# zyt334/AdaFace

Hardware: AMD Instinct MI355X
Metric: 512x512 images/sec @ 50 DDIM steps, batch 8 (higher is better)
Workload: dtype bf16

## Files before the change

adaface_amd/_lib.py:

```python
from __future__ import annotations

import ctypes as C
import os
from pathlib import Path

AF_DTYPE_BF16 = 0
AF_DTYPE_F32 = 1
AF_DTYPE_F16 = 2
DTYPES = {"bf16": AF_DTYPE_BF16, "bfloat16": AF_DTYPE_BF16, "f32": AF_DTYPE_F32, "fp32": AF_DTYPE_F32,
          "float32": AF_DTYPE_F32, "f16": AF_DTYPE_F16, "fp16": AF_DTYPE_F16, "float16": AF_DTYPE_F16}

_LIB_PATH = Path(__file__).resolve().parent / "libadaface_hip.so"


class AfConfig(C.Structure):
    _fields_ = [
        ("dtype", C.c_int),
        ("build_unet", C.c_int),
        ("in_channels", C.c_int), ("model_channels", C.c_int), ("out_channels", C.c_int),
        ("num_res_blocks", C.c_int),
        ("n_attention_resolutions", C.c_int), ("attention_resolutions", C.c_int * 8),
        ("n_channel_mult", C.c_int), ("channel_mult", C.c_int * 8),
        ("num_heads", C.c_int), ("context_dim", C.c_int), ("transformer_depth", C.c_int),
        ("n_context_layers", C.c_int),
        ("build_vae", C.c_int),
        ("vae_ch", C.c_int), ("vae_out_ch", C.c_int), ("vae_num_res_blocks", C.c_int),
        ("vae_z_channels", C.c_int), ("vae_embed_dim", C.c_int),
        ("n_vae_ch_mult", C.c_int), ("vae_ch_mult", C.c_int * 8),
        ("build_vae_encoder", C.c_int), ("vae_in_channels", C.c_int),
        ("build_clip", C.c_int),
        ("clip_vocab", C.c_int), ("clip_hidden", C.c_int), ("clip_layers", C.c_int), ("clip_heads", C.c_int),
        ("clip_intermediate", C.c_int), ("clip_max_pos", C.c_int),
    ]


class AfError(RuntimeError):
    pass


_lib = None

_P = C.c_void_p
_SIGS = [
    ("af_last_error", C.c_char_p, []),
    ("af_version", C.c_int, []),
    ("af_create", C.c_int, [C.c_int, C.POINTER(AfConfig), C.POINTER(_P)]),
    ("af_destroy", None, [_P]),
    ("af_load_tensor", C.c_int, [_P, C.c_char_p, _P, C.c_int, C.POINTER(C.c_int64)]),
    ("af_load_tensor_device", C.c_int, [_P, C.c_char_p, _P, C.c_int, C.POINTER(C.c_int64)]),
    ("af_num_tensors", C.c_int, [_P]),
    ("af_tensor_name", C.c_char_p, [_P, C.c_int]),
    ("af_tensor_loaded", C.c_int, [_P, C.c_int]),
    ("af_tensor_shape", C.c_int, [_P, C.c_int, C.POINTER(C.c_int64)]),
    ("af_set_context", C.c_int, [_P, _P, C.c_int, C.c_int, C.c_int, _P]),
    ("af_unet_forward", C.c_int, [_P, _P, _P, _P, C.c_int, C.c_int, C.c_int, _P]),
    ("af_unet_forward_twin", C.c_int, [_P, _P, _P, _P, C.c_int, C.c_int, C.c_int, _P]),
    ("af_unet_forward_cached", C.c_int, [_P, _P, _P, _P] + [C.c_int] * 6 + [_P]),
    ("af_unet_cache_invalidate", C.c_int, [_P]),
    ("af_ddim_step", C.c_int, [_P, _P, _P, _P, C.c_int64, C.c_float, C.c_float, C.c_float, C.c_float, C.c_float,
                               C.c_float, _P, _P, _P]),
    ("af_dpmpp_coeffs", C.c_int, [C.c_double, C.c_double, C.c_double, C.POINTER(C.c_double)]),
    ("af_dpmpp_step", C.c_int, [_P, _P, _P, _P, C.c_int64] + [C.c_float] * 7 + [_P, _P, _P]),
    ("af_philox4x32_10", C.c_int, [C.POINTER(C.c_uint32), C.POINTER(C.c_uint32), C.POINTER(C.c_uint32)]),
    ("af_philox_randn", C.c_int, [_P, C.c_int64, C.c_int64, _P, C.c_int64, C.c_uint64, C.c_uint32, C.c_uint32, _P]),
    ("af_dpmpp_sde_coeffs", C.c_int, [C.c_double, C.c_double, C.c_double, C.POINTER(C.c_double)]),
    ("af_dpmpp_sde_step", C.c_int, [_P, _P, _P, _P, C.c_int64] + [C.c_float] * 7 + [_P, _P, C.c_float, _P, C.c_int64, _P, C.c_int64,
                                    C.c_uint64, C.c_uint32, _P]),
    ("af_lincomb", C.c_int, [_P, C.c_int64, _P, C.c_float, _P, C.c_float, _P, C.c_float, _P, C.c_float, C.c_int, _P]),
    ("af_vae_decode", C.c_int, [_P, _P, C.c_float, _P, _P, C.c_int, C.c_int, C.c_int, _P]),
    ("af_to_uint8", C.c_int, [_P, _P, C.c_int, C.c_int, C.c_int, _P]),
    ("af_arena_bytes", C.c_int64, [_P]),
    ("af_prof_enable", C.c_int, [C.c_int]),
    ("af_prof_reset", C.c_int, []),
    ("af_set_conv_attn", C.c_int, [_P, C.c_int, C.c_int, C.POINTER(C.c_int), C.POINTER(C.c_int)]),
    ("af_vae_encode", C.c_int, [_P, _P, _P, C.c_int, C.c_int, C.c_int, _P]),
    ("af_posterior_sample", C.c_int, [_P, _P, C.c_float, _P, C.c_int, C.c_int, C.c_int, _P]),
    ("af_prof_set_stride", C.c_int, [C.c_int]),
    ("af_last_gemm_plan", C.c_int, [C.POINTER(C.c_int), C.POINTER(C.c_int), C.POINTER(C.c_int)]),
    ("af_prof_collect", C.c_int, [C.c_int, C.POINTER(C.c_double), C.POINTER(C.c_int64), C.POINTER(C.c_double),
                                  C.POINTER(C.c_double)]),
    ("af_prof_event_overhead_us", C.c_double, [_P, C.c_int]),
    ("af_unet_num_blocks", C.c_int, [_P]),
    ("af_unet_block_shape", C.c_int, [_P, C.c_int, C.c_int, C.c_int, C.POINTER(C.c_int), C.POINTER(C.c_int), C.POINTER(C.c_int)]),
    ("af_unet_set_tap", C.c_int, [_P, C.c_int, _P]),
    ("af_gemm_plan_counts", C.c_int, [C.POINTER(C.c_int64)]),
    ("af_gemm_plan_counts_reset", C.c_int, []),
    ("af_gemm_plan_query", C.c_int, [C.c_int, C.c_int64] + [C.c_int] * 16 + [C.POINTER(C.c_int64)]),
    ("af_norm_plan_query", C.c_int, [C.c_int, C.c_int, C.c_int, C.c_int64, C.c_int, C.c_int, C.POINTER(C.c_int64)]),
    ("af_knob_set", C.c_int, [C.c_char_p, C.c_int]),
    ("af_knob_get", C.c_int, [C.c_char_p, C.POINTER(C.c_int)]),
    ("af_knob_reset", C.c_int, []),
    ("af_op_conv2d", C.c_int, [C.c_int, _P, _P, _P, _P, _P] + [C.c_int] * 9 + [_P]),
    ("af_op_linear", C.c_int, [C.c_int, _P, _P, _P, _P, _P, C.c_int64, C.c_int, C.c_int, C.c_int, _P]),
    ("af_op_conv2d_ex", C.c_int, [C.c_int, _P, _P, _P, _P, _P, C.c_float, _P] + [C.c_int] * 10 + [_P]),
    ("af_op_linear_ex", C.c_int, [C.c_int, _P, _P, _P, _P, C.c_float, _P, C.c_int64, C.c_int, C.c_int, C.c_int, C.c_int, _P]),
    ("af_op_groupnorm", C.c_int, [C.c_int, _P, _P, _P, C.c_float, C.c_int, _P, C.c_int, C.c_int, C.c_int, C.c_int, _P]),
    ("af_op_conv_gn", C.c_int, [_P, _P, _P, _P, _P, _P, C.c_float, C.c_int, _P, _P] + [C.c_int] * 5 + [_P]),
    ("af_set_fp8", C.c_int, [_P, C.c_int]),
    ("af_fp8_gemm_launches", C.c_int64, []),
    ("af_set_fp8_scope", C.c_int, [_P, C.c_int]),
    ("af_get_fp8_scope", C.c_int, [_P]),
    ("af_ff8_launches", C.c_int64, []),
    ("af_op_ff_fp8", C.c_int, [_P] * 4 + [C.c_float] + [_P] * 5 + [C.c_int64] + [C.c_int] * 5 + [_P, _P, _P, C.POINTER(C.c_int), _P]),
    ("af_fp8_num_sites", C.c_int, [_P]),
    ("af_fp8_site_name", C.c_char_p, [_P, C.c_int]),
    ("af_fp8_record", C.c_int, [_P, C.c_int, _P]),
    ("af_fp8_read_record", C.c_int, [_P, C.c_int, C.POINTER(C.c_float), C.POINTER(C.c_int64), _P]),
    ("af_fp8_get_shifts", C.c_int, [_P, C.c_int, C.POINTER(C.c_int)]),
    ("af_fp8_set_shifts", C.c_int, [_P, C.c_int, C.POINTER(C.c_int)]),
    ("af_fp8_shift_for_amax", C.c_int, [C.c_float, C.c_int]),
    ("af_halo8_launches", C.c_int64, []),
    ("af_rowpanel_launches", C.c_int64, []),
    ("af_up_phase4_launches", C.c_int64, []),
    ("af_gn_producer_launches", C.c_int64, []),
    ("af_attn_short_launches", C.c_int64, []),
    ("af_gn_consumer_launches", C.c_int64, []),
    ("af_xattn_fused_launches", C.c_int64, []),
    ("af_conv_attn_short_launches", C.c_int64, []),
    ("af_op_conv_attention", C.c_int, [C.c_int, _P, _P, _P, _P] + [C.c_int] * 6 + [C.c_float] + [C.c_int] * 3 + [_P]),
    ("af_op_vae_attention", C.c_int, [C.c_int, _P, _P, _P, _P, C.c_int, C.c_int, C.c_int, _P, _P, C.POINTER(C.c_int), _P]),
    ("af_op_xattn_fused", C.c_int, [C.c_void_p] * 10 + [C.c_int] * 3 + [C.c_void_p]),
    ("af_op_conv2d_fp8", C.c_int, [_P, _P, _P, _P, _P] + [C.c_int] * 10 + [_P]),
    ("af_op_groupnorm_fp8", C.c_int, [_P, _P, _P, C.c_float, C.c_int, _P, C.c_int, C.c_int, C.c_int, C.c_int, C.c_int, _P]),
    ("af_op_layernorm_fp8", C.c_int, [_P, _P, _P, C.c_float, _P, C.c_int64, C.c_int, C.c_int, _P]),
    ("af_op_groupnorm_fp8_rec", C.c_int, [_P, _P, _P, C.c_float, C.c_int, _P, C.c_int, C.c_int, C.c_int, C.c_int, C.c_int, _P, _P]),
    ("af_op_layernorm_fp8_rec", C.c_int, [_P, _P, _P, C.c_float, _P, C.c_int64, C.c_int, C.c_int, _P, _P]),
    ("af_op_layernorm", C.c_int, [C.c_int, _P, _P, _P, C.c_float, _P, C.c_int64, C.c_int, _P]),
    ("af_op_attention", C.c_int, [C.c_int, _P, _P, _P, _P, C.c_int, C.c_int, C.c_int, C.c_int, C.c_int, C.c_float, C.c_int, _P]),
    ("af_clip_embed_tokens", C.c_int, [_P, _P, C.c_int64, _P, _P]),
    ("af_clip_text_forward", C.c_int, [_P, _P, C.c_int, C.c_int, C.c_float, C.c_float, _P, _P]),
    ("af_clip_text_forward3", C.c_int, [_P, _P, C.c_int, C.c_int, C.c_float, C.c_float, C.c_float, _P, _P]),
    ("af_op_timestep_embedding", C.c_int, [C.c_int, _P, _P, C.c_int, C.c_int, _P]),
    ("af_op_gn_conv1x1", C.c_int, [_P, _P, _P, C.c_float, _P, _P, _P, _P] + [C.c_int] * 5 + [_P]),
    ("af_set_tome", C.c_int, [_P, C.c_double, C.c_int]),
    ("af_tome_plan_query", C.c_int, [C.c_int, C.c_int, C.c_double, C.POINTER(C.c_int64)]),
    ("af_tome_num_sites", C.c_int, [_P]),
    ("af_tome_set_tap", C.c_int, [_P, C.c_int, _P]),
    ("af_op_tome_match", C.c_int, [C.c_int, _P] + [C.c_int] * 4 + [C.c_double, C.c_int, _P, _P, _P, _P]),
    ("af_op_tome_merge", C.c_int, [C.c_int, _P, _P, _P, C.c_float, _P] + [C.c_int] * 4 + [_P, _P]),
    ("af_op_tome_unmerge_add", C.c_int, [C.c_int, _P, _P, _P] + [C.c_int] * 4 + [_P, _P]),
    ("af_set_freeu", C.c_int, [_P, C.c_int] + [C.c_double] * 4),
    ("af_freeu_num_sites", C.c_int, [_P]),
    ("af_freeu_site", C.c_int, [_P, C.c_int, C.POINTER(C.c_int)]),
    ("af_freeu_plan_query", C.c_int, [C.c_int] * 6 + [C.POINTER(C.c_int64)]),
    ("af_op_freeu", C.c_int, [C.c_int, _P, _P] + [C.c_int] * 6 + [C.c_double, C.c_double, _P, _P, _P]),
    ("af_flops_issued", C.c_double, [C.c_int]),
    ("af_clock_probe", C.c_int, [_P, C.c_int, C.POINTER(C.c_double), C.POINTER(C.c_double)]),
]
EXPORTED_SYMBOLS = [s[0] for s in _SIGS]

DEEPCACHE_MODES = {"refresh": 1, "reuse": 2}


def lib_path() -> Path:
    return _LIB_PATH


def load():
    global _lib
    if _lib is not None:
        return _lib
    if not _LIB_PATH.exists():
        raise AfError(
            f"{_LIB_PATH} not found: build it with `python -m adaface_amd.build` (needs hipcc). "
            "adaface_amd has no fallback path.")
    lib = C.CDLL(os.fspath(_LIB_PATH))
    for name, res, args in _SIGS:
        fn = getattr(lib, name)
        fn.restype = res
        fn.argtypes = args
    _lib = lib
    return lib


def set_knob(name: str, value: int) -> None:
    check(load().af_knob_set(name.encode(), int(value)), f"af_knob_set({name})")


def reset_knobs() -> None:
    load().af_knob_reset()


def plan_counts(reset: bool = False) -> dict:
    lib = load()
    c = (C.c_int64 * 10)()
    check(lib.af_gemm_plan_counts(c), "af_gemm_plan_counts")
    out = {f"tile{i}": int(c[i]) for i in range(6)}
    out["halo"], out["splitk"], out["ln_consumer"], out["ln_producer"] = int(c[6]), int(c[7]), int(c[8]), int(c[9])
    out["fp8"] = int(lib.af_fp8_gemm_launches())
    out["ff8"] = int(lib.af_ff8_launches())
    out["halo8"] = int(lib.af_halo8_launches())
    out["rowpanel"] = int(lib.af_rowpanel_launches())
    out["up_phase4"] = int(lib.af_up_phase4_launches())
    out["gn_producer"] = int(lib.af_gn_producer_launches())
    out["attn_short"] = int(lib.af_attn_short_launches())
    out["gn_consumer"] = int(lib.af_gn_consumer_launches())
    out["xattn_fused"] = int(lib.af_xattn_fused_launches())
    out["conv_attn_short"] = int(lib.af_conv_attn_short_launches())
    if reset:
        lib.af_gemm_plan_counts_reset()
    return out


def gemm_plan_query(dtype, M, N, K, cin_pad, ks=1, stride=1, pad=0, up=0, Hs=1, Ws=None, Ho=1, Wo=None, ldc=None, ldo=None,
                    gn_hw=0, gn_cpg=0, flags=0) -> tuple:
    Ws = M if Ws is None else Ws
    Wo = M if Wo is None else Wo
    out = (C.c_int64 * 7)()
    check(load().af_gemm_plan_query(int(dtype), int(M), N, K, cin_pad, ks, stride, pad, up, Hs, Ws, Ho, Wo,
                                    cin_pad if ldc is None else ldc, N if ldo is None else ldo, gn_hw, gn_cpg, flags, out),
          "af_gemm_plan_query")
    return tuple(int(v) for v in out)


def tome_plan_query(H, W, ratio) -> tuple:
    out = (C.c_int64 * 4)()
    check(load().af_tome_plan_query(int(H), int(W), float(ratio), out), "af_tome_plan_query")
    return tuple(int(v) for v in out)


FREEU_KERNELS = ("refused", "single", "chunked")


def freeu_plan_query(dtype, H, W, Ch, Cs, version=1) -> dict:
    out = (C.c_int64 * 4)()
    dt = DTYPES[dtype] if isinstance(dtype, str) else int(dtype)
    check(load().af_freeu_plan_query(dt, int(H), int(W), int(Ch), int(Cs), int(version), out), "af_freeu_plan_query")
    return {"kernel": FREEU_KERNELS[int(out[0])], "launches": int(out[1]), "chunks": int(out[2]), "partial_bytes": int(out[3])}


GN_KERNELS = ("refused", "small", "fold", "finalize")
LN_KERNELS = ("refused", "wave_row", "rowgroup")
_Out5 = C.c_int64 * 5


def norm_plan_query(kind, dtype, B=1, HW=None, C=None, pre_npart=0, rows=None) -> dict:
    dt = DTYPES[dtype] if isinstance(dtype, str) else int(dtype)
    out = _Out5()
    if kind == "groupnorm":
        check(load().af_norm_plan_query(0, dt, int(B), int(HW), int(C), int(pre_npart), out), "af_norm_plan_query")
        return {"kernel": GN_KERNELS[out[0]], "P": int(out[1]), "nchunk": int(out[2]), "npart": int(out[3]), "wide": bool(out[4])}
    if kind == "layernorm":
        check(load().af_norm_plan_query(1, dt, 1, int(rows), int(C), 0, out), "af_norm_plan_query")
        return {"kernel": LN_KERNELS[out[0]], "nv": int(out[1]), "rows_per_block": int(out[2])}
    raise ValueError(f"norm_plan_query: kind {kind!r}")


def check(rc: int, what: str = "") -> None:
    if rc != 0:
        msg = load().af_last_error().decode("utf-8", "replace")
        raise AfError(f"{what or 'libadaface_hip'} failed (rc={rc}): {msg}")


def stream_ptr():
    import torch
    return C.c_void_p(torch.cuda.current_stream().cuda_stream)


def ptr(t):
    return C.c_void_p(0 if t is None else t.data_ptr())
```

adaface_amd/csrc/af_common.h:

```cpp
#pragma once
#include <hip/hip_runtime.h>
#include <stdint.h>
#include <atomic>

typedef __bf16 bf16;
typedef __attribute__((ext_vector_type(8))) __bf16 bf16x8;
typedef _Float16 f16;
typedef __attribute__((ext_vector_type(8))) _Float16 f16x8;
enum AfStorage { AF_ST_BF16 = 0, AF_ST_F32 = 1, AF_ST_F16 = 2 };
template <typename T> struct StorageOf;
template <> struct StorageOf<__bf16> { static constexpr AfStorage value = AF_ST_BF16; };
template <> struct StorageOf<float> { static constexpr AfStorage value = AF_ST_F32; };
template <> struct StorageOf<_Float16> { static constexpr AfStorage value = AF_ST_F16; };
typedef __attribute__((ext_vector_type(16))) float f32x16;
typedef __attribute__((ext_vector_type(4))) float f32x4;

#define AF_WAVE 64

#define HIP_CHECK_RET(expr)                                                       \
  do {                                                                            \
    hipError_t _e = (expr);                                                       \
    if (_e != hipSuccess) {                                                       \
      af_set_error_msg("%s failed: %s (%s:%d)", #expr, hipGetErrorString(_e),     \
                       __FILE__, __LINE__);                                       \
// ... 135 lines not shown
}
__device__ __forceinline__ float gelu_erf_f(float x) {
  return 0.5f * x * (1.0f + erf_as_f(x * 0.70710678118654752440f));
}
__device__ __forceinline__ float gelu_bf16out_f(float x) {
  const float u = x * fmaf(x * x, -0.07068715223f * 1.44269504089f, -1.59748341624f * 1.44269504089f);
  return x * __builtin_amdgcn_rcpf(1.0f + __builtin_amdgcn_exp2f(u));
}

typedef float f32x2 __attribute__((ext_vector_type(2)));
__device__ __forceinline__ f32x2 gelu_bf16out_f2(f32x2 x) {
  f32x2 xc;
  xc.x = __builtin_amdgcn_fmed3f(x.x, -4.0f, 4.0f);
  xc.y = __builtin_amdgcn_fmed3f(x.y, -4.0f, 4.0f);
  const f32x2 s = xc * xc;
  f32x2 q = s * 2.27794120e-08f + (-1.59850396e-06f);
  q = q * s + 4.79536935e-05f;
  q = q * s + (-8.13999317e-04f);
  q = q * s + 8.77231965e-03f;
  q = q * s + (-6.45729896e-02f);
  q = q * s + 3.97883296e-01f;
  const f32x2 ph = xc * q + 0.5f;
  return x * ph;
}

__device__ __forceinline__ unsigned gn_pack4_e4m3(float a, float b, float c, float d, float mul) {
  a = __builtin_amdgcn_fmed3f(a * mul, -448.f, 448.f);
  b = __builtin_amdgcn_fmed3f(b * mul, -448.f, 448.f);
  c = __builtin_amdgcn_fmed3f(c * mul, -448.f, 448.f);
  d = __builtin_amdgcn_fmed3f(d * mul, -448.f, 448.f);
  int v = 0;
  v = __builtin_amdgcn_cvt_pk_fp8_f32(a, b, v, false);
  v = __builtin_amdgcn_cvt_pk_fp8_f32(c, d, v, true);
  return (unsigned)v;
}

__device__ __forceinline__ void fp8_rec_note4(float a, float b, float c, float d, float mul, float& amax, unsigned& nsat) {
  a = fabsf(a); b = fabsf(b); c = fabsf(c); d = fabsf(d);
  amax = fmaxf(fmaxf(amax, fmaxf(a, b)), fmaxf(c, d));
  nsat += (unsigned)(a * mul > 448.f) + (unsigned)(b * mul > 448.f) + (unsigned)(c * mul > 448.f) + (unsigned)(d * mul > 448.f);
}
template <int WAVES = 4>
__device__ __forceinline__ void fp8_rec_commit(float amax, unsigned nsat, unsigned* __restrict__ rec) {
  __shared__ unsigned s_rec[2 * WAVES];
  unsigned m = __float_as_uint(amax);
#pragma unroll
  for (int o = 32; o > 0; o >>= 1) {
    m = max(m, (unsigned)__shfl_xor((int)m, o, 64));
    nsat += (unsigned)__shfl_xor((int)nsat, o, 64);
  }
  const int lane = threadIdx.x & 63, wave = threadIdx.x >> 6;
  if (lane == 0) { s_rec[wave] = m; s_rec[WAVES + wave] = nsat; }
  __syncthreads();
  if (threadIdx.x == 0) {
    if constexpr (WAVES == 4) {
      atomicMax(rec, max(max(s_rec[0], s_rec[1]), max(s_rec[2], s_rec[3])));
      atomicAdd(rec + 1, s_rec[4] + s_rec[5] + s_rec[6] + s_rec[7]);
    } else {
      unsigned mm = s_rec[0], nn = s_rec[WAVES];
#pragma unroll
      for (int w = 1; w < WAVES; ++w) { mm = max(mm, s_rec[w]); nn += s_rec[WAVES + w]; }
      atomicMax(rec, mm);
      atomicAdd(rec + 1, nn);
    }
  }
}

template <typename T> struct Mma;
template <> struct Mma<bf16> {
  static __device__ __forceinline__ void step(const uint4& a, const uint4& b, f32x16& c) {
    c = __builtin_amdgcn_mfma_f32_32x32x16_bf16(__builtin_bit_cast(bf16x8, a),
                                                __builtin_bit_cast(bf16x8, b), c, 0, 0, 0);
  }
};
template <> struct Mma<f16> {
  static __device__ __forceinline__ void step(const uint4& a, const uint4& b, f32x16& c) {
    c = __builtin_amdgcn_mfma_f32_32x32x16_f16(__builtin_bit_cast(f16x8, a), __builtin_bit_cast(f16x8, b), c, 0, 0, 0);
  }
};
template <> struct Mma<float> {
  static __device__ __forceinline__ void step(const uint4& a, const uint4& b, f32x16& c) {
    c = __builtin_amdgcn_mfma_f32_32x32x2f32(__builtin_bit_cast(float, a.x),
                                             __builtin_bit_cast(float, b.x), c, 0, 0, 0);
    c = __builtin_amdgcn_mfma_f32_32x32x2f32(__builtin_bit_cast(float, a.y),
                                             __builtin_bit_cast(float, b.y), c, 0, 0, 0);
    c = __builtin_amdgcn_mfma_f32_32x32x2f32(__builtin_bit_cast(float, a.z),
                                             __builtin_bit_cast(float, b.z), c, 0, 0, 0);
    c = __builtin_amdgcn_mfma_f32_32x32x2f32(__builtin_bit_cast(float, a.w),
                                             __builtin_bit_cast(float, b.w), c, 0, 0, 0);
  }
};

__device__ __forceinline__ int acc_row(int r, int h) { return (r & 3) + 8 * (r >> 2) + 4 * h; }

enum { AF_EPI_NONE = 0, AF_EPI_GEGLU = 1 };

struct ConvGemmParams {
  const void* src;
  long src_batch_stride;
  int ldc;
  int Cin;
  int Hs, Ws;
  int up;
  int Hi, Wi;
  int Ho, Wo;
  int ks, stride, pad;
  const void* W;
  int ldw;
  int Wrows;
  int M, N, K;
  int k_logical;
  const float* bias;
  const void* rowbias;
  int ldrb;
  const void* residual;
  int ldr;
  void* out;
  int ldo;
  int epilogue;
  float alpha;
  long bs_src, bs_w, bs_out, bs_res;
  int splitk;
  void* ws;
  int group_m;
  int howo_shift, wo_shift;
  float* ln_stats_out;
  const float* ln_stats;
  const float* ln_colsum;
  int ln_parts_n;
  float ln_inv_count, ln_eps;
  int epi_direct;
  int ablate;
  int fp8;
  const unsigned char* w_scale;
  int x_scale_e8;
  const void* W_up4;
  int phase4;
  float* gn_stats_out;
  int gn_cpg;
  const float* gn_ab;
  int gn_hw;
};

enum AfGemmKernel {
  AF_GK_NONE = 0,
  AF_GK_WAVE4 = 1,
  AF_GK_HALO4 = 2,
  AF_GK_PP = 3,
  AF_GK_PP_FP8 = 4,
  AF_GK_HALO8 = 5,
  AF_GK_S8 = 6,
  AF_GK_UP_PHASE4 = 7,
  AF_GK_ROWPANEL = 8,
  AF_GK_M128 = 9
};

struct AfGemmPlan {
  int kernel;
  int rowpanel;
  int tile;
  int splitk;
  size_t ws_bytes;
  int halo_tw;
  int group_m;
  int ln_slabs;
};
inline AfGemmPlan af_empty_plan(int kernel, int tile) { return AfGemmPlan{kernel, 0, tile, 1, 0, 0, 1, 0}; }

struct AttnParams {
  const void* q; const void* k; const void* v; void* o;
  int ldq, ldk, ldv, ldo;
  long bsq, bsk, bsv, bso;
  int Nq, Nk, H;
  float scale;
  float* lse;
  int causal;
  const void* vt_pack;
};
```

adaface_amd/csrc/af_conv_gemm.hip:

```cpp
#include "af_device.h"
#include "af_kernels.h"

#include <cstdlib>
#include <cstring>
#include <mutex>

template <int BM, int BN> struct TileCfg {
  static constexpr int XR = BM / 32, WR = BN / 32;
  static constexpr int WM = BM / 2, WN = BN / 2;
  static constexpr int MI = WM / 32, NI = WN / 32;
  static constexpr int TILE_BYTES = (BM + BN) * 128;
  static constexpr int EPI_LD = BN + 4;
  static constexpr int EPI_BYTES = BM * EPI_LD * 4;
  static constexpr int LDS_BYTES = (2 * TILE_BYTES > EPI_BYTES) ? 2 * TILE_BYTES : EPI_BYTES;
};

__device__ __forceinline__ void tile_coords(int wg, int nwg, int ntm, int ntn, int gm, int& tm, int& tn) {
  const int xcd = wg & 7, q = nwg >> 3, r = nwg & 7;
  wg = (xcd < r ? xcd * (q + 1) : r * (q + 1) + (xcd - r) * q) + (wg >> 3);
  const int per_group = gm * ntn;
  const int gid = wg / per_group;
  const int first_m = gid * gm;
  const int gsz = min(ntm - first_m, gm);
  const int in_g = wg - gid * per_group;
// ... 826 lines not shown
  auto dma = [&](__amdgpu_buffer_rsrc_t rs, char* dst, unsigned voff, unsigned soff) {
    if constexpr ((LABL & 1) == 0) lds_dma16(rs, dst, voff, soff);
  };

  if (!(lab & 32)) {
    const unsigned kc = (unsigned)chunk0 * 128u;
#pragma unroll
    for (int q = 0; q < NHQ; ++q)
      if (q < nhq) lds_dma16(rs_x, smem + (wid + 8 * q) * 1024, h_off[q], kc);
#pragma unroll
    for (int s = 0; s < 2; ++s) {
      char* const dst = smem + H::W_BASE + s * H::WBYTES + wid * 1024;
      lds_dma16(rs_w, dst, w_off[0], s * cin2 + kc);
      lds_dma16(rs_w, dst + 8 * 1024, w_off[1], s * cin2 + kc);
      if (g == 0) lds_dma16(rs_w, dst + 16 * 1024, w_off[2], s * cin2 + kc);
    }
  }
#ifdef AF_LAB_ABLATE
  if (lab & 64) st1 = lab_now();
#endif

  auto chunk_loop = [&](auto gc) {
    constexpr int G = decltype(gc)::value;
    constexpr int NWQ = G == 0 ? 3 : 2;
    constexpr int NHT = G == 0 ? 7 : 6;
    char* const wdst = smem + H::W_BASE + wid * 1024;
    for (int c = 0; c < nch; ++c) {
      const unsigned kc = (unsigned)(chunk0 + c) * 128u;
      const int nrec = c + 1 < nch ? (int)0xFFFFFFF0u : 0;
      const __amdgpu_buffer_rsrc_t rs_xn = buffer_rsrc(p.src, nrec);
      const __amdgpu_buffer_rsrc_t rs_wn = buffer_rsrc(p.W, nrec);
      const unsigned hrd8 = (lds0 + (unsigned)((c & 1) * H::HBUF)) >> 3;
      char* const hdst = smem + ((c & 1) ^ 1) * H::HBUF + wid * 1024;
      static_for<0, 9>([&](auto tc) {
        constexpr int TAP = decltype(tc)::value;
        constexpr int KY = TAP / 3, KX = TAP % 3, WS = TAP % 3, WS2 = (TAP + 2) % 3, T2 = TAP + 2;
        constexpr int NB = NI + MI;
        wait_vm<NWQ + (TAP >= 1 && TAP <= NHT ? 1 : 0)>();
        __builtin_amdgcn_s_barrier();
        const unsigned ut = hrd8 + KY * hw16 + KX * 16u;
        unsigned xa0[MI];
#pragma unroll
        for (int j = 0; j < MI; ++j) {
          const unsigned u = xh16[j] + ut;
          xa0[j] = (u << 3) | ((u ^ qsel16) & 0x70u);
        }
        u32x4 xc[MI][2];
        if constexpr ((LABL & 2) != 0) {
#pragma unroll
          for (int j = 0; j < MI; ++j) xc[j][0] = xc[j][1] = u32x4{0u, 0u, 0u, 0u};
        }
        auto rd_block = [&](auto bc) {
          constexpr int bi = decltype(bc)::value;
          if constexpr ((LABL & 2) != 0) {
          } else if constexpr (bi == 0) {
            w8[0][0] = lds_read128<WS * H::WBYTES>(wrd0);
            w8[0][1] = lds_read128<WS * H::WBYTES>(wrd1);
          } else if constexpr (bi <= MI) {
            xc[bi - 1][0] = lds_read128<0>(xa0[bi - 1]);
            xc[bi - 1][1] = lds_read128<0>(xa0[bi - 1] ^ 64u);
          } else {
            w8[bi - MI][0] = lds_read128<WS * H::WBYTES + (bi - MI) * 2048>(wrd0);
            w8[bi - MI][1] = lds_read128<WS * H::WBYTES + (bi - MI) * 2048>(wrd1);
          }
        };
        auto stage_w = [&](auto qc) {
          constexpr int q = decltype(qc)::value;
          char* const dst = wdst + WS2 * H::WBYTES + 8 * q * 1024;
          if constexpr (T2 < 9) dma(rs_w, dst, w_off[q], T2 * cin2 + kc);
          else dma(rs_wn, dst, w_off[q], (T2 - 9) * cin2 + kc + 128u);
        };
        auto stage_h = [&]() {
          if constexpr (TAP < NHT) {
            if constexpr (TAP < NHQ - 1) dma(rs_xn, hdst + 8 * TAP * 1024, h_off[TAP], kc + 128u);
            else dma(rs_xn, hdst + hl6, h_off[NHQ - 1], kc + 128u);
          }
        };
        rd_block(std::integral_constant<int, 0>{});
        rd_block(std::integral_constant<int, 1>{});
        __builtin_amdgcn_sched_barrier(0);
        static_for<0, MI * NI>([&](auto mc) {
          constexpr int m = decltype(mc)::value;
          if constexpr (m < MI) {
            mfma2(acc[NI - 1][m], w8[NI - 1], xp[m]);
          } else {
            constexpr int i = (m - MI) / MI, j = (m - MI) % MI;
            constexpr int issued = (2 + m) < NB ? (2 + m) : NB;
            constexpr int need = i == 0 ? 1 + j : (j == 0 ? MI + i : -1);
            if constexpr (need >= 0) {
              std::integral_constant<int, 2 * (issued - need - 1)> cnt;
              if constexpr (i == 0 && j == 0) wait_block2(cnt, xc[0], w8[0]);
              else if constexpr (i == 0) wait_block(cnt, xc[j]);
              else wait_block(cnt, w8[i]);
            }
            mfma2(acc[i][j], w8[i], xc[j]);
          }
          if constexpr (2 + m < NB) rd_block(std::integral_constant<int, 2 + m>{});
          if constexpr (m == MI + G) stage_w(std::integral_constant<int, 0>{});
          if constexpr (m == MI + 2 + G) stage_w(std::integral_constant<int, 1>{});
          if constexpr (G == 0 && m == MI + 4) stage_w(std::integral_constant<int, 2>{});
          if constexpr (m == MI + 6 + G) stage_h();
          __builtin_amdgcn_sched_barrier(0);
        });
        wait_lgkm_fenced<0>();
#pragma unroll
        for (int j = 0; j < MI; ++j) xp[j][0] = xc[j][0], xp[j][1] = xc[j][1];
      });
    }
  };
  if (g == 0) chunk_loop(std::integral_constant<int, 0>{});
  else chunk_loop(std::integral_constant<int, 1>{});
  wait_vm<0>();
#pragma unroll
  for (int j = 0; j < MI; ++j) mfma2(acc[NI - 1][j], w8[NI - 1], xp[j]);
  __builtin_amdgcn_s_barrier();
#ifdef AF_LAB_ABLATE
  if (lab & 64) st2 = lab_now();
#endif
  if (lab & 8) {
    float sum = 0.f;
#pragma unroll
    for (int i = 0; i < NI; ++i)
#pragma unroll
      for (int j = 0; j < MI; ++j) sum += acc[i][j][0] + acc[i][j][1] + acc[i][j][2] + acc[i][j][3];
    if (sum == 12345.678f) reinterpret_cast<float*>(p.out)[tid] = sum;
    return;
  }
  const int cl = 4 * (lane >> 4);
  float4 bias_r[NI];
#pragma unroll
  for (int i = 0; i < NI; ++i) {
    bias_r[i] = float4{0.f, 0.f, 0.f, 0.f};
    if (p.bias && p.splitk <= 1) bias_r[i] = *reinterpret_cast<const float4*>(p.bias + n0 + g * C::HN + i * 16 + cl);
  }
  float4 ln_cs[1];
  float ln_mu[1], ln_rs[1];
  pp_epilogue<160, 0>(p, acc, bias_r, ln_cs, ln_mu, ln_rs, smem, tid, lane, g, wq, m0, n0, tn, zk);
#ifdef AF_LAB_ABLATE
  if (lab & 64) {
    wait_vm<0>();
    __syncthreads();
    const unsigned long long st3 = lab_now();
    unsigned xcc, hwid;
    asm volatile("s_getreg_b32 %0, hwreg(HW_REG_XCC_ID)" : "=s"(xcc));
    asm volatile("s_getreg_b32 %0, hwreg(HW_REG_HW_ID)" : "=s"(hwid));
    if (tid == 0 && blockIdx.x < 2048 && blockIdx.z == 0) {
      unsigned long long* o = g_lab_stamps + (long)blockIdx.x * 5;
      o[0] = st0; o[1] = st1; o[2] = st2; o[3] = st3; o[4] = ((unsigned long long)xcc << 32) | hwid;
    }
  }
#endif
}

template <bool GEGLU, int KC_ = 5, int MJ_ = 2, int D_ = 2> struct RowPanelCfgT {
  static constexpr int KC = KC_, MJ = MJ_, K = KC * 64, D = D_, NS = D_ + 1;
  static constexpr int WROWS = 16 * MJ, BM = 8 * WROWS;
  static constexpr int BN = GEGLU ? 128 : 160;
  static constexpr int WBYTES = BN * 128, WPIECES = BN / 8;
  static constexpr int NIW = BN / 16;
  static constexpr int OCOLS = GEGLU ? BN / 2 : BN;
  static constexpr int OPITCH = OCOLS * 2 + 16, OBYTES = WROWS * OPITCH;
  static constexpr int LDS_BYTES = NS * WBYTES + 8 * OBYTES;
  static constexpr int CPR = OCOLS / 8;
  static constexpr int NST = WROWS * CPR / 64;
  static_assert(LDS_BYTES <= 160 * 1024 && (WROWS * CPR) % 64 == 0 && (MJ * KC == 10 || (MJ == 1 && KC == 20)) && D >= 2 && D <= KC,
                "row-panel LDS / store mapping / 80 (K = 1280, 16 rows per wave: 160) fragment registers / ring depth");
};
typedef RowPanelCfgT<true> RowPanelCfg;

template <bool GEGLU, int LNMODE, bool RES, int KC_ = 5, int MJ_ = 2, int D_ = 2>
__global__ __launch_bounds__(512) void rowpanel_kernel(const ConvGemmParams p) {
  using C = RowPanelCfgT<GEGLU, KC_, MJ_, D_>;
  typedef bf16 T;
  constexpr int KC = C::KC, NIW = C::NIW, MJ = C::MJ, NST = C::NST, CPR = C::CPR, D = C::D, NS = C::NS;
  static_assert(!(GEGLU && (RES || LNMODE == 2)), "GEGLU: plain or LayerNorm-consumer epilogue, no residual");
  extern __shared__ __attribute__((aligned(1024))) char smem[];
  const int tid = threadIdx.x, lane = tid & 63, wid = __builtin_amdgcn_readfirstlane(tid >> 6);
  const int m0 = blockIdx.x * C::BM;
  const int r0 = m0 + wid * C::WROWS;
  const int ntn_all = p.N / C::BN;
  const int nt_begin = (int)((long)blockIdx.y * ntn_all / gridDim.y), nt_end = (int)((long)(blockIdx.y + 1) * ntn_all / gridDim.y);
  const int ntn = nt_end - nt_begin;
  const __amdgpu_buffer_rsrc_t rs_x = buffer_rsrc(p.src);
  const __amdgpu_buffer_rsrc_t rs_w = buffer_rsrc(p.W);
  const __amdgpu_buffer_rsrc_t rs_o = buffer_rsrc(p.out);

  float* vecs = reinterpret_cast<float*>(smem + C::LDS_BYTES);
  const int nvcol = ntn * C::BN;
  float4 vb[3], vc[3];
#pragma unroll
  for (int r = 0; r < 3; ++r) {
    const int c4 = tid + 512 * r;
    const int col = nt_begin * C::BN + 4 * c4;
    vb[r] = vc[r] = float4{0.f, 0.f, 0.f, 0.f};
    if (c4 < nvcol / 4) {
      if (p.bias) vb[r] = *reinterpret_cast<const float4*>(p.bias + col);
      if constexpr (LNMODE == 1) vc[r] = *reinterpret_cast<const float4*>(p.ln_colsum + col);
    }
  }

  u32x4 xr[MJ][KC][2];
  unsigned orow[NST];
#pragma unroll
  for (int i = 0; i < NST; ++i) {
    const int c = lane + 64 * i;
    const int row = c / CPR, ch = c - row * CPR;
    const int m = r0 + row;
    orow[i] = m < p.M ? (unsigned)((long)m * p.ldo * 2) + (unsigned)ch * 16u : 0xFFFFFFFFu;
  }
  float ln_mu[LNMODE == 1 ? MJ : 1], ln_rs[LNMODE == 1 ? MJ : 1];
#pragma unroll
  for (int j = 0; j < MJ; ++j) {
    const int m = r0 + j * 16 + (lane & 15);
    const bool ok = m < p.M;
    const unsigned xo = ok ? (unsigned)((long)m * p.ldc * 2) + (unsigned)(lane >> 4) * 16u : 0xFFFFFFFFu;
#pragma unroll
    for (int kc = 0; kc < KC; ++kc)
#pragma unroll
      for (int u = 0; u < 2; ++u)
        xr[j][kc][u] = __builtin_bit_cast(u32x4, __builtin_amdgcn_raw_buffer_load_b128(rs_x, xo, (kc * 64 + u * 32) * 2, 0));
    if constexpr (LNMODE == 1) {
      float2 st = float2{0.f, 0.f};
      if (ok && p.ln_parts_n > 0) {
        float s1 = 0.f, s2 = 0.f;
        for (int q = 0; q < p.ln_parts_n; ++q) {
          const float2 pq2 = *reinterpret_cast<const float2*>(p.ln_stats + ((long)q * p.M + m) * 2);
          s1 += pq2.x;
          s2 += pq2.y;
        }
        st = ln_mu_rstd(s1, s2, p.ln_inv_count, p.ln_eps);
      } else if (ok) {
        st = *reinterpret_cast<const float2*>(p.ln_stats + (long)m * 2);
      }
      ln_mu[j] = st.x;
      ln_rs[j] = st.y;
    }
  }

#pragma unroll
  for (int r = 0; r < 3; ++r) {
    const int c4 = tid + 512 * r;
    if (c4 < nvcol / 4) {
      *reinterpret_cast<float4*>(vecs + 4 * c4) = vb[r];
      if constexpr (LNMODE == 1) *reinterpret_cast<float4*>(vecs + nvcol + 4 * c4) = vc[r];
    }
  }
  wait_lgkm<0>();

  if (p.gn_ab) {
    const float* ga = p.gn_ab + (long)(m0 / p.gn_hw) * 2 * C::K + 8 * (lane >> 4);
#pragma unroll
    for (int kc = 0; kc < KC; ++kc)
#pragma unroll
      for (int u = 0; u < 2; ++u) {
        const float* gp = ga + kc * 64 + u * 32;
        float sc[8], sh[8];
        *reinterpret_cast<float4*>(sc) = *reinterpret_cast<const float4*>(gp);
        *reinterpret_cast<float4*>(sc + 4) = *reinterpret_cast<const float4*>(gp + 4);
        *reinterpret_cast<float4*>(sh) = *reinterpret_cast<const float4*>(gp + C::K);
        *reinterpret_cast<float4*>(sh + 4) = *reinterpret_cast<const float4*>(gp + C::K + 4);
#pragma unroll
        for (int j = 0; j < MJ; ++j) {
          Vec16<T> v;
          v.u = __builtin_bit_cast(uint4, xr[j][kc][u]);
#pragma unroll
          for (int e = 0; e < 8; ++e) v.e[e] = from_f32<T>(fmaf(to_f32<T>(v.e[e]), sc[e], sh[e]));
          xr[j][kc][u] = __builtin_bit_cast(u32x4, v.u);
        }
      }
  }

  const int srow = lane >> 3;
  const unsigned dchunk = (unsigned)((lane & 7) ^ srow);
  constexpr int NWQ = (C::WPIECES + 7) / 8;
  const int nwq = (C::WPIECES - wid + 7) / 8;
  unsigned w_off[NWQ];
#pragma unroll
  for (int q = 0; q < NWQ; ++q) w_off[q] = (unsigned)(((wid + 8 * q) * 8 + srow) * p.ldw * 2) + dchunk * 16u;
  const int T_all = ntn * KC;
  const unsigned tile_stride = (unsigned)(C::BN * p.ldw * 2);
  auto stage = [&](int t, int slot) {
    const int ntl = t / KC, kc = t - ntl * KC;
    const bool live = t < T_all;
    const unsigned so = (unsigned)(nt_begin + ntl) * tile_stride + (unsigned)kc * 128u;
#pragma unroll
    for (int q = 0; q < NWQ; ++q)
      if (q < 2 || wid + 8 * q < C::WPIECES)
        lds_dma16(rs_w, smem + slot * C::WBYTES + (wid + 8 * q) * 1024, live ? w_off[q] : 0xFFFFFFFFu, so);
  };

  const unsigned lds0 = (unsigned)(__UINTPTR_TYPE__)((__attribute__((address_space(3))) char*)smem);
  const unsigned fch0 = (unsigned)((lane >> 4) ^ (lane & 7)) * 16u;
  const unsigned fch1 = (unsigned)(((lane >> 4) + 4) ^ (lane & 7)) * 16u;
  const unsigned w_base = (unsigned)((lane & 15) * 128);
  const int cl = 4 * (lane >> 4);

#ifdef AF_LAB_ABLATE
  const int lab = p.ablate >> 4;
#else
  constexpr int lab = 0;
#endif
  char* otile = smem + NS * C::WBYTES + wid * C::OBYTES;
  f32x4 acc[NIW][MJ];
  u32x4 wf[NIW][2];
  auto zero_acc = [&]() {
#pragma unroll
// ... 742 lines not shown
    const int idx = q * 4, u = idx >> 6, i = idx & 63;
    const int cc = u / taps, tap = u - cc * taps;
    float v[4] = {0.f, 0.f, 0.f, 0.f};
    if (cc * 64 < cin_pad) {
      const bf16* sp = wr + (long)tap * cin_pad + cc * 64 + i;
#pragma unroll
      for (int j = 0; j < 4; ++j) v[j] = to_f32<bf16>(sp[j]) * mul;
    }
    dst[q] = pack4_e4m3(v[0], v[1], v[2], v[3]);
  }
}
int af_launch_quant_weight_fp8(const void* w, int rows, int ldw, int cin_pad, int ks, void* w8, int k8, unsigned char* sc,
                               hipStream_t stream) {
  if (cin_pad % 64 != 0 || k8 % 128 != 0 || k8 < ks * ks * cin_pad || ldw != ks * ks * cin_pad) {
    af_set_error_msg("quant_weight_fp8: cin_pad=%d k8=%d ldw=%d ks=%d", cin_pad, k8, ldw, ks);
    return -1;
  }
  hipLaunchKernelGGL(quant_weight_fp8_kernel, dim3(rows), dim3(256), 0, stream, reinterpret_cast<const bf16*>(w), ldw,
                     cin_pad, ks * ks, reinterpret_cast<unsigned char*>(w8), k8, sc);
  HIP_CHECK_RET(hipGetLastError());
  return 0;
}
__global__ __launch_bounds__(256) void cast_fp8_kernel(const bf16* __restrict__ x, unsigned* __restrict__ y, long n4, float mul) {
  for (long i = (long)blockIdx.x * 256 + threadIdx.x; i < n4; i += (long)gridDim.x * 256) {
    Quad<bf16> q;
    q.load(x + i * 4);
    y[i] = pack4_e4m3(to_f32<bf16>(q.e[0]) * mul, to_f32<bf16>(q.e[1]) * mul, to_f32<bf16>(q.e[2]) * mul, to_f32<bf16>(q.e[3]) * mul);
  }
}
int af_launch_cast_fp8(const void* x, void* y, long n, float mul, hipStream_t stream) {
  if (n % 4 != 0) { af_set_error_msg("cast_fp8: n must be a multiple of 4"); return -1; }
  unsigned blocks = (unsigned)((n / 4 + 255) / 256);
  if (blocks > 8192) blocks = 8192;
  if (blocks == 0) return 0;
  hipLaunchKernelGGL(cast_fp8_kernel, dim3(blocks), dim3(256), 0, stream, reinterpret_cast<const bf16*>(x),
                     reinterpret_cast<unsigned*>(y), n / 4, mul);
  HIP_CHECK_RET(hipGetLastError());
  return 0;
}

static std::mutex g_last_plan_mu;
static AfGemmPlan g_af_last_plan = af_empty_plan(AF_GK_WAVE4, 0);
void af_set_last_plan(const AfGemmPlan& pl) { std::lock_guard<std::mutex> lk(g_last_plan_mu); g_af_last_plan = pl; }
AfGemmPlan af_get_last_plan() { std::lock_guard<std::mutex> lk(g_last_plan_mu); return g_af_last_plan; }
std::atomic<long> g_af_gn_consumer_launches{0};
std::atomic<long> g_af_ff8_launches{0};
std::atomic<long> g_af_plan_counts[AF_PC_COUNT] = {};

static void plan_group_m(AfGemmPlan& pl, const ConvGemmParams& p);

static AfGemmPlan plan_fp8(const ConvGemmParams& p, int batch) {
  AfGemmPlan pl = af_empty_plan(AF_GK_NONE, -1);
  const int cand = p.N % 160 == 0 ? 5 : (p.N % 128 == 0 ? 4 : -1);
  if (batch != 1 || p.epilogue == AF_EPI_GEGLU || cand < 0 || p.K % 128 != 0 || p.Cin % 64 != 0 || (p.ks != 1 && p.ks != 3) ||
      p.up != 0 || p.M < 512 || !g_af_knobs.gemm_pp)
    return pl;
  const int KT = p.K / 128;
  const long nb = (long)((p.M + 255) / 256) * (p.N / (cand == 5 ? 160 : 128));
  int s = 1;
  if (nb < 208) {
    s = (int)((256 + nb / 2) / nb);
    if (s > KT / 8) s = KT / 8;
    if (s > 16) s = 16;
    if (s < 1) s = 1;
  }
  const long nbs = nb * s;
  const double fill = (double)nbs / (double)(((nbs + 255) / 256) * 256);
  if (fill < g_af_knobs.gemm_pp_minfill * 0.01) return pl;
  pl.kernel = AF_GK_PP_FP8;
  pl.tile = cand;
  pl.splitk = s;
  plan_group_m(pl, p);
  return pl;
}

static AfGemmPlan plan_tiled(const ConvGemmParams& p, int batch, AfStorage st) {
  const int elem_size = st == AF_ST_F32 ? 4 : 2;
  const bool is_bf16 = st == AF_ST_BF16;
  AfGemmPlan pl = af_empty_plan(AF_GK_WAVE4, 0);
  const bool geglu = p.epilogue == AF_EPI_GEGLU;
  const bool n128 = geglu || (p.N % 128) == 0 || p.N > 640;
  static const int bm[4] = {128, 64, 128, 64}, bn[4] = {128, 128, 64, 64};
  static const double eff[4] = {1.0, 0.88, 0.88, 0.72};
  double best = 1e30;
  for (int t = 0; t < 4; ++t) {
    if (n128 && bn[t] != 128) continue;
    if (!n128 && bn[t] != 64) continue;
    const long nb = (long)((p.M + bm[t] - 1) / bm[t]) * ((p.N + bn[t] - 1) / bn[t]) * batch;
    const double rounds = (double)((nb + 255) / 256);
    const double cost = rounds * bm[t] * bn[t] / eff[t];
    if (cost < best) { best = cost; pl.tile = t; }
  }
  const int BK = 128 / elem_size;
  const int KT = p.K / BK;
  const long nb = (long)((p.M + bm[pl.tile] - 1) / bm[pl.tile]) * ((p.N + bn[pl.tile] - 1) / bn[pl.tile]) * batch;
  if (batch == 1 && !geglu && nb < 256 && KT >= 16) {
    const int target = g_af_knobs.splitk_target;
    int s = (int)((target + nb - 1) / nb);
    if (s > KT / 8) s = KT / 8;
    if (s > 16) s = 16;
    if (s >= 2) {
      pl.tile = n128 ? 0 : 2;
      const long nb2 = (long)((p.M + bm[pl.tile] - 1) / bm[pl.tile]) * ((p.N + bn[pl.tile] - 1) / bn[pl.tile]);
      s = (int)((target + nb2 - 1) / nb2);
      if (s > KT / 8) s = KT / 8;
      if (s > 16) s = 16;
      if (s >= 2) pl.splitk = s;
    }
  }
  if (g_af_knobs.small_m_tile64 && batch == 1 && !geglu && p.M <= 1024 && p.N % 64 == 0 && KT <= 32) {
    const long nb64 = (long)((p.M + 63) / 64) * (p.N / 64);
    if (nb64 >= 64 && nb64 <= 1024) { pl.tile = 3; pl.splitk = 1; }
  }
  if (p.ks == 3 && p.stride == 1 && p.up == 0 && p.pad == 1 && batch == 1 && !geglu && pl.splitk == 1 &&
      p.Ho == p.Hi && p.Wo == p.Wi && p.ldc >= p.Cin && g_af_knobs.conv_halo) {
    if (p.Wo % 32 == 0 && p.Ho % 4 == 0) pl.halo_tw = 32;
    else if (p.Wo % 16 == 0 && p.Ho % 8 == 0) pl.halo_tw = 16;
    if (pl.halo_tw) {
      const long nb128 = (long)(p.M / 128) * ((p.N + 127) / 128), nb64 = (long)(p.M / 128) * ((p.N + 63) / 64);
      const double c128 = (double)((nb128 + 255) / 256) * 128, c64 = (double)((nb64 + 255) / 256) * 64 / 0.9;
      pl.tile = (n128 && c128 <= c64) ? 0 : 2;
      if (!n128 && (p.N % 64) != 0) pl.tile = 2;
    }
  }
  if (is_bf16 && batch == 1 && p.K % 64 == 0 && p.Cin % 64 == 0 && g_af_knobs.gemm_pp) {
    int cand = -1;
    if (!geglu && p.N % 160 == 0) cand = 5;
    else if (p.N % 128 == 0) cand = 4;
    if (cand >= 0) {
      const int tbn = cand == 5 ? 160 : 128;
      const long nb = (long)((p.M + 255) / 256) * (p.N / tbn);
      int s = 1;
      if (!geglu && nb < 208) {
        s = (int)((256 + nb / 2) / nb);
        if (s > KT / 16) s = KT / 16;
        if (s > 16) s = 16;
        if (s < 1) s = 1;
      }
      const long nbs = nb * s;
      const double fill = (double)nbs / (double)(((nbs + 255) / 256) * 256);
      if (fill >= g_af_knobs.gemm_pp_minfill * 0.01 && p.M >= 512) {
        pl.tile = cand;
        pl.splitk = s;
        pl.halo_tw = 0;
      }
    }
  }
  if (pl.tile == 5 && pl.halo_tw == 0 && p.ks == 3 && p.stride == 1 && p.pad == 1 && p.up == 0 && p.Ho == p.Hi && p.Wo == p.Wi &&
      (p.Wo == 16 || p.Wo == 32 || p.Wo == 64) && (p.Ho & (p.Ho - 1)) == 0 && p.Ho >= 256 / p.Wo && p.M % 256 == 0 &&
      p.K == 9 * p.Cin && p.ldc >= p.Cin && (g_af_knobs.conv_halo8 & 1) && !p.ln_stats && !p.ln_stats_out) {
    pl.halo_tw = 256;
    while (pl.splitk > 1 && (p.Cin / 64) % pl.splitk != 0) --pl.splitk;
  }
  if (is_bf16 && (g_af_knobs.conv_halo8 & 2) && g_af_knobs.gemm_pp && af_conv_s8_slices(p, batch) && !p.gn_stats_out &&
      (p.Wo <= 16 || (g_af_knobs.conv_halo8 & 4))) {
    pl.tile = 5;
    pl.halo_tw = 8;
    pl.splitk = af_conv_s8_slices(p, batch);
  }
  const int ft = g_af_knobs.gemm_tile;
  if (ft >= 0 && ft < 4 && !(geglu && bn[ft] != 128)) pl.tile = ft;
  const int fs = g_af_knobs.gemm_splitk;
  if (fs >= 1 && batch == 1 && !geglu) pl.splitk = fs > KT ? KT : fs;
  if (pl.halo_tw == 8 && (pl.tile != 5 || pl.splitk != af_conv_s8_slices(p, batch))) pl.halo_tw = 0;
  if (pl.splitk > 1 && pl.halo_tw != 256 && pl.halo_tw != 8) pl.halo_tw = 0;
  if (pl.halo_tw == 256 && (pl.tile != 5 || (p.Cin / 64) % pl.splitk != 0)) pl.halo_tw = 0;
  pl.kernel = pl.halo_tw == 8 ? AF_GK_S8 : pl.halo_tw == 256 ? AF_GK_HALO8 : pl.halo_tw ? AF_GK_HALO4 : pl.tile >= 4 ? AF_GK_PP : AF_GK_WAVE4;
  plan_group_m(pl, p);
  return pl;
}

static void plan_group_m(AfGemmPlan& pl, const ConvGemmParams& p) {
  static const int bm[4] = {128, 64, 128, 64}, bn[4] = {128, 128, 64, 64};
  {
    const bool h4 = pl.kernel == AF_GK_HALO4;
    const int tbm = h4 ? 128 : (pl.tile >= 4 ? 256 : bm[pl.tile]);
    const int tbn = h4 ? ((pl.tile == 0 || pl.tile == 1) ? 128 : 64) : (pl.tile == 5 ? 160 : pl.tile == 4 ? 128 : bn[pl.tile]);
    const int MT = (p.M + tbm - 1) / tbm, NT = (p.N + tbn - 1) / tbn;
    const int resident = pl.tile >= 4 ? 32 : 32 * ((tbm * tbn >= 128 * 128) ? 2 : 3);
    const bool taps_reuse = pl.halo_tw || (pl.tile >= 4 && p.ks > 1);
    const double xb = (double)p.M * (p.K / (p.ks * p.ks)) * (taps_reuse ? (p.stride == 1 ? 1.5 : 1.0) : (double)(p.ks * p.ks) / (p.stride * p.stride));
    const double wb = (double)p.N * p.K;
    double bestc = 1e300;
    int bestg = 1;
    for (int gmm = 1; gmm <= 64; gmm *= 2) {
      const int gm_eff = gmm < MT ? gmm : MT;
      int gn_eff = resident / gm_eff;
      if (gn_eff < 1) gn_eff = 1;
      if (gn_eff > NT) gn_eff = NT;
      const double c = xb * ((double)NT / gn_eff) + wb * ((double)MT / gm_eff);
      if (c < bestc * 0.999) { bestc = c; bestg = gmm; }
    }
    pl.group_m = g_af_knobs.gemm_groupm >= 1 ? g_af_knobs.gemm_groupm : bestg;
  }
}

template <typename T, int BM, int BN, bool DMA>
static int launch_cfg2(const ConvGemmParams& p, int batch, hipStream_t stream) {
  using C = TileCfg<BM, BN>;
  const int ntm = (p.M + BM - 1) / BM, ntn = (p.N + BN - 1) / BN;
  dim3 grid(ntm * ntn, 1, p.splitk > 1 ? p.splitk : batch);
  return af_launch_lds<conv_gemm_kernel<T, BM, BN, DMA>>(grid, dim3(256), C::LDS_BYTES, C::LDS_BYTES, stream, p);
}
template <typename T, int BM, int BN>
static int launch_cfg(const ConvGemmParams& p, int batch, hipStream_t stream) {
  const int force = g_af_knobs.gemm_dma;
  const int kt_per_slice = p.K / (128 / (int)sizeof(T)) / (p.splitk > 1 ? p.splitk : 1);
  const bool use_dma = force >= 0 ? force != 0 : kt_per_slice >= 32;
  return use_dma ? launch_cfg2<T, BM, BN, true>(p, batch, stream) : launch_cfg2<T, BM, BN, false>(p, batch, stream);
}

static void set_launch_fields(ConvGemmParams& p, const AfGemmPlan& pl) {
  auto lg2 = [](int v) { int s = 0; while ((1 << s) < v) ++s; return (v > 0 && (1 << s) == v) ? s : -1; };
  p.howo_shift = lg2(p.Ho * p.Wo);
  p.wo_shift = lg2(p.Wo);
  p.group_m = pl.group_m > 0 ? pl.group_m : 1;
  p.epi_direct = (p.gn_stats_out || p.phase4) ? 1 : 0;
  p.ablate = p.phase4 ? 0 : g_af_knobs.ablate;
}

template <typename T> static int launch_splitk_reduce(const ConvGemmParams& p, hipStream_t stream) {
  const long nq = (long)p.M * (p.N >> 2);
  unsigned blocks = (unsigned)((nq + 255) / 256);
  if (blocks > 4096) blocks = 4096;
  hipLaunchKernelGGL((splitk_reduce_kernel<T>), dim3(blocks), dim3(256), 0, stream, p);
  HIP_CHECK_RET(hipGetLastError());
  return 0;
}

template <int BN, int LNMODE, bool GATHER, bool FP8, int SCHED>
static int launch_pp_one(const ConvGemmParams& p, dim3 grid, hipStream_t stream) {
  using C = PpCfg<BN>;
  return af_launch_lds<conv_gemm_pp_kernel<BN, GATHER, LNMODE, FP8, SCHED>>(grid, dim3(512), C::LDS_BYTES, C::LDS_BYTES, stream, p);
}
template <int BN, int LNMODE, bool GATHER> static int launch_pp_bf16(const ConvGemmParams& p, dim3 grid, hipStream_t stream) {
  const bool phased = p.epilogue == AF_EPI_GEGLU || (GATHER && !(p.up == 0 && p.ks * p.ks <= 31));
  if (!phased) return launch_pp_one<BN, LNMODE, GATHER, false, 2>(p, grid, stream);
  if constexpr (GATHER || (BN == 128 && LNMODE != 2)) return launch_pp_one<BN, LNMODE, GATHER, false, 0>(p, grid, stream);
  af_set_error_msg("conv_gemm: GEGLU on the ping-pong kernel needs the 128-column tile and no LayerNorm statistics");
  return -1;
}
template <int BN> static int launch_pp(const ConvGemmParams& p, hipStream_t stream) {
  const bool gather = !(p.ks == 1 && p.pad == 0);
  dim3 grid(((p.M + 255) / 256) * (p.N / BN), 1, p.splitk > 1 ? p.splitk : 1);
  if (p.ln_stats || p.ln_stats_out) {
    if (gather || p.splitk > 1 || (p.ln_stats && p.ln_stats_out) || (p.ln_stats_out && p.epilogue == AF_EPI_GEGLU)) {
      af_set_error_msg("conv_gemm: LayerNorm-fused launch needs a 1x1 GEMM without split-K");
      return -1;
    }
    return p.ln_stats ? launch_pp_bf16<BN, 1, false>(p, grid, stream) : launch_pp_bf16<BN, 2, false>(p, grid, stream);
  }
  return gather ? launch_pp_bf16<BN, 0, true>(p, grid, stream) : launch_pp_bf16<BN, 0, false>(p, grid, stream);
}

template <int BN> static int launch_pp8(const ConvGemmParams& p, hipStream_t stream) {
  const bool gather = !(p.ks == 1 && p.pad == 0);
  dim3 grid(((p.M + 255) / 256) * (p.N / BN), 1, p.splitk > 1 ? p.splitk : 1);
  return gather ? launch_pp_one<BN, 0, true, true, 2>(p, grid, stream) : launch_pp_one<BN, 0, false, true, 2>(p, grid, stream);
}

static int validate_fp8(const ConvGemmParams& p) {
  if (p.K % 128 != 0 || p.Cin % 64 != 0 || (p.ks != 1 && p.ks != 3) || p.K < p.ks * p.ks * p.Cin || p.ldw < p.K ||
      p.ldw % 16 != 0 || p.ldc % 16 != 0 || p.ldc < p.Cin || !p.w_scale || p.epilogue == AF_EPI_GEGLU || p.ln_stats || p.ln_stats_out) {
    af_set_error_msg("conv_gemm fp8: K=%d Cin=%d ks=%d ldw=%d ldc=%d (need K%%128==0, Cin%%64==0, ks 1|3, 16-byte pitches, row scales)",
                     p.K, p.Cin, p.ks, p.ldw, p.ldc);
    return -1;
  }
  return 0;
}

bool af_ff_geglu_fp8_ok(const ConvGemmParams& p) {
  return g_af_knobs.gemm_pp && p.fp8 && p.epilogue == AF_EPI_GEGLU && p.ks == 1 && p.pad == 0 && p.stride == 1 && p.up == 0 &&
         p.K % 128 == 0 && p.Cin % 64 == 0 && p.K >= p.Cin && p.ldw >= p.K && p.ldw % 16 == 0 && p.ldc % 16 == 0 && p.ldc >= p.Cin &&
         p.w_scale && p.N % 128 == 0 && p.Wrows >= p.N && p.ldo % 16 == 0 && p.ldo >= p.N / 2 && p.M >= 512 && !p.residual &&
         !p.rowbias && !p.ln_stats && !p.ln_stats_out && !p.gn_stats_out && !p.gn_ab &&
         (double)p.M * p.ldc < 4294967280.0 && (double)p.Wrows * p.ldw < 4294967280.0;
}
int af_launch_ff_geglu_fp8(ConvGemmParams p, float out_mul, unsigned* rec, hipStream_t stream) {
  if (!af_ff_geglu_fp8_ok(p) || ((__UINTPTR_TYPE__)p.out & 15) != 0 || !(out_mul > 0.f)) {
    af_set_error_msg("ff_geglu_fp8: M=%d N=%d K=%d Cin=%d ldo=%d cannot be launched (ask af_ff_geglu_fp8_ok first)", p.M, p.N, p.K, p.Cin, p.ldo);
    return -1;
  }
  using C = PpCfg<128>;
  AfGemmPlan pl = af_empty_plan(AF_GK_PP_FP8, 4);
  plan_group_m(pl, p);
  p.splitk = 1;
  p.ws = nullptr;
  set_launch_fields(p, pl);
  af_set_last_plan(pl);
  g_af_plan_counts[AF_PC_FP8] += 1;
  g_af_ff8_launches += 1;
  AfProfScope prof(AF_K_PP_FP8, stream, 2.0 * p.M * (double)p.N * (p.k_logical ? p.k_logical : p.K),
                   (double)p.M * p.Cin + (double)p.N * p.K + (double)p.M * p.N * 0.5);
  const dim3 grid(((p.M + 255) / 256) * (p.N / 128), 1, 1);
  if (rec) return af_launch_lds<ff_geglu_fp8_kernel<true>>(grid, dim3(512), C::LDS_BYTES, C::LDS_BYTES, stream, p, out_mul, rec);
  return af_launch_lds<ff_geglu_fp8_kernel<false>>(grid, dim3(512), C::LDS_BYTES, C::LDS_BYTES, stream, p, out_mul, nullptr);
}

template <int LABL> static int launch_halo8_lab(const ConvGemmParams& p, hipStream_t stream) {
  dim3 grid((p.M / 256) * (p.N / 160), 1, p.splitk > 1 ? p.splitk : 1);
  return af_launch_lds<conv3x3_halo8_kernel<LABL>>(grid, dim3(512), Halo8Cfg::LDS_BYTES, Halo8Cfg::LDS_BYTES, stream, p);
}
static int launch_halo8(const ConvGemmParams& p, hipStream_t stream) {
  if (p.Cin % 64 != 0 || (p.Cin / 64) % (p.splitk > 1 ? p.splitk : 1) != 0) {
    af_set_error_msg("conv_gemm: halo kernel needs K slices of whole 64-channel chunks (Cin=%d splitk=%d)", p.Cin, p.splitk);
    return -1;
  }
#ifdef AF_LAB_ABLATE
  switch ((p.ablate >> 4) & 7) {
    case 1: return launch_halo8_lab<1>(p, stream);
    case 2: return launch_halo8_lab<2>(p, stream);
    case 3: return launch_halo8_lab<3>(p, stream);
    case 4: return launch_halo8_lab<4>(p, stream);
    case 5: return launch_halo8_lab<5>(p, stream);
    case 6: return launch_halo8_lab<6>(p, stream);
    case 7: return launch_halo8_lab<7>(p, stream);
    default: break;
  }
#endif
  return launch_halo8_lab<0>(p, stream);
}

template <typename T, int TW, int BN> static int launch_halo(const ConvGemmParams& p, hipStream_t stream) {
  using C = HaloCfg<TW, BN>;
  dim3 grid((p.M / 128) * ((p.N + BN - 1) / BN), 1, 1);
  return af_launch_lds<conv3x3_halo_kernel<T, TW, BN>>(grid, dim3(256), C::LDS_BYTES, C::LDS_BYTES, stream, p);
}

__global__ __launch_bounds__(256) void up_phase4_weights_kernel(const bf16* __restrict__ w3, bf16* __restrict__ w4, long total,
                                                                int rows, int cin, int ldw3) {
  const long idx = (long)blockIdx.x * 256 + threadIdx.x;
  if (idx >= total) return;
  const int n = (int)(idx / cin), c = (int)(idx - (long)n * cin);
  float w[3][3];
#pragma unroll
  for (int ky = 0; ky < 3; ++ky)
#pragma unroll
    for (int kx = 0; kx < 3; ++kx) w[ky][kx] = to_f32<bf16>(w3[(long)n * ldw3 + (ky * 3 + kx) * cin + c]);
  const long ld4 = 4L * cin;
#pragma unroll
  for (int ph = 0; ph < 4; ++ph) {
    const int dy = ph >> 1, dx = ph & 1;
#pragma unroll
    for (int ty = 0; ty < 2; ++ty)
#pragma unroll
      for (int tx = 0; tx < 2; ++tx) {
        const int ylo = ty == 0 ? 0 : (dy == 0 ? 1 : 2), yhi = ty == 0 ? (dy == 0 ? 0 : 1) : 2;
        const int xlo = tx == 0 ? 0 : (dx == 0 ? 1 : 2), xhi = tx == 0 ? (dx == 0 ? 0 : 1) : 2;
        float sum = 0.f;
#pragma unroll
        for (int ky = 0; ky < 3; ++ky)
#pragma unroll
          for (int kx = 0; kx < 3; ++kx)
            if (ky >= ylo && ky <= yhi && kx >= xlo && kx <= xhi) sum += w[ky][kx];
        w4[((long)ph * rows + n) * ld4 + (ty * 2 + tx) * cin + c] = from_f32<bf16>(sum);
      }
  }
}
int af_launch_up_phase4_weights(const void* w3, int rows, int cin, int ldw3, void* w4, hipStream_t stream) {
  const long total = (long)rows * cin;
  if (total <= 0) return 0;
  hipLaunchKernelGGL(up_phase4_weights_kernel, dim3((unsigned)((total + 255) / 256)), dim3(256), 0, stream,
                     reinterpret_cast<const bf16*>(w3), reinterpret_cast<bf16*>(w4), total, rows, cin, ldw3);
  HIP_CHECK_RET(hipGetLastError());
  return 0;
}
static bool up_phase4_ok(const ConvGemmParams& p, int batch) {
  auto pow2 = [](int v) { return v > 0 && (v & (v - 1)) == 0; };
  return p.W_up4 && g_af_knobs.conv_up_phase4 && g_af_knobs.gemm_pp && batch == 1 && p.up == 1 && p.ks == 3 && p.stride == 1 &&
         p.pad == 1 && p.Cin % 64 == 0 && p.ldc >= p.Cin && p.K == 9 * p.Cin && (p.N % 160 == 0 || p.N % 128 == 0) &&
         pow2(p.Hs) && pow2(p.Ws) && p.Ho == 2 * p.Hs && p.Wo == 2 * p.Ws && p.M == (p.M / (p.Ho * p.Wo)) * p.Ho * p.Wo &&
         p.M / 4 >= 1024 && !p.residual && !p.rowbias && !p.ln_stats && !p.ln_stats_out && p.epilogue != AF_EPI_GEGLU &&
         (double)4 * p.Wrows * 4 * p.Cin * 2 < 4294967280.0;
}
static void up_phase4_params(ConvGemmParams& p) {
  p.W = p.W_up4;
  p.ks = 2; p.up = 0; p.pad = 1;
  p.Hi = p.Ho = p.Hs; p.Wi = p.Wo = p.Ws;
  p.M /= 4;
  p.K = 4 * p.Cin; p.ldw = p.K;
  p.k_logical = p.K;
  p.phase4 = 1;
  p.splitk = 1; p.ws = nullptr;
}
static int launch_up_phase4(const ConvGemmParams& p, int tile, hipStream_t stream) {
  const int bn = tile == 5 ? 160 : 128;
  dim3 grid(((p.M + 255) / 256) * (p.N / bn), 4, 1);
  return bn == 160 ? launch_pp_one<160, 0, true, false, 2>(p, grid, stream) : launch_pp_one<128, 0, true, false, 2>(p, grid, stream);
}

bool af_conv_gn_stats_ok(const ConvGemmParams& p, const AfGemmPlan& pl, int cpg) {
  auto pow2 = [](int v) { return v > 0 && (v & (v - 1)) == 0; };
  const int hn = pl.tile == 5 ? 80 : 64;
  const bool eight_wave = pl.kernel == AF_GK_PP || pl.kernel == AF_GK_PP_FP8 || pl.kernel == AF_GK_HALO8;
  return g_af_knobs.gn_producer && eight_wave && pl.splitk <= 1 && p.ks == 3 && p.stride == 1 && p.up == 0 &&
         p.epilogue != AF_EPI_GEGLU && !p.ln_stats && !p.ln_stats_out && cpg >= 2 && cpg % 2 == 0 && hn % cpg == 0 &&
         p.N == 32 * cpg && pow2(p.Ho * p.Wo) && p.Ho * p.Wo >= 64 && p.M % 64 == 0;
}

static int rowpanel_kind(const ConvGemmParams& p, int batch) {
  const int lvl = g_af_knobs.geglu_rowpanel;
  if (!lvl || batch != 1 || p.ks != 1 || p.pad != 0 || p.stride != 1 || p.up != 0 || p.rowbias || p.fp8 ||
      p.Cin != p.K || p.ldc < p.Cin)
    return 0;
  const bool geglu = p.epilogue == AF_EPI_GEGLU;
  if (p.K == RowPanelCfg::K && p.M >= 128 * RowPanelCfg::BM) {
    if (p.gn_ab && (p.gn_hw <= 0 || p.gn_hw % RowPanelCfg::BM != 0)) return 0;
    if (geglu) return (p.N % RowPanelCfg::BN == 0 && !p.residual && !p.ln_stats_out) ? 1 : 0;
    return (lvl >= 2 && p.N % 160 == 0 && p.alpha == 1.0f && !(p.ln_stats && p.ln_stats_out) && (!p.residual || p.ldr % 4 == 0)) ? 2 : 0;
  }
  if (g_af_knobs.gemm_m128 && !geglu && !(p.ln_stats && p.ln_stats_out) && (!p.ln_stats || p.alpha == 1.0f) && !p.gn_ab && p.M % 128 == 0 &&
      p.M <= 8192 && p.N % 160 == 0 &&
      p.K % 64 == 0 && p.K >= 256 && (!p.residual || p.ldr % 4 == 0) && p.ldo % 8 == 0 && ((__UINTPTR_TYPE__)p.out & 15) == 0) {
    const long nb128 = (long)(p.M / 128) * (p.N / 160), nb256 = (long)((p.M + 255) / 256) * (p.N / 160);
    if (nb128 >= 128 && nb128 <= 512 && nb256 <= 170) return 6;
    if (nb128 % 256 == 0 && nb128 <= 1024 && nb256 % 256 != 0) return 6;
  }
  if (g_af_knobs.gemm_m128 && !geglu && !(p.ln_stats && p.ln_stats_out) && (!p.ln_stats || p.alpha == 1.0f) && !p.gn_ab && p.M % 128 == 0 &&
      p.M > 8192 && p.M <= 16384 && p.N % 160 == 0 && p.K % 64 == 0 && p.K >= 256 && p.K <= 1280 && (!p.residual || p.ldr % 4 == 0) &&
      p.ldo % 8 == 0 && ((__UINTPTR_TYPE__)p.out & 15) == 0 && (long)(p.M / 128) * (p.N / 160) == 512)
    return 6;
  if (p.K == 1280)
    return (lvl >= 4 && p.N == 1280 && p.M >= 4096 && !geglu && p.alpha == 1.0f && !p.ln_stats && !p.ln_stats_out && !p.gn_ab &&
            (!p.residual || p.ldr % 4 == 0)) ? 3 : 0;
  if (p.K == 640 && lvl >= 3 && p.M >= 16384 && !p.residual) {
    if (p.gn_ab) return 0;
    if (p.ln_stats_out) return 0;
    if (geglu) return p.N % 128 == 0 ? 4 : 0;
    return (p.N % 160 == 0 && p.N >= 1920 && p.alpha == 1.0f) ? 5 : 0;
  }
  return 0;
}

AfGemmPlan af_plan_conv_gemm(const ConvGemmParams& p, int batch, AfStorage st, bool have_ws) {
  const bool is_bf16 = st == AF_ST_BF16;
  AfGemmPlan pl;
  if (p.fp8) {
    pl = plan_fp8(p, batch);
  } else if (is_bf16 && up_phase4_ok(p, batch)) {
    ConvGemmParams q = p;
    up_phase4_params(q);
    pl = af_empty_plan(AF_GK_UP_PHASE4, p.N % 160 == 0 ? 5 : 4);
    plan_group_m(pl, q);
    return pl;
  } else {
    pl = plan_tiled(p, batch, st);
    if (pl.kernel == AF_GK_PP && pl.splitk == 1) pl.ln_slabs = (p.N / (pl.tile == 5 ? 160 : 128)) * 2;
  }
  if (!have_ws) pl.splitk = 1;
  if (const int rk = is_bf16 ? rowpanel_kind(p, batch) : 0; rk == 6 || (rk && pl.splitk == 1)) {
    pl.kernel = rk == 6 ? AF_GK_M128 : AF_GK_ROWPANEL;
    pl.rowpanel = rk == 6 ? 0 : rk;
    pl.splitk = 1;
  }
  if (pl.splitk > 1) pl.ws_bytes = (size_t)pl.splitk * p.M * p.N * sizeof(float);
  return pl;
}

static int launch_bf16_only(const ConvGemmParams& p, const AfGemmPlan& pl, hipStream_t stream) {
  switch (pl.kernel) {
    case AF_GK_PP: return pl.tile == 4 ? launch_pp<128>(p, stream) : launch_pp<160>(p, stream);
    case AF_GK_PP_FP8: return pl.tile == 4 ? launch_pp8<128>(p, stream) : launch_pp8<160>(p, stream);
    case AF_GK_HALO8: return launch_halo8(p, stream);
    case AF_GK_S8: return af_launch_conv_s8(p, stream);
    case AF_GK_UP_PHASE4: return launch_up_phase4(p, pl.tile, stream);
    case AF_GK_M128: return launch_gemm_m128(p, stream);
    case AF_GK_ROWPANEL:
      switch (pl.rowpanel) {
        case 1: return launch_geglu_rowpanel(p, stream);
        case 2: return launch_plain_rowpanel(p, stream);
        case 3: return launch_plain_rowpanel_k1280(p, stream);
        case 4: return launch_geglu_rowpanel(p, stream, true);
        case 5: return launch_plain_rowpanel(p, stream, true);
        default: break;
      }
      break;
    default: break;
  }
  af_set_error_msg("conv_gemm: plan names no kernel (kernel %d, row-panel kind %d)", pl.kernel, pl.rowpanel);
  return -1;
}

template <typename T>
int af_launch_conv_gemm(const ConvGemmParams& p_in, int batch, hipStream_t stream, const AfGemmPlan* plan, void* ws) {
  constexpr int BK = 128 / sizeof(T);
  constexpr bool kBf16 = std::is_same_v<T, bf16>;
  ConvGemmParams p = p_in;
  if (p.fp8) {
    if (!kBf16) { af_set_error_msg("conv_gemm: fp8 operands need the bf16 storage mode"); return -1; }
    if (batch != 1) { af_set_error_msg("conv_gemm fp8: no batched form"); return -1; }
    if (int rc = validate_fp8(p)) return rc;
  } else {
    if (p.gn_ab && !kBf16) { af_set_error_msg("conv_gemm: consumer-side GroupNorm exists on the bf16 row-panel kernels only"); return -1; }
    if (p.K % BK != 0 || p.Cin % BK != 0 || p.K != p.ks * p.ks * p.Cin) {
      af_set_error_msg("conv_gemm: K=%d Cin=%d ks=%d must satisfy K==ks*ks*Cin and Cin%%%d==0", p.K, p.Cin, p.ks, BK);
      return -1;
    }
    if (p.ldw % (16 / (int)sizeof(T)) != 0 || p.ldc % (16 / (int)sizeof(T)) != 0) {
      af_set_error_msg("conv_gemm: ldw/ldc must be multiples of 16 bytes");
      return -1;
    }
    if (p.epilogue == AF_EPI_GEGLU && p.N % 64 != 0) { af_set_error_msg("conv_gemm: GEGLU needs N%%64==0"); return -1; }
  }
  if (p.N % 4 != 0 || p.ldo % 4 != 0 || (p.residual && p.ldr % 4 != 0) || (p.rowbias && p.ldrb % 4 != 0)) {
    af_set_error_msg("conv_gemm: N/ldo/ldr/ldrb must be multiples of 4 (N=%d ldo=%d)", p.N, p.ldo);
    return -1;
  }
  if (p.M <= 0 || p.N <= 0) return 0;
  {
    const int HoWo = p.Ho * p.Wo > 0 ? p.Ho * p.Wo : 1;
    const double nb = (double)((p.M + HoWo - 1) / HoWo), esz = p.fp8 ? 1.0 : (double)sizeof(T);
    const double src_bytes = nb * (double)p.src_batch_stride * esz, w_bytes = (double)p.Wrows * p.ldw * esz;
    if (src_bytes >= 4294967280.0 || w_bytes >= 4294967280.0) {
      af_set_error_msg("conv_gemm: operand of %.2f GB exceeds the 4 GB range of the 32-bit gather offsets (split the batch)",
                       (src_bytes > w_bytes ? src_bytes : w_bytes) / 1e9);
      return -1;
    }
  }
  const AfGemmPlan pl = (plan && (ws || plan->splitk <= 1)) ? *plan : af_plan_conv_gemm(p, batch, StorageOf<T>::value, ws != nullptr);
  const int k = pl.kernel;
  if ((k == AF_GK_PP_FP8) != (p.fp8 != 0)) {
    af_set_error_msg("conv_gemm%s: shape M=%d N=%d K=%d has no %s plan (ask af_plan_conv_gemm first)", p.fp8 ? " fp8" : "", p.M, p.N, p.K,
                     p.fp8 ? "fp8" : "bf16-operand");
    return -1;
  }
  if (!kBf16 && k != AF_GK_WAVE4 && k != AF_GK_HALO4) { af_set_error_msg("conv_gemm: kernel %d of the plan is bf16 only", k); return -1; }
  p.splitk = pl.splitk;
  p.ws = ws;
  af_set_last_plan(pl);
  if (g_af_knobs.plan_log && k != AF_GK_PP_FP8 && k != AF_GK_UP_PHASE4)
    fprintf(stderr, "[af plan] M=%ld N=%d K=%d ks=%d stride=%d up=%d HoWo=%dx%d batch=%d tile=%d halo=%d splitk=%d rowpanel=%d res=%d geglu=%d ln=%d\n",
            (long)p.M, p.N, p.K, p.ks, p.stride, p.up, p.Ho, p.Wo, batch, pl.tile, pl.halo_tw, pl.splitk, k == AF_GK_M128 ? 6 : pl.rowpanel,
            p.residual ? 1 : 0, p.epilogue == AF_EPI_GEGLU ? 1 : 0, (p.ln_stats || p.ln_stats_out) ? 1 : 0);
  if (k == AF_GK_PP_FP8 || k == AF_GK_UP_PHASE4) {
    g_af_plan_counts[k == AF_GK_PP_FP8 ? AF_PC_FP8 : AF_PC_UP_PHASE4] += 1;
  } else {
    g_af_plan_counts[k == AF_GK_HALO4 ? AF_PC_HALO4 : AF_PC_TILE0 + (pl.tile >= 0 && pl.tile < 6 ? pl.tile : 0)] += 1;
    if (k == AF_GK_HALO8) g_af_plan_counts[AF_PC_HALO8] += 1;
    if (p.ln_stats) g_af_plan_counts[AF_PC_LN_CONSUMER] += 1;
    if (p.ln_stats_out) g_af_plan_counts[AF_PC_LN_PRODUCER] += 1;
  }
  if (pl.splitk > 1) g_af_plan_counts[AF_PC_SPLITK] += 1;
  if (p.gn_stats_out) {
    if (!kBf16 || batch != 1 || !af_conv_gn_stats_ok(p, pl, p.gn_cpg)) {
      af_set_error_msg("conv_gemm: GroupNorm partial sums asked of a launch that cannot write them (ask af_conv_gn_stats_ok first)");
      return -1;
    }
    g_af_plan_counts[AF_PC_GN_PRODUCER] += 1;
  }
  const bool rows_resident = k == AF_GK_ROWPANEL || k == AF_GK_M128;
  if ((p.ln_stats || p.ln_stats_out) && k != AF_GK_PP && k != AF_GK_M128 && !(k == AF_GK_ROWPANEL && pl.tile >= 4)) {
    af_set_error_msg("conv_gemm: LayerNorm-fused launch planned on a kernel without that epilogue (kernel %d, tile %d)", k, pl.tile);
    return -1;
  }
  if (p.ln_parts_n > 0 && !rows_resident) {
    af_set_error_msg("conv_gemm: un-finalised LayerNorm statistics handed to a launch that is not a row-panel one");
    return -1;
  }
  if (p.gn_ab && k != AF_GK_ROWPANEL) {
    af_set_error_msg("conv_gemm: consumer-side GroupNorm asked of a launch that is not a row-panel one (ask af_plan_conv_gemm first)");
    return -1;
  }
  if (p.gn_ab) g_af_gn_consumer_launches += 1;
  if (rows_resident) g_af_plan_counts[AF_PC_ROWPANEL] += 1;
  if (k == AF_GK_UP_PHASE4) up_phase4_params(p);
  set_launch_fields(p, pl);
  int prof_cls = pl.tile == 5 ? ((p.ks == 1 && p.pad == 0) ? AF_K_PP160_PLAIN : AF_K_PP160_GATHER) : (pl.tile == 4 ? AF_K_PP128 : AF_K_CONV_GEMM);
  double flops = 2.0 * p.M * (double)p.N * (p.k_logical ? p.k_logical : p.K) * batch;
  double bytes = ((double)p.M * p.K / (p.ks * p.ks) + (double)p.N * p.K + (double)p.M * p.N) * batch * sizeof(T);
  if (k == AF_GK_HALO8) prof_cls = AF_K_HALO8;
  if (k == AF_GK_PP_FP8) { prof_cls = AF_K_PP_FP8; bytes = (double)p.M * p.Cin + (double)p.N * p.K + (double)p.M * p.N * 2.0; }
  if (k == AF_GK_UP_PHASE4) { flops *= 4; bytes = ((double)p.M * p.Cin + 4.0 * p.N * p.K + 4.0 * p.M * p.N) * 2; }
  AfProfScope prof(prof_cls, stream, flops, bytes);
  int rc;
  switch (k) {
    case AF_GK_WAVE4:
      switch (pl.tile) {
        case 0: rc = launch_cfg<T, 128, 128>(p, batch, stream); break;
        case 1: rc = launch_cfg<T, 64, 128>(p, batch, stream); break;
        case 2: rc = launch_cfg<T, 128, 64>(p, batch, stream); break;
        default: rc = launch_cfg<T, 64, 64>(p, batch, stream); break;
      }
      break;
    case AF_GK_HALO4: {
      const bool bn128 = pl.tile == 0 || pl.tile == 1;
      if (pl.halo_tw == 32) rc = bn128 ? launch_halo<T, 32, 128>(p, stream) : launch_halo<T, 32, 64>(p, stream);
      else rc = bn128 ? launch_halo<T, 16, 128>(p, stream) : launch_halo<T, 16, 64>(p, stream);
      break;
    }
    default:
      if constexpr (kBf16) rc = launch_bf16_only(p, pl, stream);
      else rc = -1;
      break;
  }
  if (rc) return rc;
  return p.splitk > 1 ? launch_splitk_reduce<T>(p, stream) : 0;
}

template int af_launch_conv_gemm<bf16>(const ConvGemmParams&, int, hipStream_t, const AfGemmPlan*, void*);
template int af_launch_conv_gemm<float>(const ConvGemmParams&, int, hipStream_t, const AfGemmPlan*, void*);
template int af_launch_conv_gemm<f16>(const ConvGemmParams&, int, hipStream_t, const AfGemmPlan*, void*);
```

adaface_amd/csrc/af_kernels.h:

```cpp
#pragma once
#include "af_common.h"

AfGemmPlan af_plan_conv_gemm(const ConvGemmParams& p, int batch, AfStorage st, bool have_ws = true);
template <typename T>
int af_launch_conv_gemm(const ConvGemmParams& p, int batch, hipStream_t stream, const AfGemmPlan* plan = nullptr,
                        void* ws = nullptr);
template <typename T> int af_launch_attention(const AttnParams& p, int B, int dh, hipStream_t stream);
template <typename T> long af_attn_short_pack_elems(int B, int H, int dh, int Nk);
template <typename T>
int af_launch_attn_short_pack(const void* v, int ldv, long bsv, int Nk, int H, int dh, int B, void* vt, hipStream_t stream);
extern std::atomic<long> g_af_attn_short_launches;
bool af_conv_attn_short_ok(bool is_bf16, int dh, int Nk, bool vt_pack, int ks, int groups);
int af_launch_conv_attn_short(const AttnParams& p, int B, int dh, int ks, int groups, int Hh, int Ww, const float* amap,
                              hipStream_t stream);
extern std::atomic<long> g_af_conv_attn_short_launches;
struct AfXattnFusedParams {
  const void* x; int ldx; int M; int rows_per_sample;
  const float* ln_stats; int ln_parts_n; float ln_inv_count, ln_eps;
  const void* wq; int ldwq; const float* q_colsum; const float* q_bias;
  const void* kvpack;
  const void* wo; int ldwo; const float* o_bias;
  void* out; int ldo;
  float* ln_stats_out;
  int Nk;
// ... 5 lines not shown
int af_launch_xattn_fused(const AfXattnFusedParams& a, hipStream_t stream);
extern std::atomic<long> g_af_xattn_fused_launches;

bool af_ff_geglu_fp8_ok(const ConvGemmParams& p);
int af_launch_ff_geglu_fp8(ConvGemmParams p, float out_mul, unsigned* rec, hipStream_t stream);
extern std::atomic<long> g_af_ff8_launches;

enum AfGnKernel {
  AF_GNK_REFUSED = 0,
  AF_GNK_SMALL = 1,
  AF_GNK_FOLD = 2,
  AF_GNK_FINALIZE = 3
};
struct AfGnPlan {
  int kernel;
  int P;
  int nchunk;
  int npart;
  int wide_stats;
};
AfGnPlan af_plan_groupnorm(AfStorage st, int B, int HW, int Cn, int pre_npart, bool to_affine = false);
enum AfLnKernel {
  AF_LNK_REFUSED = 0,
  AF_LNK_WAVE_ROW = 1,
  AF_LNK_ROWGROUP = 2
};
struct AfLnPlan {
  int kernel;
  int nv;
  int rows_per_block;
};
AfLnPlan af_plan_layernorm(AfStorage st, long rows, int Cn);

size_t af_gn_workspace_bytes(int B, int HW);
template <typename T>
int af_launch_groupnorm(const void* x, long x_bs, int ldx, int B, int HW, int Cn, const float* gamma,
                        const float* beta, float eps, int silu, void* y, long y_bs, int ldy, void* workspace,
                        hipStream_t stream, float fp8_mul = 0.f,
                        const float* pre_partial = nullptr, int pre_npart = 0,
                        unsigned* fp8_rec = nullptr);
template <typename T>
int af_launch_groupnorm_fold(const void* x, long x_bs, int ldx, int B, int HW, int Cn, const float* gamma, const float* beta,
                             float eps, void* workspace, hipStream_t stream, const float* pre_partial, int pre_npart,
                             float* ab_out);
bool af_conv_gn_stats_ok(const ConvGemmParams& p, const AfGemmPlan& pl, int cpg);
int af_conv_s8_slices(const ConvGemmParams& p, int batch);
int af_launch_conv_s8(const ConvGemmParams& p, hipStream_t stream);
template <typename T>
int af_launch_layernorm(const void* x, int ldx, long rows, int Cn, const float* gamma, const float* beta,
                        float eps, void* y, int ldy, hipStream_t stream, float fp8_mul = 0.f, unsigned* fp8_rec = nullptr);

struct AfTomePlan { long Nd, Ns, r, Np; };
int af_tome_plan(int H, int W, double ratio, AfTomePlan* pl);
size_t af_tome_match_ws_bytes(int B, int H, int W);
template <typename T>
int af_launch_tome_match(const void* x, int ldx, int B, int H, int W, int C, double ratio, int normalize, int* node_idx,
                         float* node_max, int* map, void* ws, hipStream_t s);
template <typename T>
int af_launch_tome_merge(const void* x, int ldx, const float* gamma, const float* beta, float eps, const int* map, int B, int N,
                         int Np, int C, void* y, int ldy, hipStream_t s);
template <typename T>
int af_launch_tome_unmerge_add(const void* o, int ldo, const void* res, int ldr, const int* map, int B, int N, int Np, int C,
                               void* y, int ldy, float* ln_stats_out, int ln_parts, hipStream_t s);

enum AfFreeuKernel {
  AF_FREEUK_REFUSED = 0,
  AF_FREEUK_SINGLE = 1,
  AF_FREEUK_CHUNKED = 2
};
struct AfFreeuPlan {
  int kernel;
  int launches;
  int nchunk;
  long part_bytes;
};
int af_plan_freeu(int H, int W, int Ch, int Cs, int version, AfFreeuPlan* pl);
size_t af_freeu_ws_bytes(int B, int H, int W, int Ch, int Cs, int version);
template <typename T>
int af_launch_freeu(void* cat, int ld, int B, int H, int W, int Ch, int Cs, int version, float b, float s, bool backbone,
                    bool skip, void* ws, hipStream_t stream);

template <typename T>
int af_launch_nchw_to_nhwc(const float* x, void* y, int B, int Cn, int HW, int Cpad, float scale, hipStream_t s);
template <typename T> int af_launch_nhwc_to_nchw(const void* x, float* y, int B, int Cn, int HW, int ld, hipStream_t s);
template <typename T> int af_launch_cast_f32(const float* x, void* y, long n, hipStream_t s);
template <typename T>
int af_launch_gather_rows_cast(const float* x, const int* rowmap, void* y, long rows, int D, hipStream_t s);
template <typename T>
int af_launch_conv_attn(const void* q, int ldq, long bsq, const void* kv, int ldk, long bsk, int tok0, float* sN,
                        float* lse, void* o, int ldo, long bso, int B, int N, int H, int dh, int Hh, int Ww,
                        float scale, int ks, hipStream_t s);
inline size_t af_conv_attn_map_floats(int groups, int B, int H, int N) { return (size_t)groups * B * H * N + 1; }
template <typename T>
int af_launch_conv_attn_map(const void* q, int ldq, long bsq, const void* k, int ldk, long bsk, int tok0, int groups,
                            float* amap, int B, int H, int dh, int Hh, int Ww, int ks, hipStream_t s);
template <typename T> int af_launch_cast_to_f32(const void* x, float* y, long n, hipStream_t s);
template <typename T> int af_launch_timestep_embedding(const long long* t, void* y, int B, int dim, hipStream_t s);
template <typename T> int af_launch_silu(const void* x, void* y, long n, hipStream_t s);
template <typename T> int af_launch_quick_gelu(const void* x, void* y, long n, hipStream_t s);
template <typename T>
int af_launch_embed_rows(const long long* ids, const void* table, int vocab, int D, float* y, long n, hipStream_t s);
template <typename T>
int af_launch_add_pos_cast(const float* x, const void* pos, int Tn, int D, void* y, long rows, hipStream_t s);
template <typename T> int af_launch_blend2(const void* a, float w0, const void* b, float w1, void* y, long n, hipStream_t s);
template <typename T>
int af_launch_copy_channels(const void* src, int lds_, void* dst, int ldd, int off, int Cn, long npix, hipStream_t s);
int af_launch_ddim_step(const float* x, const float* eps_c, const float* eps_u, const float* noise, long n,
                        float guidance, float a_t, float a_prev, float sqrt_one_minus_at, float sigma_t,
                        float temperature, float* x_prev, float* pred_x0, hipStream_t s);
int af_launch_dpmpp_step(const float* x, const float* eps_c, const float* eps_u, const float* x0_prev, long n, float guidance,
                         float alpha_t, float sigma_t, float c_x, float c_d, float w_cur, float w_prev, float* x_next,
                         float* x0_out, hipStream_t s);
int af_launch_posterior_sample(const float* mom, const float* noise, float scale, float* z, int B, int Cn, long HW,
                               hipStream_t s);
int af_launch_lincomb(float* out, long n, const float* x0, float w0, const float* x1, float w1, const float* x2, float w2,
                      const float* x3, float w3, int mode, hipStream_t s);
template <typename T> int af_launch_softmax_rows(void* x, int ld, int ncols, long rows, hipStream_t s);
template <typename T>
int af_launch_transpose(const void* x, long x_bs, int ldx, void* y, long y_bs, int R, int Cn, int B, hipStream_t s);
struct AfVaeAttnTaps {
  void* scores;
  void* probs;
  int plans[2][3];
};
bool af_vae_attn_shape_ok(int dtype, int N);
int af_vae_attn_core(int dtype, void* qkv, void* sc, void* vt, void* out, int B, int N, int C, hipStream_t s,
                     AfVaeAttnTaps* taps = nullptr);
template <typename T> int af_launch_to_uint8(const void* x, int ld, uint8_t* y, long npix, hipStream_t s);
int af_launch_nchw_to_uint8(const float* x, uint8_t* y, int B, int HW, hipStream_t s);

template <typename T>
int af_launch_repack_weight(const float* src, void* dst, int rows, int cin, int cin_pad, int ks, int ldw, int row_off,
                            int perm, hipStream_t s);
int af_launch_permute_bias(const float* src, float* dst, int rows, int perm, hipStream_t s);
template <typename T>
int af_launch_ln_fold(const void* W, void* Wf, const float* gamma, const float* beta, const float* bias, float* colsum,
                      float* biasf, int rows, int K, int ldw, hipStream_t s);

int af_launch_ln_finalize(const float* part, int parts, int M, int count, float eps, float* out, hipStream_t s);

void af_set_last_plan(const AfGemmPlan& pl);
AfGemmPlan af_get_last_plan();
enum AfPlanCount {
  AF_PC_TILE0 = 0,
  AF_PC_HALO4 = 6,
  AF_PC_SPLITK = 7,
  AF_PC_LN_CONSUMER = 8,
  AF_PC_LN_PRODUCER = 9,
  AF_PC_FP8 = 10,
  AF_PC_HALO8 = 11,
  AF_PC_ROWPANEL = 12,
  AF_PC_UP_PHASE4 = 13,
  AF_PC_GN_PRODUCER = 14,
  AF_PC_COUNT = 15
};
extern std::atomic<long> g_af_plan_counts[AF_PC_COUNT];
extern std::atomic<long> g_af_gn_consumer_launches;
int af_launch_up_phase4_weights(const void* w3, int rows, int cin, int ldw3, void* w4, hipStream_t stream);
int af_launch_quant_weight_fp8(const void* w, int rows, int ldw, int cin_pad, int ks, void* w8, int k8, unsigned char* sc,
                               hipStream_t stream);
int af_launch_cast_fp8(const void* x, void* y, long n, float mul, hipStream_t stream);
```

adaface_amd/csrc/af_model.hip:

```cpp
#include "../../include/adaface_hip.h"
#include "af_host.h"

#include <cmath>
#include <cstdarg>
#include <cstdio>
#include <cstdlib>
#include <cstring>
#include <algorithm>
#include <map>
#include <memory>
#include <string>
#include <vector>

static thread_local char g_err[1024] = "";
void af_set_error_msg(const char* fmt, ...) {
  va_list ap;
  va_start(ap, fmt);
  vsnprintf(g_err, sizeof(g_err), fmt, ap);
  va_end(ap);
}
static int knob_env(const char* name, int dflt) {
  const char* s = getenv(name);
  return s ? atoi(s) : dflt;
}
AfKnobs g_af_knobs = {
    knob_env("AF_SPLITK_TARGET", 320), knob_env("AF_CONV_HALO", 1),       knob_env("AF_GEMM_PP", 1),
    knob_env("AF_GEMM_PP_MINFILL", 50), knob_env("AF_GEMM_TILE", -1),
    knob_env("AF_GEMM_SPLITK", -1),    knob_env("AF_GEMM_GROUPM", -1),    knob_env("AF_GEMM_DMA", -1),
    knob_env("AF_ATTN_RING", 3),       knob_env("AF_GN_SMALL", 1),
    knob_env("AF_LN_FUSE", 1),         knob_env("AF_GEGLU_ROWPANEL", 4), knob_env("AF_CONV_HALO8", 3), knob_env("AF_ABLATE", 0),
    knob_env("AF_GN_PRODUCER", 1),     knob_env("AF_CONV_UP_PHASE4", 1), knob_env("AF_ATTN_SHORT", 1),
    knob_env("AF_GEMM_M128", 1),       knob_env("AF_SMALL_M_TILE64", 1),  knob_env("AF_GN_CONSUMER", 1),
    knob_env("AF_XATTN_FUSED", 1),     knob_env("AF_PLAN_LOG", 0),      knob_env("AF_FF8_MIN_K", 512),   knob_env("AF_FF8_MIN_ROWS", 0),
    knob_env("AF_CONV_ATTN_SHORT", 1)};
static const AfKnobs g_af_knobs_initial = g_af_knobs;
static int* knob_slot(const char* name) {
  static const struct { const char* n; int AfKnobs::*m; } tab[] = {
      {"splitk_target", &AfKnobs::splitk_target}, {"conv_halo", &AfKnobs::conv_halo}, {"gemm_pp", &AfKnobs::gemm_pp},
      {"gemm_pp_minfill", &AfKnobs::gemm_pp_minfill},
      {"gemm_tile", &AfKnobs::gemm_tile}, {"gemm_splitk", &AfKnobs::gemm_splitk}, {"gemm_groupm", &AfKnobs::gemm_groupm},
      {"gemm_dma", &AfKnobs::gemm_dma}, {"attn_ring", &AfKnobs::attn_ring},
      {"gn_small", &AfKnobs::gn_small}, {"ln_fuse", &AfKnobs::ln_fuse},
      {"geglu_rowpanel", &AfKnobs::geglu_rowpanel}, {"conv_halo8", &AfKnobs::conv_halo8}, {"ablate", &AfKnobs::ablate}, {"gn_producer", &AfKnobs::gn_producer}, {"conv_up_phase4", &AfKnobs::conv_up_phase4},
      {"attn_short", &AfKnobs::attn_short},
      {"gemm_m128", &AfKnobs::gemm_m128}, {"small_m_tile64", &AfKnobs::small_m_tile64}, {"gn_consumer", &AfKnobs::gn_consumer}, {"xattn_fused", &AfKnobs::xattn_fused}, {"plan_log", &AfKnobs::plan_log}, {"ff8_min_k", &AfKnobs::ff8_min_k}, {"ff8_min_rows", &AfKnobs::ff8_min_rows},
      {"conv_attn_short", &AfKnobs::conv_attn_short}};
  if (!name) return nullptr;
  for (auto& t : tab)
    if (strcmp(t.n, name) == 0) return &(g_af_knobs.*(t.m));
  return nullptr;
}

int g_af_prof_enabled = 0;
int g_af_prof_stride = 1;
std::atomic<long> g_af_prof_seen[AF_K_COUNT] = {};
std::atomic<double> g_af_flops_issued{0.0};
namespace {
struct ProfRec {
  hipEvent_t start, stop;
  int cls;
  double flops, bytes;
};
std::vector<ProfRec> g_prof_recs;
std::vector<hipEvent_t> g_prof_pool;
size_t g_prof_pool_used = 0;
hipEvent_t prof_event() {
  if (g_prof_pool_used == g_prof_pool.size()) {
    hipEvent_t e;
    hipEventCreate(&e);
    g_prof_pool.push_back(e);
  }
  return g_prof_pool[g_prof_pool_used++];
}
}
void af_prof_begin_impl(int cls, hipStream_t s, double flops, double bytes) {
  ProfRec r;
  r.start = prof_event();
  r.stop = prof_event();
  r.cls = cls;
  r.flops = flops;
  r.bytes = bytes;
  hipEventRecord(r.start, s);
  g_prof_recs.push_back(r);
}
void af_prof_end_impl(hipStream_t s) { hipEventRecord(g_prof_recs.back().stop, s); }

struct Arena {
  char* base = nullptr;
  size_t cap = 0, off = 0, peak = 0;
  bool dry = false;
  void* alloc(size_t bytes) {
    bytes = (bytes + 255) & ~(size_t)255;
    size_t o = off;
    off += bytes;
    if (off > peak) peak = off;
    if (dry) return reinterpret_cast<void*>((uintptr_t)0x1000 + o);
    if (off > cap) return nullptr;
    return base + o;
  }
  size_t mark() const { return off; }
  void release(size_t m) { off = m; }
};

struct Act {
  void* p = nullptr;
  int B = 0, H = 0, W = 0, C = 0;
  int ld = 0;
  bool f8 = false;
  int f8_shift = AF_FP8_SHIFT_DEFAULT;
  int f8_site = -1;
  const float* gn_part = nullptr;
  int gn_npart = 0;
  long npix() const { return (long)B * H * W; }
};

struct Linear {
  void* w = nullptr;
  float* bias = nullptr;
  int cin = 0, cin_pad = 0, cout = 0, ks = 1, rows_pad = 0, ldw = 0;
  bool geglu = false;
  void* w8 = nullptr;
  unsigned char* sc8 = nullptr;
  int k8 = 0;
  int f8_site = -1;
  void* w_up4 = nullptr;
};
struct Norm {
  float* gamma = nullptr;
  float* beta = nullptr;
  int C = 0;
  float eps = 1e-5f;
};
struct ResBlockW {
  Norm n1, n2;
  Linear c1, c2, skip;
  bool has_skip = false;
  int cin = 0, cout = 0;
  int emb_off = -1;
};
struct XfmrBlockW {
  Norm ln1, ln2, ln3;
  Linear qkv1, out1, q2, kv2, out2, ff1, ff2;
  Linear qkv1_ln, q2_ln, ff1_ln;
  float *qkv1_cs = nullptr, *q2_cs = nullptr, *ff1_cs = nullptr;
  void* out2_perm = nullptr;
};
struct XfmrW {
  int C = 0, heads = 0, dh = 0;
  Norm gn;
  Linear proj_in, proj_out;
  std::vector<XfmrBlockW> blocks;
  int ca_slot = -1;
  int ds = 1;
};
struct VaeAttnW {
  Norm gn;
  Linear qkv, proj_out;
  int C = 0;
};
struct ClipLayerW {
  Norm ln1, ln2;
  Linear qkv, out, fc1, fc2;
};
enum LayerKind { L_CONV_IN, L_RES, L_XFMR, L_DOWN, L_UP };
struct LayerRef {
  LayerKind kind;
  int idx;
};
struct UBlock {
  std::vector<LayerRef> layers;
};

struct Slot {
  enum Kind { WEIGHT, BIAS_VEC, TABLE } kind = WEIGHT;
  std::vector<int64_t> shape;
  void* dst = nullptr;
  int rows = 0, cin = 0, cin_pad = 0, ks = 1, ldw = 0, row_off = 0, perm = 0;
  float* dst_f = nullptr;
  bool loaded = false;
};

struct CtxKV {
  void* kv = nullptr;
// ... 2243 lines not shown
  if (!out) { af_set_error_msg("af_dpmpp_coeffs: null output"); return AF_ERR_INVALID; }
  if (!std::isfinite(acp_t) || !std::isfinite(acp_prev) || !std::isfinite(h_last)) {
    af_set_error_msg("af_dpmpp_coeffs: non-finite argument (acp_t %g, acp_prev %g, h_last %g)", acp_t, acp_prev, h_last);
    return AF_ERR_INVALID;
  }
  if (!(acp_t > 0.0 && acp_t < 1.0 && acp_prev > 0.0 && acp_prev < 1.0)) {
    af_set_error_msg("af_dpmpp_coeffs: acp_t %g / acp_prev %g outside (0, 1)", acp_t, acp_prev);
    return AF_ERR_INVALID;
  }
  if (!(acp_prev > acp_t)) {
    af_set_error_msg("af_dpmpp_coeffs: acp_prev %g <= acp_t %g (a step must go towards less noise)", acp_prev, acp_t);
    return AF_ERR_INVALID;
  }
  const double alpha_t = sqrt(acp_t), sigma_t = sqrt(1.0 - acp_t);
  const double alpha_p = sqrt(acp_prev), sigma_p = sqrt(1.0 - acp_prev);
  const double h = 0.5 * log((acp_prev * (1.0 - acp_t)) / (acp_t * (1.0 - acp_prev)));
  const bool second = h_last > 0.0;
  const double r = second ? h_last / h : 0.0;
  out[0] = alpha_t;
  out[1] = sigma_t;
  out[2] = sigma_p / sigma_t;
  out[3] = -alpha_p * expm1(-h);
  out[4] = second ? 1.0 + 1.0 / (2.0 * r) : 1.0;
  out[5] = second ? -1.0 / (2.0 * r) : 0.0;
  out[6] = h;
  out[7] = r;
  return AF_OK;
}

int af_dpmpp_step(const float* x_dev, const float* eps_cond_dev, const float* eps_uncond_dev, const float* x0_prev_dev, int64_t n,
                  float guidance, float alpha_t, float sigma_t, float c_x, float c_d, float w_cur, float w_prev,
                  float* x_next_dev, float* x0_out_dev, void* stream) {
  if (!x_dev || !eps_cond_dev || !x_next_dev || n <= 0) { af_set_error_msg("af_dpmpp_step: bad argument"); return AF_ERR_INVALID; }
  if (!(alpha_t > 0.f)) { af_set_error_msg("af_dpmpp_step: alpha_t %g is not positive", (double)alpha_t); return AF_ERR_INVALID; }
  auto overlaps = [n](const float* p, const float* q) {
    return p && q && (uintptr_t)p < (uintptr_t)(q + n) && (uintptr_t)q < (uintptr_t)(p + n);
  };
  if (overlaps(x0_out_dev, x0_prev_dev) || overlaps(x0_out_dev, x_dev) || overlaps(x0_out_dev, x_next_dev)) {
    af_set_error_msg("af_dpmpp_step: x0_out must not alias x0_prev, x or x_next");
    return AF_ERR_INVALID;
  }
  return af_launch_dpmpp_step(x_dev, eps_cond_dev, eps_uncond_dev, x0_prev_dev, (long)n, guidance, alpha_t, sigma_t, c_x, c_d,
                              w_cur, w_prev, x_next_dev, x0_out_dev, reinterpret_cast<hipStream_t>(stream));
}

int af_lincomb(float* out_dev, int64_t n, const float* x0_dev, float w0, const float* x1_dev, float w1,
               const float* x2_dev, float w2, const float* x3_dev, float w3, int mode, void* stream) {
  if (!out_dev || !x0_dev || n <= 0 || (mode == 1 && !x1_dev)) { af_set_error_msg("af_lincomb: bad argument"); return AF_ERR_INVALID; }
  return af_launch_lincomb(out_dev, (long)n, x0_dev, w0, x1_dev, w1, x2_dev, w2, x3_dev, w3, mode,
                           reinterpret_cast<hipStream_t>(stream));
}

int af_vae_decode(af_handle* h, const float* z_dev, float scale_factor, float* img_dev, uint8_t* u8_dev, int B, int H,
                  int W, void* stream) {
  if (!h || !z_dev || (!img_dev && !u8_dev)) { af_set_error_msg("af_vae_decode: null argument"); return AF_ERR_INVALID; }
  if (!h->cfg.build_vae) { af_set_error_msg("af_vae_decode: handle has no VAE"); return AF_ERR_STATE; }
  HIP_CHECK_RET(hipSetDevice(h->device));
  AF_TRY(check_loaded(h, "first_stage_model.decoder."));
  AF_TRY(check_loaded(h, "first_stage_model.post_quant_conv."));
  hipStream_t s = reinterpret_cast<hipStream_t>(stream);
  AF_TRY(ensure_up4_twins(h, s));
  auto run = [&] { return vae_decode_impl(h, s, z_dev, scale_factor, img_dev, u8_dev, B, H, W); };
  AF_TRY(run_sized(h, s, run));
  return run();
}

int af_vae_encode(af_handle* h, const float* x_dev, float* moments_dev, int B, int H, int W, void* stream) {
  if (!h || !x_dev || !moments_dev || B <= 0) { af_set_error_msg("af_vae_encode: bad argument"); return AF_ERR_INVALID; }
  if (!h->cfg.build_vae || !h->cfg.build_vae_encoder) { af_set_error_msg("af_vae_encode: handle has no VAE encoder"); return AF_ERR_STATE; }
  const int f = 1 << (h->cfg.n_vae_ch_mult - 1);
  if (H % f != 0 || W % f != 0) { af_set_error_msg("af_vae_encode: H, W must be multiples of %d", f); return AF_ERR_INVALID; }
  HIP_CHECK_RET(hipSetDevice(h->device));
  AF_TRY(check_loaded(h, "first_stage_model.encoder."));
  AF_TRY(check_loaded(h, "first_stage_model.quant_conv."));
  hipStream_t s = reinterpret_cast<hipStream_t>(stream);
  auto run = [&] { return vae_encode_impl(h, s, x_dev, moments_dev, B, H, W); };
  AF_TRY(run_sized(h, s, run));
  return run();
}

int af_posterior_sample(const float* moments_dev, const float* noise_dev, float scale, float* z_dev, int B, int C,
                        int HW, void* stream) {
  if (!moments_dev || !z_dev || B <= 0 || C <= 0 || HW <= 0) { af_set_error_msg("af_posterior_sample: bad argument"); return AF_ERR_INVALID; }
  return af_launch_posterior_sample(moments_dev, noise_dev, scale, z_dev, B, C, (long)HW, reinterpret_cast<hipStream_t>(stream));
}

int af_to_uint8(const float* img_dev, uint8_t* u8_dev, int B, int H, int W, void* stream) {
  if (!img_dev || !u8_dev) { af_set_error_msg("af_to_uint8: null argument"); return AF_ERR_INVALID; }
  return af_launch_nchw_to_uint8(img_dev, u8_dev, B, H * W, reinterpret_cast<hipStream_t>(stream));
}

int64_t af_arena_bytes(af_handle* h) { return h ? (int64_t)h->arena.cap : 0; }

int af_knob_set(const char* name, int value) {
  int* k = knob_slot(name);
  if (!k) { af_set_error_msg("af_knob_set: unknown knob '%s'", name ? name : "(null)"); return AF_ERR_NAME; }
  *k = value;
  return AF_OK;
}
int af_knob_get(const char* name, int* value) {
  int* k = knob_slot(name);
  if (!k || !value) { af_set_error_msg("af_knob_get: unknown knob '%s'", name ? name : "(null)"); return AF_ERR_NAME; }
  *value = *k;
  return AF_OK;
}
int af_knob_reset(void) {
  g_af_knobs = g_af_knobs_initial;
  return AF_OK;
}

int af_prof_enable(int class_mask) {
  g_af_prof_enabled = class_mask;
  return 0;
}
int af_prof_reset(void) {
  g_prof_recs.clear();
  g_prof_pool_used = 0;
  for (int c = 0; c < AF_K_COUNT; ++c) g_af_prof_seen[c] = 0;
  return 0;
}
double af_flops_issued(int reset) {
  const double v = reset ? g_af_flops_issued.exchange(0.0) : g_af_flops_issued.load();
  return v;
}
int af_prof_set_stride(int every) {
  if (every < 1) { af_set_error_msg("af_prof_set_stride: stride must be >= 1"); return AF_ERR_INVALID; }
  g_af_prof_stride = every;
  return AF_OK;
}
int af_last_gemm_plan(int* tile, int* splitk, int* halo_tw) {
  const AfGemmPlan lp = af_get_last_plan();
  if (tile) *tile = lp.tile;
  if (splitk) *splitk = lp.splitk;
  if (halo_tw) *halo_tw = lp.halo_tw;
  return AF_OK;
}
int af_gemm_plan_counts(int64_t* counts10) {
  if (!counts10) { af_set_error_msg("af_gemm_plan_counts: null argument"); return AF_ERR_INVALID; }
  for (int i = 0; i < 10; ++i) counts10[i] = g_af_plan_counts[i];
  return AF_OK;
}
int af_gemm_plan_counts_reset(void) {
  g_af_attn_short_launches = 0;
  g_af_xattn_fused_launches = 0;
  g_af_conv_attn_short_launches = 0;
  g_af_gn_consumer_launches = 0;
  g_af_ff8_launches = 0;
  for (int i = 0; i < AF_PC_COUNT; ++i) g_af_plan_counts[i] = 0;
  return AF_OK;
}
int64_t af_fp8_gemm_launches(void) { return g_af_plan_counts[AF_PC_FP8]; }
int64_t af_ff8_launches(void) { return g_af_ff8_launches; }
int64_t af_halo8_launches(void) { return g_af_plan_counts[AF_PC_HALO8]; }
int64_t af_rowpanel_launches(void) { return g_af_plan_counts[AF_PC_ROWPANEL]; }
int64_t af_up_phase4_launches(void) { return g_af_plan_counts[AF_PC_UP_PHASE4]; }
int64_t af_gn_producer_launches(void) { return g_af_plan_counts[AF_PC_GN_PRODUCER]; }
int64_t af_attn_short_launches(void) { return g_af_attn_short_launches; }
int64_t af_xattn_fused_launches(void) { return g_af_xattn_fused_launches; }
int64_t af_conv_attn_short_launches(void) { return g_af_conv_attn_short_launches; }
int64_t af_gn_consumer_launches(void) { return g_af_gn_consumer_launches; }
int af_set_fp8(af_handle* h, int on) {
  if (!h) { af_set_error_msg("af_set_fp8: null handle"); return AF_ERR_INVALID; }
  if (on && h->tome_ratio > 0.0) { af_set_error_msg("af_set_fp8: the fp8 mode does not combine with token merging (af_set_tome)"); return AF_ERR_STATE; }
  if (on && h->dtype != AF_DTYPE_BF16) { af_set_error_msg("af_set_fp8: the fp8 convolutions extend the bf16 mode (handle is %s)", h->dtype == AF_DTYPE_F16 ? "f16" : "f32"); return AF_ERR_STATE; }
  if (h->fp8_on != (on != 0)) h->dc.valid = false;
  h->fp8_on = on != 0;
  return AF_OK;
}
int af_set_fp8_scope(af_handle* h, int mask) {
  if (!h) { af_set_error_msg("af_set_fp8_scope: null handle"); return AF_ERR_INVALID; }
  if (h->dtype != AF_DTYPE_BF16) { af_set_error_msg("af_set_fp8_scope: the fp8 mode extends the bf16 mode (handle is %s)", h->dtype == AF_DTYPE_F16 ? "f16" : "f32"); return AF_ERR_STATE; }
  if (!(mask & AF_FP8_SCOPE_BASE) || (mask & ~(AF_FP8_SCOPE_BASE | AF_FP8_SCOPE_FF))) {
    af_set_error_msg("af_set_fp8_scope: mask %d (AF_FP8_SCOPE_BASE is always part of the scope, AF_FP8_SCOPE_FF may be added)", mask);
    return AF_ERR_INVALID;
  }
  if (mask != h->fp8_scope) h->dc.valid = false;
  if (mask != h->fp8_scope) h->fp8_dirty = true;
  h->fp8_scope = mask;
  return AF_OK;
}
int af_get_fp8_scope(af_handle* h) { return h ? h->fp8_scope : 0; }
int af_fp8_num_sites(af_handle* h) { return h ? h->fp8_nsites() : 0; }
const char* af_fp8_site_name(af_handle* h, int i) {
  if (!h || i < 0 || i >= h->fp8_nsites()) return nullptr;
  return h->fp8_site_names[i].c_str();
}
static int fp8_sites_arg(af_handle* h, int n, const char* who) {
  if (!h) { af_set_error_msg("%s: null handle", who); return AF_ERR_INVALID; }
  if (n != h->fp8_nsites()) { af_set_error_msg("%s: n = %d, the handle has %d fp8 sites in its scope", who, n, h->fp8_nsites()); return AF_ERR_INVALID; }
  return AF_OK;
}
int af_fp8_record(af_handle* h, int on, void* stream) {
  if (!h) { af_set_error_msg("af_fp8_record: null handle"); return AF_ERR_INVALID; }
  if (on && !h->fp8_rec) { af_set_error_msg("af_fp8_record: the handle has no fp8 sites (f32 or fp16 handle, or no UNet)"); return AF_ERR_STATE; }
  if (on) {
    HIP_CHECK_RET(hipSetDevice(h->device));
    HIP_CHECK_RET(hipMemsetAsync(h->fp8_rec, 0, h->fp8_shift.size() * 2 * sizeof(unsigned), reinterpret_cast<hipStream_t>(stream)));
  }
  h->fp8_recording = on != 0;
  return AF_OK;
}
int af_fp8_read_record(af_handle* h, int n, float* amax, int64_t* nsat, void* stream) {
  AF_TRY(fp8_sites_arg(h, n, "af_fp8_read_record"));
  if (n == 0) return AF_OK;
  if (!amax || !nsat) { af_set_error_msg("af_fp8_read_record: null output"); return AF_ERR_INVALID; }
  std::vector<unsigned> host(2 * (size_t)n);
  hipStream_t s = reinterpret_cast<hipStream_t>(stream);
  HIP_CHECK_RET(hipSetDevice(h->device));
  HIP_CHECK_RET(hipMemcpyAsync(host.data(), h->fp8_rec, host.size() * sizeof(unsigned), hipMemcpyDeviceToHost, s));
  HIP_CHECK_RET(hipStreamSynchronize(s));
  for (int i = 0; i < n; ++i) {
    memcpy(&amax[i], &host[2 * i], sizeof(float));
    nsat[i] = (int64_t)host[2 * i + 1];
  }
  return AF_OK;
}
int af_fp8_get_shifts(af_handle* h, int n, int* shifts) {
  AF_TRY(fp8_sites_arg(h, n, "af_fp8_get_shifts"));
  if (n && !shifts) { af_set_error_msg("af_fp8_get_shifts: null output"); return AF_ERR_INVALID; }
  for (int i = 0; i < n; ++i) shifts[i] = h->fp8_shift[i];
  return AF_OK;
}
int af_fp8_set_shifts(af_handle* h, int n, const int* shifts) {
  if (!h) { af_set_error_msg("af_fp8_set_shifts: null handle"); return AF_ERR_INVALID; }
  h->dc.valid = false;
  if (!shifts) {
    for (int& v : h->fp8_shift) v = AF_FP8_SHIFT_DEFAULT;
    return AF_OK;
  }
  AF_TRY(fp8_sites_arg(h, n, "af_fp8_set_shifts"));
  for (int i = 0; i < n; ++i)
    if (shifts[i] < AF_FP8_SHIFT_MIN || shifts[i] > AF_FP8_SHIFT_MAX) {
      af_set_error_msg("af_fp8_set_shifts: shift %d of site %d (%s) outside [%d, %d]", shifts[i], i, h->fp8_site_names[i].c_str(),
                       AF_FP8_SHIFT_MIN, AF_FP8_SHIFT_MAX);
      return AF_ERR_INVALID;
    }
  for (int i = 0; i < n; ++i) h->fp8_shift[i] = shifts[i];
  return AF_OK;
}
int af_fp8_shift_for_amax(float amax, int headroom) {
  if (!(amax > 0.f) || std::isinf(amax)) return AF_FP8_SHIFT_DEFAULT;
  int e = 0;
  const float m = frexpf(amax, &e);
  long sft = 9L - e - (m > 0.875f ? 1 : 0) - headroom;
  if (sft < AF_FP8_SHIFT_MIN) sft = AF_FP8_SHIFT_MIN;
  if (sft > AF_FP8_SHIFT_MAX) sft = AF_FP8_SHIFT_MAX;
  return (int)sft;
}
double af_prof_event_overhead_us(void* stream, int n) {
  hipStream_t s = reinterpret_cast<hipStream_t>(stream);
  if (n <= 0) n = 32;
  std::vector<hipEvent_t> ev(2 * (size_t)n);
  for (auto& e : ev) if (hipEventCreate(&e) != hipSuccess) return -1.0;
  for (int i = 0; i < n; ++i) { hipEventRecord(ev[2 * i], s); hipEventRecord(ev[2 * i + 1], s); }
  if (hipStreamSynchronize(s) != hipSuccess) return -1.0;
  double tot = 0.0;
  for (int i = 0; i < n; ++i) { float ms = 0.f; hipEventElapsedTime(&ms, ev[2 * i], ev[2 * i + 1]); tot += ms; }
  for (auto& e : ev) hipEventDestroy(e);
  return 1e3 * tot / n;
}
int af_prof_collect(int n_classes, double* ms, int64_t* launches, double* flops, double* bytes) {
  for (int c = 0; c < n_classes; ++c) { ms[c] = 0; launches[c] = 0; flops[c] = 0; bytes[c] = 0; }
  for (auto& r : g_prof_recs) {
    HIP_CHECK_RET(hipEventSynchronize(r.stop));
    float t = 0.f;
    HIP_CHECK_RET(hipEventElapsedTime(&t, r.start, r.stop));
    if (r.cls < n_classes) {
      ms[r.cls] += t;
      launches[r.cls] += 1;
      flops[r.cls] += r.flops;
      bytes[r.cls] += r.bytes;
    }
  }
  return 0;
}

}
```

adaface_amd/csrc/af_ops.hip:

```cpp
#include "../../include/adaface_hip.h"
#include "af_host.h"

#include <algorithm>
#include <cstring>
#include <vector>

namespace {
struct Tmp {
  std::vector<void*> bufs;
  void* get(size_t bytes, bool zero = false) {
    void* p = nullptr;
    if (hipMalloc(&p, bytes ? bytes : 16) != hipSuccess) return nullptr;
    if (zero) hipMemset(p, 0, bytes);
    bufs.push_back(p);
    return p;
  }
  ~Tmp() {
    hipDeviceSynchronize();
    for (void* p : bufs) hipFree(p);
  }
};
}

template <typename T> __global__ __launch_bounds__(256) void fill_cols_kernel(T* __restrict__ y, long rows, int ld, int c0, float v) {
// ... 387 lines not shown
  if (mid8_dev && hipMemcpyAsync(mid8_dev, f8, (size_t)M * F, hipMemcpyDeviceToDevice, s) != hipSuccess) return AF_ERR_HIP;
  ConvGemmParams q;
  memset(&q, 0, sizeof(q));
  q.src = f8; q.src_batch_stride = (long)M * F; q.ldc = F; q.Cin = F;
  q.Hs = 1; q.Ws = Mi; q.Hi = 1; q.Wi = Mi; q.Ho = 1; q.Wo = Mi;
  q.ks = 1; q.stride = 1; q.pad = 0;
  q.W = w28; q.ldw = k2; q.Wrows = rows2;
  q.M = Mi; q.N = Cout; q.K = k2; q.k_logical = F;
  q.bias = b2_dev ? reinterpret_cast<float*>(b2n) : nullptr;
  q.residual = rn; q.ldr = Cout; q.out = yn; q.ldo = Cout; q.alpha = 1.f;
  q.fp8 = 1; q.w_scale = sc2; q.x_scale_e8 = 127 - shift2;
  const AfGemmPlan pl = af_plan_conv_gemm(q, 1, AF_ST_BF16);
  if (pl.kernel != AF_GK_PP_FP8) { af_set_error_msg("af_op_ff_fp8: no fp8 plan for ff.net.2 M=%d N=%d K=%d", q.M, q.N, q.K); return AF_ERR_INVALID; }
  if (plan_out) { plan_out[0] = pl.tile; plan_out[1] = pl.splitk; }
  void* ws = nullptr;
  if (pl.splitk > 1) { ws = tmp.get(pl.ws_bytes, false); if (!ws) return AF_ERR_HIP; }
  AF_TRY(af_launch_conv_gemm<bf16>(q, 1, s, &pl, ws));
  AF_TRY(af_launch_cast_to_f32<bf16>(yn, y_dev, M * Cout, s));
  return 0;
}

int af_op_linear_ex(int dtype, const float* x_dev, const float* w_dev, const float* bias_dev, const float* residual_dev, float alpha,
                    float* y_dev, int64_t M, int K, int N, int geglu, int ld_slack, void* stream) {
  if (ld_slack < 0 || ld_slack % 8 != 0) { af_set_error_msg("af_op_linear_ex: ld_slack must be a non-negative multiple of 8"); return AF_ERR_INVALID; }
  hipStream_t s = reinterpret_cast<hipStream_t>(stream);
  Tmp tmp;
  const int kp = round_up(K, bk_of(dtype));
  const int rows = geglu ? 2 * N : N;
  const int rows_pad = round_up(rows, 128);
  const int no4 = round_up(N, 4);
  const int ldc = kp + ld_slack, ldo = no4 + ld_slack;
  OP_ALLOC(xn, (size_t)M * ldc * esize(dtype), false);
  OP_ALLOC(wn, (size_t)rows_pad * kp * esize(dtype), true);
  OP_ALLOC(yn, (size_t)M * ldo * esize(dtype), false);
  float* bn = nullptr;
  void* rn = nullptr;
  AF_TRY(fill_cols_dt(dtype, yn, M, ldo, 0, OP_SENTINEL, s));
  AF_TRY(AF_TYPED(dtype, af_launch_nchw_to_nhwc<Elem>(x_dev, xn, (int)M, K, 1, ldc, 1.f, s)));
  AF_TRY(fill_cols_dt(dtype, xn, M, ldc, kp, OP_NAN, s));
  AF_TRY(AF_TYPED(dtype, af_launch_repack_weight<Elem>(w_dev, wn, rows, K, kp, 1, kp, 0, geglu ? 1 : 0, s)));
  if (bias_dev) {
    bn = reinterpret_cast<float*>(tmp.get((size_t)rows_pad * 4, true));
    if (!bn) return AF_ERR_HIP;
    AF_TRY(af_launch_permute_bias(bias_dev, bn, rows, geglu ? 1 : 0, s));
  }
  if (residual_dev) {
    rn = tmp.get((size_t)M * ldo * esize(dtype), false);
    if (!rn) return AF_ERR_HIP;
    AF_TRY(AF_TYPED(dtype, af_launch_nchw_to_nhwc<Elem>(residual_dev, rn, (int)M, N, 1, ldo, 1.f, s)));
    AF_TRY(fill_cols_dt(dtype, rn, M, ldo, no4, OP_NAN, s));
  }
  ConvGemmParams p;
  memset(&p, 0, sizeof(p));
  p.src = xn; p.src_batch_stride = (long)M * ldc; p.ldc = ldc; p.Cin = kp;
  p.Hs = 1; p.Ws = (int)M; p.Hi = 1; p.Wi = (int)M; p.Ho = 1; p.Wo = (int)M;
  p.ks = 1; p.stride = 1; p.pad = 0;
  p.W = wn; p.ldw = kp; p.Wrows = rows_pad;
  p.M = (int)M; p.N = geglu ? 2 * N : no4; p.K = kp;
  p.bias = bn; p.residual = rn; p.ldr = ldo; p.out = yn; p.ldo = ldo;
  p.epilogue = geglu ? AF_EPI_GEGLU : AF_EPI_NONE;
  p.alpha = alpha;
  p.k_logical = K;
  const AfGemmPlan pl = af_plan_conv_gemm(p, 1, storage_of(dtype));
  void* ws = nullptr;
  if (pl.splitk > 1) { ws = tmp.get(pl.ws_bytes, false); if (!ws) return AF_ERR_HIP; }
  AF_TRY(AF_TYPED(dtype, af_launch_conv_gemm<Elem>(p, 1, s, &pl, ws)));
  if (ld_slack > 0) {
    AF_TRY(AF_TYPED(dtype, af_launch_cast_to_f32<Elem>(yn, y_dev, M * ldo, s)));
    return 0;
  }
  AF_TRY(AF_TYPED(dtype, af_launch_nhwc_to_nchw<Elem>(yn, y_dev, (int)M, N, 1, no4, s)));
  return 0;
}
int af_op_linear(int dtype, const float* x_dev, const float* w_dev, const float* bias_dev, const float* residual_dev,
                 float* y_dev, int64_t M, int K, int N, int geglu, void* stream) {
  return af_op_linear_ex(dtype, x_dev, w_dev, bias_dev, residual_dev, 1.f, y_dev, M, K, N, geglu, 0, stream);
}

int af_op_gn_conv1x1(const float* x_dev, const float* gamma_dev, const float* beta_dev, float eps, const float* w_dev,
                     const float* bias_dev, float* y_plain_dev, float* y_fused_dev, int B, int C, int H, int W, int N,
                     void* stream) {
  hipStream_t s = reinterpret_cast<hipStream_t>(stream);
  Tmp tmp;
  const int HW = H * W, rows_pad = round_up(N, 128);
  if (C % 64 || N % 4) { af_set_error_msg("af_op_gn_conv1x1: C %% 64 and N %% 4"); return AF_ERR_INVALID; }
  OP_ALLOC(xn, (size_t)B * HW * C * 2, false);
  OP_ALLOC(gn, (size_t)B * HW * C * 2, false);
  OP_ALLOC(wn, (size_t)rows_pad * C * 2, true);
  OP_ALLOC(y0, (size_t)B * HW * N * 2, true);
  OP_ALLOC(y1, (size_t)B * HW * N * 2, true);
  OP_ALLOC(ws, af_gn_workspace_bytes(B, HW), false);
  OP_ALLOC(ab, (size_t)B * 2 * C * sizeof(float), false);
  float* bn = nullptr;
  if (bias_dev) {
    bn = reinterpret_cast<float*>(tmp.get((size_t)rows_pad * 4, true));
    if (!bn) return AF_ERR_HIP;
    if (hipMemcpyAsync(bn, bias_dev, (size_t)N * 4, hipMemcpyDeviceToDevice, s) != hipSuccess) return AF_ERR_HIP;
  }
  AF_TRY(af_launch_nchw_to_nhwc<bf16>(x_dev, xn, B, C, HW, C, 1.f, s));
  AF_TRY(af_launch_repack_weight<bf16>(w_dev, wn, N, C, C, 1, C, 0, 0, s));
  ConvGemmParams p;
  memset(&p, 0, sizeof(p));
  p.src_batch_stride = (long)HW * C; p.ldc = C; p.Cin = C;
  p.Hs = H; p.Ws = W; p.Hi = H; p.Wi = W; p.Ho = H; p.Wo = W;
  p.ks = 1; p.stride = 1; p.pad = 0;
  p.W = wn; p.ldw = C; p.Wrows = rows_pad;
  p.M = B * HW; p.N = N; p.K = C; p.k_logical = C;
  p.bias = bn; p.ldo = N; p.alpha = 1.f;
  AF_TRY(af_launch_groupnorm<bf16>(xn, (long)HW * C, C, B, HW, C, gamma_dev, beta_dev, eps, 0, gn, (long)HW * C, C, ws, s));
  {
    ConvGemmParams q = p;
    q.src = gn; q.out = y0;
    const AfGemmPlan pl = af_plan_conv_gemm(q, 1, AF_ST_BF16);
    void* wsk = nullptr;
    if (pl.splitk > 1) { wsk = tmp.get(pl.ws_bytes, false); if (!wsk) return AF_ERR_HIP; }
    AF_TRY(af_launch_conv_gemm<bf16>(q, 1, s, &pl, wsk));
  }
  AF_TRY(af_launch_groupnorm_fold<bf16>(xn, (long)HW * C, C, B, HW, C, gamma_dev, beta_dev, eps, ws, s, nullptr, 0, (float*)ab));
  {
    ConvGemmParams q = p;
    q.src = xn; q.out = y1;
    q.gn_ab = (const float*)ab; q.gn_hw = HW;
    const AfGemmPlan pl = af_plan_conv_gemm(q, 1, AF_ST_BF16);
    if (pl.kernel != AF_GK_ROWPANEL) { af_set_error_msg("af_op_gn_conv1x1: M=%d K=%d N=%d has no row-panel launch", q.M, q.K, q.N); return AF_ERR_INVALID; }
    AF_TRY(af_launch_conv_gemm<bf16>(q, 1, s, &pl, nullptr));
  }
  AF_TRY(af_launch_nhwc_to_nchw<bf16>(y0, y_plain_dev, B, N, HW, N, s));
  AF_TRY(af_launch_nhwc_to_nchw<bf16>(y1, y_fused_dev, B, N, HW, N, s));
  return 0;
}

int af_op_groupnorm(int dtype, const float* x_dev, const float* gamma_dev, const float* beta_dev, float eps, int silu,
                    float* y_dev, int B, int C, int H, int W, void* stream) {
  hipStream_t s = reinterpret_cast<hipStream_t>(stream);
  Tmp tmp;
  const int HW = H * W;
  if (af_plan_groupnorm(storage_of(dtype), B, HW, C, 0).kernel == AF_GNK_REFUSED) {
    af_set_error_msg("af_op_groupnorm: unsupported B=%d C=%d %dx%d", B, C, H, W);
    return AF_ERR_INVALID;
  }
  OP_ALLOC(xn, (size_t)B * HW * C * esize(dtype), false);
  OP_ALLOC(yn, (size_t)B * HW * C * esize(dtype), false);
  OP_ALLOC(ws, af_gn_workspace_bytes(B, HW), false);
  AF_TRY(AF_TYPED(dtype, af_launch_nchw_to_nhwc<Elem>(x_dev, xn, B, C, HW, C, 1.f, s)));
  AF_TRY(AF_TYPED(dtype, af_launch_groupnorm<Elem>(xn, (long)HW * C, C, B, HW, C, gamma_dev, beta_dev, eps, silu, yn,
                                                   (long)HW * C, C, ws, s)));
  AF_TRY(AF_TYPED(dtype, af_launch_nhwc_to_nchw<Elem>(yn, y_dev, B, C, HW, C, s)));
  return 0;
}

int af_op_conv_gn(const float* x_dev, const float* w_dev, const float* bias_dev, const float* residual_dev,
                  const float* gamma_dev, const float* beta_dev, float eps, int silu, float* h_dev, float* y_dev, int B,
                  int Cin, int H, int W, int Cout, void* stream) {
  hipStream_t s = reinterpret_cast<hipStream_t>(stream);
  Tmp tmp;
  if (Cin % 64 != 0 || Cout % 32 != 0) { af_set_error_msg("af_op_conv_gn: Cin%%64==0 and Cout%%32==0"); return AF_ERR_INVALID; }
  const int HW = H * W, rows_pad = round_up(Cout, 128), ldw = 9 * Cin;
  OP_ALLOC(xn, (size_t)B * HW * Cin * 2, false);
  OP_ALLOC(wn, (size_t)rows_pad * ldw * 2, true);
  OP_ALLOC(hn, (size_t)B * HW * Cout * 2, true);
  OP_ALLOC(yn, (size_t)B * HW * Cout * 2, false);
  OP_ALLOC(ws, af_gn_workspace_bytes(B, HW), false);
  OP_ALLOC(st, (size_t)B * (HW / 64 + 1) * 32 * 2 * sizeof(float), true);
  void* rn = nullptr;
  float* bn = nullptr;
  AF_TRY(af_launch_nchw_to_nhwc<bf16>(x_dev, xn, B, Cin, HW, Cin, 1.f, s));
  AF_TRY(af_launch_repack_weight<bf16>(w_dev, wn, Cout, Cin, Cin, 3, ldw, 0, 0, s));
  if (bias_dev) {
    bn = reinterpret_cast<float*>(tmp.get((size_t)rows_pad * 4, true));
    if (!bn) return AF_ERR_HIP;
    if (hipMemcpyAsync(bn, bias_dev, (size_t)Cout * 4, hipMemcpyDeviceToDevice, s) != hipSuccess) return AF_ERR_HIP;
  }
  if (residual_dev) {
    rn = tmp.get((size_t)B * HW * Cout * 2, false);
    if (!rn) return AF_ERR_HIP;
    AF_TRY(af_launch_nchw_to_nhwc<bf16>(residual_dev, rn, B, Cout, HW, Cout, 1.f, s));
  }
  ConvGemmParams p;
  memset(&p, 0, sizeof(p));
  p.src = xn; p.src_batch_stride = (long)HW * Cin; p.ldc = Cin; p.Cin = Cin;
  p.Hs = H; p.Ws = W; p.Hi = H; p.Wi = W; p.Ho = H; p.Wo = W;
  p.ks = 3; p.stride = 1; p.pad = 1;
  p.W = wn; p.ldw = ldw; p.Wrows = rows_pad;
  p.M = B * HW; p.N = Cout; p.K = ldw;
  p.bias = bn; p.residual = rn; p.ldr = Cout; p.out = hn; p.ldo = Cout; p.alpha = 1.f;
  p.k_logical = 9 * Cin;
  const AfGemmPlan pl = af_plan_conv_gemm(p, 1, AF_ST_BF16);
  if (!af_conv_gn_stats_ok(p, pl, Cout / 32)) {
    af_set_error_msg("af_op_conv_gn: no GroupNorm-statistics producer plan for M=%d N=%d K=%d", p.M, p.N, p.K);
    return AF_ERR_INVALID;
  }
  p.gn_stats_out = reinterpret_cast<float*>(st);
  p.gn_cpg = Cout / 32;
  AF_TRY(af_launch_conv_gemm<bf16>(p, 1, s, &pl, nullptr));
  AF_TRY(af_launch_groupnorm<bf16>(hn, (long)HW * Cout, Cout, B, HW, Cout, gamma_dev, beta_dev, eps, silu, yn, (long)HW * Cout,
                                   Cout, ws, s, 0.f, reinterpret_cast<const float*>(st), HW / 64));
  AF_TRY(af_launch_nhwc_to_nchw<bf16>(hn, h_dev, B, Cout, HW, Cout, s));
  AF_TRY(af_launch_nhwc_to_nchw<bf16>(yn, y_dev, B, Cout, HW, Cout, s));
  return 0;
}

int af_op_layernorm(int dtype, const float* x_dev, const float* gamma_dev, const float* beta_dev, float eps,
                    float* y_dev, int64_t rows, int C, void* stream) {
  hipStream_t s = reinterpret_cast<hipStream_t>(stream);
  Tmp tmp;
  if (af_plan_layernorm(storage_of(dtype), rows, C).kernel == AF_LNK_REFUSED) {
    af_set_error_msg("af_op_layernorm: unsupported C=%d", C);
    return AF_ERR_INVALID;
  }
  OP_ALLOC(xn, (size_t)rows * C * esize(dtype), false);
  OP_ALLOC(yn, (size_t)rows * C * esize(dtype), false);
  AF_TRY(AF_TYPED(dtype, af_launch_cast_f32<Elem>(x_dev, xn, rows * C, s)));
  AF_TRY(AF_TYPED(dtype, af_launch_layernorm<Elem>(xn, C, rows, C, gamma_dev, beta_dev, eps, yn, C, s)));
  AF_TRY(AF_TYPED(dtype, af_launch_cast_to_f32<Elem>(yn, y_dev, rows * C, s)));
  return 0;
}

int af_op_attention(int dtype, const float* q_dev, const float* k_dev, const float* v_dev, float* o_dev, int B, int Nq,
                    int Nk, int heads, int dh, float scale, int causal, void* stream) {
  hipStream_t s = reinterpret_cast<hipStream_t>(stream);
  Tmp tmp;
  const int C = heads * dh;
  const long nq = (long)B * Nq * C, nk = (long)B * Nk * C;
  OP_ALLOC(qn, (size_t)nq * esize(dtype), false);
  const bool guard = (causal & 2) != 0;
  causal &= 1;
  const size_t tail = guard ? (size_t)128 * C * esize(dtype) : 0;
  OP_ALLOC(kn, (size_t)nk * esize(dtype) + tail, false);
  OP_ALLOC(vn, (size_t)nk * esize(dtype) + tail, false);
  if (guard) {
    if (hipMemsetAsync((char*)kn + (size_t)nk * esize(dtype), 0xFF, tail, s) != hipSuccess ||
        hipMemsetAsync((char*)vn + (size_t)nk * esize(dtype), 0xFF, tail, s) != hipSuccess) return AF_ERR_HIP;
  }
  OP_ALLOC(on, (size_t)nq * esize(dtype), true);
  AF_TRY(AF_TYPED(dtype, af_launch_cast_f32<Elem>(q_dev, qn, nq, s)));
  AF_TRY(AF_TYPED(dtype, af_launch_cast_f32<Elem>(k_dev, kn, nk, s)));
  AF_TRY(AF_TYPED(dtype, af_launch_cast_f32<Elem>(v_dev, vn, nk, s)));
  AttnParams p;
  p.q = qn; p.k = kn; p.v = vn; p.o = on; p.lse = nullptr; p.causal = causal;
  p.ldq = p.ldk = p.ldv = p.ldo = C;
  p.bsq = (long)Nq * C; p.bso = (long)Nq * C; p.bsk = (long)Nk * C; p.bsv = (long)Nk * C;
  p.Nq = Nq; p.Nk = Nk; p.H = heads; p.scale = scale;
  p.vt_pack = nullptr;
  if (dtype == AF_DTYPE_BF16 && !causal) {
    const long pe = af_attn_short_pack_elems<bf16>(B, heads, dh, Nk);
    if (pe > 0) {
      OP_ALLOC(vt, (size_t)pe * 2, false);
      AF_TRY(af_launch_attn_short_pack<bf16>(vn, C, (long)Nk * C, Nk, heads, dh, B, vt, s));
      p.vt_pack = vt;
    }
  }
  AF_TRY(AF_TYPED(dtype, af_launch_attention<Elem>(p, B, dh, s)));
  AF_TRY(AF_TYPED(dtype, af_launch_cast_to_f32<Elem>(on, o_dev, nq, s)));
  return 0;
}

int af_op_conv_attention(int dtype, const float* q_dev, const float* k_dev, const float* v_dev, float* o_dev, int B, int Hh,
                         int Ww, int Nk, int heads, int dh, float scale, int ks, int n_groups, int path, void* stream) {
  hipStream_t s = reinterpret_cast<hipStream_t>(stream);
  Tmp tmp;
  if (!q_dev || !k_dev || !v_dev || !o_dev || B <= 0 || Hh <= 0 || Ww <= 0 || heads <= 0 || dh <= 0 || dh > 160 || dh % 8 ||
      ks < 2 || ks > 4 || n_groups <= 0 || n_groups * ks * ks >= Nk || path < 0 || path > 2) {
    af_set_error_msg("af_op_conv_attention: B=%d map %dx%d Nk=%d heads=%d dh=%d ks=%d groups=%d path=%d", B, Hh, Ww, Nk, heads,
                     dh, ks, n_groups, path);
    return AF_ERR_INVALID;
  }
  const int C = heads * dh, N = Hh * Ww, nt = ks * ks;
  const long nq = (long)B * N * C, nk = (long)B * Nk * C;
  const bool bf = dtype == AF_DTYPE_BF16;
  const long pe = bf ? af_attn_short_pack_elems<bf16>(B, heads, dh, Nk) : 0;
  const bool can = af_conv_attn_short_ok(bf, dh, Nk, pe > 0, ks, n_groups);
  if (path == 2 && !can) {
    af_set_error_msg("af_op_conv_attention: no one-pass kernel for dtype %d, dh %d, %d keys, ks %d, %d subject strings (bf16, dh 40 / 80, "
                     "<= 96 keys)", dtype, dh, Nk, ks, n_groups);
    return AF_ERR_INVALID;
  }
  const bool one_pass = path == 2 || (path == 0 && can && g_af_knobs.conv_attn_short && g_af_knobs.attn_short);
  OP_ALLOC(qn, (size_t)nq * esize(dtype), false);
  OP_ALLOC(kn, (size_t)nk * esize(dtype), false);
  OP_ALLOC(vn, (size_t)nk * esize(dtype), false);
  OP_ALLOC(kvn, (size_t)2 * nk * esize(dtype), false);
  OP_ALLOC(on, (size_t)nq * esize(dtype), true);
  AF_TRY(AF_TYPED(dtype, af_launch_cast_f32<Elem>(q_dev, qn, nq, s)));
  AF_TRY(AF_TYPED(dtype, af_launch_cast_f32<Elem>(k_dev, kn, nk, s)));
  AF_TRY(AF_TYPED(dtype, af_launch_cast_f32<Elem>(v_dev, vn, nk, s)));
  AF_TRY(AF_TYPED(dtype, af_launch_copy_channels<Elem>(kn, C, kvn, 2 * C, 0, C, (long)B * Nk, s)));
  AF_TRY(AF_TYPED(dtype, af_launch_copy_channels<Elem>(vn, C, kvn, 2 * C, C, C, (long)B * Nk, s)));
  AttnParams p;
  p.q = qn; p.k = kvn; p.v = (char*)kvn + (size_t)C * esize(dtype); p.o = on; p.lse = nullptr; p.causal = 0;
  p.ldq = C; p.ldo = C; p.ldk = p.ldv = 2 * C;
  p.bsq = p.bso = (long)N * C; p.bsk = p.bsv = (long)Nk * 2 * C;
  p.Nq = N; p.Nk = Nk; p.H = heads; p.scale = scale;
  p.vt_pack = nullptr;
  if (one_pass) {
    OP_ALLOC(vt, (size_t)pe * 2, false);
    OP_ALLOC(amap, af_conv_attn_map_floats(n_groups, B, heads, N) * sizeof(float), false);
    AF_TRY(af_launch_attn_short_pack<bf16>(p.v, 2 * C, (long)Nk * 2 * C, Nk, heads, dh, B, vt, s));
    p.vt_pack = vt;
    AF_TRY(af_launch_conv_attn_map<bf16>(qn, C, (long)N * C, kvn, 2 * C, (long)Nk * 2 * C, Nk - n_groups * nt, n_groups,
                                         (float*)amap, B, heads, dh, Hh, Ww, ks, s));
    AF_TRY(af_launch_conv_attn_short(p, B, dh, ks, n_groups, Hh, Ww, (const float*)amap, s));
  } else {
    OP_ALLOC(lse, (size_t)B * heads * N * sizeof(float), false);
    OP_ALLOC(s9, (size_t)B * heads * N * nt * sizeof(float), false);
    p.lse = (float*)lse;
    p.Nk = Nk - n_groups * nt;
    AF_TRY(AF_TYPED(dtype, af_launch_attention<Elem>(p, B, dh, s)));
    for (int g = 0; g < n_groups; ++g) {
      const int tok0 = Nk - (n_groups - g) * nt;
      AF_TRY(AF_TYPED(dtype, af_launch_conv_attn<Elem>(qn, C, (long)N * C, kvn, 2 * C, (long)Nk * 2 * C, tok0, (float*)s9,
                                                       (float*)lse, on, C, (long)N * C, B, N, heads, dh, Hh, Ww, scale, ks, s)));
    }
  }
  AF_TRY(AF_TYPED(dtype, af_launch_cast_to_f32<Elem>(on, o_dev, nq, s)));
  return 0;
}

int af_op_vae_attention(int dtype, const float* q_dev, const float* k_dev, const float* v_dev, float* o_dev, int B, int N, int C,
                        float* scores_dev, float* probs_dev, int* plans6, void* stream) {
  hipStream_t s = reinterpret_cast<hipStream_t>(stream);
  Tmp tmp;
  if ((dtype != AF_DTYPE_BF16 && dtype != AF_DTYPE_F32 && dtype != AF_DTYPE_F16) || !q_dev || !k_dev || !v_dev || !o_dev ||
      B <= 0 || N <= 0 || C <= 0 || C % bk_of(dtype) != 0 || (double)B * N * std::max(N, C) >= 1073741824.0) {
    af_set_error_msg("af_op_vae_attention: dtype=%d B=%d N=%d C=%d (C: a multiple of the K tile; B * N * max(N, C) below 2^30)", dtype, B,
                     N, C);
    return AF_ERR_INVALID;
  }
  if (!af_vae_attn_shape_ok(dtype, N)) return AF_ERR_INVALID;
  const size_t es = esize(dtype), guard = 4096;
  const long nx = (long)B * N * C, nn = (long)B * N * N, ng = (long)(guard / es);
  const size_t tail = (size_t)128 * 3 * C * es;
  OP_ALLOC(qn, (size_t)nx * es, false);
  OP_ALLOC(kn, (size_t)nx * es, false);
  OP_ALLOC(vn, (size_t)nx * es, false);
  OP_ALLOC(qkv, (size_t)3 * nx * es + tail, false);
  OP_ALLOC(sc, (size_t)nn * es + guard, false);
  OP_ALLOC(vt, (size_t)nx * es + guard, false);
  OP_ALLOC(on, (size_t)nx * es + guard, false);
  HIP_CHECK_RET(hipMemsetAsync((char*)qkv + (size_t)3 * nx * es, 0xFF, tail, s));
  AF_TRY(fill_cols_dt(dtype, sc, 1, (int)(nn + ng), 0, OP_SENTINEL, s));
  AF_TRY(fill_cols_dt(dtype, vt, 1, (int)(nx + ng), 0, OP_SENTINEL, s));
  AF_TRY(fill_cols_dt(dtype, on, 1, (int)(nx + ng), 0, OP_SENTINEL, s));
  AF_TRY(AF_TYPED(dtype, af_launch_cast_f32<Elem>(q_dev, qn, nx, s)));
  AF_TRY(AF_TYPED(dtype, af_launch_cast_f32<Elem>(k_dev, kn, nx, s)));
  AF_TRY(AF_TYPED(dtype, af_launch_cast_f32<Elem>(v_dev, vn, nx, s)));
  AF_TRY(AF_TYPED(dtype, af_launch_copy_channels<Elem>(qn, C, qkv, 3 * C, 0, C, (long)B * N, s)));
  AF_TRY(AF_TYPED(dtype, af_launch_copy_channels<Elem>(kn, C, qkv, 3 * C, C, C, (long)B * N, s)));
// ... 164 lines not shown
```

adaface_amd/ops.py:

```python
from __future__ import annotations

import math

import torch

from . import _lib
from ._lib import DTYPES, check, ptr, stream_ptr


def _dev_f32(t: torch.Tensor) -> torch.Tensor:
    if not t.is_cuda:
        raise ValueError("adaface_amd.ops: tensors must live on the GPU (no CPU path)")
    return t.contiguous().float()


def conv2d(x, weight, bias=None, stride=1, padding=None, upsample=False, residual=None, dtype="bf16", rowbias=None, alpha=1.0,
           ld_slack=0):
    lib = _lib.load()
    x, weight = _dev_f32(x), _dev_f32(weight)
    B, Cin, H, W = x.shape
    Cout, Cin2, ks, ks2 = weight.shape
    if Cin2 != Cin or ks != ks2:
        raise ValueError(f"conv2d: weight {tuple(weight.shape)} does not match input {tuple(x.shape)}")
    pad = ks // 2 if padding is None else padding
    up = 1 if upsample else 0
    Hi, Wi = H << up, W << up
    if pad == 0 and ks == 3:
        Ho, Wo = (Hi + 1 - ks) // stride + 1, (Wi + 1 - ks) // stride + 1
    else:
        Ho, Wo = (Hi + 2 * pad - ks) // stride + 1, (Wi + 2 * pad - ks) // stride + 1
    b = None if bias is None else _dev_f32(bias)
    r = None if residual is None else _dev_f32(residual)
    if rowbias is None and alpha == 1.0 and ld_slack == 0 and pad == ks // 2:
        y = torch.empty(B, Cout, Ho, Wo, device=x.device, dtype=torch.float32)
        check(lib.af_op_conv2d(DTYPES[dtype], ptr(x), ptr(weight), ptr(b), ptr(r), ptr(y), B, Cin, H, W, Cout, ks, stride,
                               pad, up, stream_ptr()), "af_op_conv2d")
        return y
    rb = None if rowbias is None else _dev_f32(rowbias)
    if rb is not None and tuple(rb.shape) != (B, Cout):
        raise ValueError(f"conv2d: rowbias {tuple(rb.shape)} is not [{B}, {Cout}]")
    co4 = (Cout + 3) // 4 * 4
    y = torch.empty((B * Ho * Wo, co4 + ld_slack) if ld_slack else (B, Cout, Ho, Wo), device=x.device, dtype=torch.float32)
    check(lib.af_op_conv2d_ex(DTYPES[dtype], ptr(x), ptr(weight), ptr(b), ptr(r), ptr(rb), float(alpha), ptr(y), B, Cin, H, W, Cout,
                              ks, stride, pad, up, ld_slack, stream_ptr()), "af_op_conv2d_ex")
    if not ld_slack:
        return y
    return y[:, :Cout].reshape(B, Ho, Wo, Cout).permute(0, 3, 1, 2).contiguous(), y[:, co4:].contiguous()


OUTPUT_SENTINEL = 49152.0


FP8_ACT_SHIFT = 3


def _fp8_record(rec):
    words = rec.cpu()
    return float(words.view(torch.float32)[0]), int(words[1]) & 0xFFFFFFFF


def conv2d_fp8(x, weight, bias=None, stride=1, upsample=False, residual=None, act_shift=FP8_ACT_SHIFT):
    lib = _lib.load()
    x, weight = _dev_f32(x), _dev_f32(weight)
    B, Cin, H, W = x.shape
    Cout, Cin2, ks, ks2 = weight.shape
    if Cin2 != Cin or ks != ks2:
        raise ValueError(f"conv2d_fp8: weight {tuple(weight.shape)} does not match input {tuple(x.shape)}")
    pad, up = ks // 2, 1 if upsample else 0
    Hi, Wi = H << up, W << up
    Ho, Wo = (Hi + 2 * pad - ks) // stride + 1, (Wi + 2 * pad - ks) // stride + 1
    y = torch.empty(B, Cout, Ho, Wo, device=x.device, dtype=torch.float32)
    b = None if bias is None else _dev_f32(bias)
    r = None if residual is None else _dev_f32(residual)
    check(lib.af_op_conv2d_fp8(ptr(x), ptr(weight), ptr(b), ptr(r), ptr(y), B, Cin, H, W, Cout, ks, stride, pad, up,
                               act_shift, stream_ptr()), "af_op_conv2d_fp8")
    return y


def group_norm_fp8(x, weight, bias, eps=1e-5, silu=False, act_shift=FP8_ACT_SHIFT, record=False):
    lib = _lib.load()
    x = _dev_f32(x)
    B, Cn, H, W = x.shape
    y = torch.empty(B, H * W, Cn, device=x.device, dtype=torch.uint8)
    if record:
        rec = torch.zeros(2, device=x.device, dtype=torch.int32)
        check(lib.af_op_groupnorm_fp8_rec(ptr(x), ptr(_dev_f32(weight)), ptr(_dev_f32(bias)), eps, 1 if silu else 0, ptr(y), B,
                                          Cn, H, W, act_shift, ptr(rec), stream_ptr()), "af_op_groupnorm_fp8_rec")
        return y, _fp8_record(rec)
    check(lib.af_op_groupnorm_fp8(ptr(x), ptr(_dev_f32(weight)), ptr(_dev_f32(bias)), eps, 1 if silu else 0, ptr(y), B, Cn,
                                  H, W, act_shift, stream_ptr()), "af_op_groupnorm_fp8")
    return y


def layer_norm_fp8(x, weight, bias, eps=1e-5, act_shift=FP8_ACT_SHIFT, record=False):
    lib = _lib.load()
    x = _dev_f32(x)
    Cn = x.shape[-1]
    rows = x.numel() // Cn
    y = torch.empty(x.shape, device=x.device, dtype=torch.uint8)
    if record:
        rec = torch.zeros(2, device=x.device, dtype=torch.int32)
        check(lib.af_op_layernorm_fp8_rec(ptr(x), ptr(_dev_f32(weight)), ptr(_dev_f32(bias)), eps, ptr(y), rows, Cn, act_shift,
                                          ptr(rec), stream_ptr()), "af_op_layernorm_fp8_rec")
        return y, _fp8_record(rec)
    check(lib.af_op_layernorm_fp8(ptr(x), ptr(_dev_f32(weight)), ptr(_dev_f32(bias)), eps, ptr(y), rows, Cn, act_shift,
                                  stream_ptr()), "af_op_layernorm_fp8")
    return y


def ff_fp8(x, ln_weight, ln_bias, w1, b1, w2, b2, residual=None, shift1=FP8_ACT_SHIFT, shift2=FP8_ACT_SHIFT, eps=1e-5,
           x8=None, record=False):
    import ctypes as C
    lib = _lib.load()
    w1, w2 = _dev_f32(w1), _dev_f32(w2)
    F2, Cn = w1.shape
    Cout, Fn = w2.shape
    if F2 != 2 * Fn:
        raise ValueError(f"ff_fp8: w1 {tuple(w1.shape)} / w2 {tuple(w2.shape)}")
    if x8 is not None:
        x8 = x8.contiguous()
        assert x8.dtype == torch.uint8 and x8.shape[-1] == Cn
        M, dev = x8.numel() // Cn, x8.device
        xf = g = b = None
    else:
        xf, g, b = _dev_f32(x), _dev_f32(ln_weight), _dev_f32(ln_bias)
        M, dev = xf.numel() // Cn, xf.device
    b1 = None if b1 is None else _dev_f32(b1)
    b2 = None if b2 is None else _dev_f32(b2)
    r = None if residual is None else _dev_f32(residual)
    y = torch.empty(M, Cout, device=dev, dtype=torch.float32)
    mid = torch.empty(M, Fn, device=dev, dtype=torch.uint8)
    rec = torch.zeros(2, device=dev, dtype=torch.int32) if record else None
    plan = (C.c_int * 2)()
    check(lib.af_op_ff_fp8(ptr(xf), ptr(x8), ptr(g), ptr(b), eps, ptr(w1), ptr(b1), ptr(w2), ptr(b2), ptr(r), M, Cn, Fn, Cout,
                           shift1, shift2, ptr(rec), ptr(y), ptr(mid), plan, stream_ptr()), "af_op_ff_fp8")
    out = {"y": y, "mid8": mid, "plan": (int(plan[0]), int(plan[1]))}
    if record:
        out["record"] = _fp8_record(rec)
    return out


def linear(x, weight, bias=None, residual=None, geglu=False, dtype="bf16", alpha=1.0, ld_slack=0):
    lib = _lib.load()
    x, weight = _dev_f32(x), _dev_f32(weight)
    K = x.shape[-1]
    M = x.numel() // K
    rows = weight.shape[0]
    N = rows // 2 if geglu else rows
    b = None if bias is None else _dev_f32(bias)
    r = None if residual is None else _dev_f32(residual)
    if alpha == 1.0 and ld_slack == 0:
        y = torch.empty(*x.shape[:-1], N, device=x.device, dtype=torch.float32)
        check(lib.af_op_linear(DTYPES[dtype], ptr(x), ptr(weight), ptr(b), ptr(r), ptr(y), M, K, N, 1 if geglu else 0,
                               stream_ptr()), "af_op_linear")
        return y
    no4 = (N + 3) // 4 * 4
    y = torch.empty((M, no4 + ld_slack) if ld_slack else (*x.shape[:-1], N), device=x.device, dtype=torch.float32)
    check(lib.af_op_linear_ex(DTYPES[dtype], ptr(x), ptr(weight), ptr(b), ptr(r), float(alpha), ptr(y), M, K, N, 1 if geglu else 0,
                              ld_slack, stream_ptr()), "af_op_linear_ex")
    if not ld_slack:
        return y
    return y[:, :N].reshape(*x.shape[:-1], N).contiguous(), y[:, no4:].contiguous()


def group_norm(x, weight, bias, eps=1e-5, silu=False, dtype="bf16"):
    lib = _lib.load()
    x = _dev_f32(x)
    B, Cn, H, W = x.shape
    y = torch.empty_like(x)
    check(lib.af_op_groupnorm(DTYPES[dtype], ptr(x), ptr(_dev_f32(weight)), ptr(_dev_f32(bias)), eps, 1 if silu else 0,
                              ptr(y), B, Cn, H, W, stream_ptr()), "af_op_groupnorm")
    return y


def conv_gn(x, w, b, gamma, beta, eps=1e-5, silu=True, residual=None):
    lib = _lib.load()
    x = _dev_f32(x)
    B, Cin, H, W = x.shape
    Cout = w.shape[0]
    h = torch.empty(B, Cout, H, W, device=x.device, dtype=torch.float32)
    y = torch.empty_like(h)
    check(lib.af_op_conv_gn(ptr(x), ptr(_dev_f32(w)), ptr(_dev_f32(b)) if b is not None else None,
                            ptr(_dev_f32(residual)) if residual is not None else None, ptr(_dev_f32(gamma)), ptr(_dev_f32(beta)),
                            eps, 1 if silu else 0, ptr(h), ptr(y), B, Cin, H, W, Cout, stream_ptr()), "af_op_conv_gn")
    return h, y


def gn_conv1x1(x, gamma, beta, w, bias=None, eps=1e-6):
    lib = _lib.load()
    x = _dev_f32(x)
    B, Cn, H, W = x.shape
    N = w.shape[0]
    y0 = torch.empty(B, N, H, W, device=x.device, dtype=torch.float32)
    y1 = torch.empty_like(y0)
    check(lib.af_op_gn_conv1x1(ptr(x), ptr(_dev_f32(gamma)), ptr(_dev_f32(beta)), eps, ptr(_dev_f32(w.reshape(N, Cn))),
                               ptr(_dev_f32(bias)) if bias is not None else None, ptr(y0), ptr(y1), B, Cn, H, W, N, stream_ptr()),
          "af_op_gn_conv1x1")
    return y0, y1


def layer_norm(x, weight, bias, eps=1e-5, dtype="bf16"):
    lib = _lib.load()
    x = _dev_f32(x)
    Cn = x.shape[-1]
    y = torch.empty_like(x)
    check(lib.af_op_layernorm(DTYPES[dtype], ptr(x), ptr(_dev_f32(weight)), ptr(_dev_f32(bias)), eps, ptr(y),
                              x.numel() // Cn, Cn, stream_ptr()), "af_op_layernorm")
    return y


def tome_match(x, hw, ratio, normalize=True, dtype="bf16"):
    lib = _lib.load()
    x = _dev_f32(x)
    B, N, Cn = x.shape
    H, W = hw
    if H * W != N:
        raise ValueError(f"tome_match: {H} x {W} map, {N} tokens")
    Nd, Ns, _, _ = _lib.tome_plan_query(H, W, ratio)
    node_idx = torch.empty(B, Ns, device=x.device, dtype=torch.int32)
    node_max = torch.empty(B, Ns, device=x.device, dtype=torch.float32)
    tmap = torch.empty(B, N, device=x.device, dtype=torch.int32)
    check(lib.af_op_tome_match(DTYPES[dtype], ptr(x), B, H, W, Cn, float(ratio), 1 if normalize else 0, ptr(node_idx),
                               ptr(node_max), ptr(tmap), stream_ptr()), "af_op_tome_match")
    return node_idx, node_max, tmap


def tome_merge(x, tmap, n_rows, weight=None, bias=None, eps=1e-5, dtype="bf16"):
    lib = _lib.load()
    x = _dev_f32(x)
    B, N, Cn = x.shape
    tmap = tmap.to(device=x.device, dtype=torch.int32).contiguous()
    y = torch.empty(B, int(n_rows), Cn, device=x.device, dtype=torch.float32)
    check(lib.af_op_tome_merge(DTYPES[dtype], ptr(x), ptr(_dev_f32(weight)) if weight is not None else None,
                               ptr(_dev_f32(bias)) if bias is not None else None, eps, ptr(tmap), B, N, int(n_rows), Cn, ptr(y),
                               stream_ptr()), "af_op_tome_merge")
    return y


def tome_unmerge_add(o, res, tmap, dtype="bf16"):
    lib = _lib.load()
    o, res = _dev_f32(o), _dev_f32(res)
    B, N, Cn = res.shape
    tmap = tmap.to(device=res.device, dtype=torch.int32).contiguous()
    y = torch.empty_like(res)
    check(lib.af_op_tome_unmerge_add(DTYPES[dtype], ptr(o), ptr(res), ptr(tmap), B, N, o.shape[1], Cn, ptr(y), stream_ptr()),
          "af_op_tome_unmerge_add")
    return y


def freeu(h, skip, version, b, s, dtype="bf16"):
    lib = _lib.load()
    h, skip = _dev_f32(h), _dev_f32(skip)
    B, Ch, H, W = h.shape
    if skip.shape[0] != B or tuple(skip.shape[2:]) != (H, W):
        raise ValueError(f"freeu: h {tuple(h.shape)} and skip {tuple(skip.shape)} do not concatenate")
    h_out, skip_out = torch.empty_like(h), torch.empty_like(skip)
    check(lib.af_op_freeu(DTYPES[dtype], ptr(h), ptr(skip), B, Ch, skip.shape[1], H, W, int(version), float(b), float(s),
                          ptr(h_out), ptr(skip_out), stream_ptr()), "af_op_freeu")
    return h_out, skip_out


def attention(q, k, v, heads, scale=None, dtype="bf16", causal=False, nan_guard=False):
    lib = _lib.load()
    q, k, v = _dev_f32(q), _dev_f32(k), _dev_f32(v)
    B, Nq, Cn = q.shape
    Nk = k.shape[1]
    dh = Cn // heads
    scale = dh ** -0.5 if scale is None else scale
    o = torch.empty_like(q)
    check(lib.af_op_attention(DTYPES[dtype], ptr(q), ptr(k), ptr(v), ptr(o), B, Nq, Nk, heads, dh, scale,
                              (1 if causal else 0) | (2 if nan_guard else 0), stream_ptr()),
          "af_op_attention")
    return o


CONV_ATTN_PATHS = {"auto": 0, "merge": 1, "one_pass": 2}


def conv_attn_key_order(n_keys, token_idx, ks):
    nt = ks * ks
    groups = [[int(t) for t in g] for g in token_idx]
    if ks not in (2, 3, 4):
        raise ValueError(f"conv attention: kernel size {ks} (the reference has 2, 3 and 4)")
    if not groups or any(len(g) != nt for g in groups):
        raise ValueError(f"conv attention: every subject string needs ks^2 = {nt} token positions")
    flat = [t for g in groups for t in g]
    if any(t < 0 or t >= n_keys for t in flat):
        raise ValueError(f"conv attention: token position outside [0, {n_keys})")
    if len(set(flat)) != len(flat):
        raise ValueError("conv attention: a token position appears twice")
    if len(flat) >= n_keys:
        raise ValueError("conv attention: no ordinary key left")
    subj = set(flat)
    return [t for t in range(n_keys) if t not in subj] + flat


def conv_attention(q, k, v, heads, hw, ks, token_idx, scale=None, dtype="bf16", path="auto"):
    lib = _lib.load()
    q, k, v = _dev_f32(q), _dev_f32(k), _dev_f32(v)
    B, N, Cn = q.shape
    Nk = k.shape[1]
    Hh, Ww = hw
    if Hh * Ww != N:
        raise ValueError(f"conv_attention: hw {hw} does not match {N} queries")
    dh = Cn // heads
    scale = dh ** -0.5 if scale is None else scale
    order = torch.tensor(conv_attn_key_order(Nk, token_idx, ks), device=q.device)
    k, v = k[:, order].contiguous(), v[:, order].contiguous()
    o = torch.empty_like(q)
    check(lib.af_op_conv_attention(DTYPES[dtype], ptr(q), ptr(k), ptr(v), ptr(o), B, Hh, Ww, Nk, heads, dh, scale, ks,
                                   len(token_idx), CONV_ATTN_PATHS[path], stream_ptr()), "af_op_conv_attention")
    return o


GEMM_KERNELS = {1: "wave4", 2: "halo4", 3: "pp", 4: "pp_fp8", 5: "halo8", 6: "s8", 7: "up_phase4", 8: "rowpanel", 9: "m128"}


def vae_attention(q, k, v, dtype="bf16", taps=False):
    import ctypes as C
    lib = _lib.load()
    q, k, v = _dev_f32(q), _dev_f32(k), _dev_f32(v)
    if q.dim() != 3 or k.shape != q.shape or v.shape != q.shape:
        raise ValueError(f"vae_attention: q {tuple(q.shape)}, k {tuple(k.shape)}, v {tuple(v.shape)} must all be [B, N, C]")
    B, N, Cn = q.shape
    o = torch.empty_like(q)
    sc = torch.empty(B, N, N, device=q.device, dtype=torch.float32) if taps else None
    pr = torch.empty(B, N, N, device=q.device, dtype=torch.float32) if taps else None
    plans = (C.c_int * 6)()
    check(lib.af_op_vae_attention(DTYPES[dtype], ptr(q), ptr(k), ptr(v), ptr(o), B, N, Cn, ptr(sc), ptr(pr), plans, stream_ptr()),
          "af_op_vae_attention")
    if not taps:
        return o
    return {"out": o, "scores": sc, "probs": pr,
            "plans": tuple((GEMM_KERNELS.get(int(plans[3 * i]), int(plans[3 * i])), int(plans[3 * i + 1]), int(plans[3 * i + 2]))
                           for i in range(2))}


def xattn_fused(x, gamma, beta, wq, kv, wo, bo, eps=1e-5):
    lib = _lib.load()
    x = _dev_f32(x)
    B, N, Cn = x.shape
    S = kv.shape[1]
    xb = x.to(torch.bfloat16).float().reshape(B * N, Cn)
    mu = xb.mean(dim=1)
    var = (xb * xb).mean(dim=1) - mu * mu
    stats = torch.stack([mu, torch.rsqrt(var.clamp_min(0) + eps)], dim=1).contiguous()
    y = torch.empty_like(x)
    parts = torch.empty(4, B * N, 2, device=x.device, dtype=torch.float32)
    check(lib.af_op_xattn_fused(ptr(x), ptr(stats), ptr(_dev_f32(gamma)), ptr(_dev_f32(beta)), ptr(_dev_f32(wq)), ptr(_dev_f32(kv)),
                                ptr(_dev_f32(wo)), ptr(_dev_f32(bo)), ptr(y), ptr(parts), B, N, S, stream_ptr()), "af_op_xattn_fused")
    return y, parts


def timestep_embedding(t, dim, dtype="f32"):
    lib = _lib.load()
    t = t.contiguous().long()
    y = torch.empty(t.shape[0], dim, device=t.device, dtype=torch.float32)
    check(lib.af_op_timestep_embedding(DTYPES[dtype], ptr(t), ptr(y), t.shape[0], dim, stream_ptr()),
          "af_op_timestep_embedding")
    return y


def ddim_step(x, e_cond, e_uncond, guidance, a_t, a_prev, sqrt_one_minus_at, sigma_t=0.0, noise=None, temperature=1.0):
    lib = _lib.load()
    x, e_cond = _dev_f32(x), _dev_f32(e_cond)
    eu = None if e_uncond is None else _dev_f32(e_uncond)
    nz = None if noise is None else _dev_f32(noise)
    x_prev, pred_x0 = torch.empty_like(x), torch.empty_like(x)
    check(lib.af_ddim_step(ptr(x), ptr(e_cond), ptr(eu), ptr(nz), x.numel(), float(guidance), float(a_t), float(a_prev),
                           float(sqrt_one_minus_at), float(sigma_t), float(temperature), ptr(x_prev), ptr(pred_x0),
                           stream_ptr()), "af_ddim_step")
    return x_prev, pred_x0


def dpmpp_coeffs(acp_t, acp_prev, h_last=0.0):
    import ctypes
    out = (ctypes.c_double * 8)()
    check(_lib.load().af_dpmpp_coeffs(float(acp_t), float(acp_prev), float(h_last), out), "af_dpmpp_coeffs")
    return tuple(float(v) for v in out)


def dpmpp_step(x, e_cond, e_uncond, x0_prev, guidance, alpha_t, sigma_t, c_x, c_d, w_cur=1.0, w_prev=0.0, x_next=None,
               x0_out=None, want_x0=True):
    lib = _lib.load()
    x, e_cond = _dev_f32(x), _dev_f32(e_cond)
    eu = None if e_uncond is None else _dev_f32(e_uncond)
    xp = None if x0_prev is None else _dev_f32(x0_prev)
    for name, t in (("e_cond", e_cond), ("e_uncond", eu), ("x0_prev", xp)):
        if t is not None and t.numel() != x.numel():
            raise ValueError(f"dpmpp_step: {name} has {t.numel()} elements, x has {x.numel()}")
    for name, t in (("x_next", x_next), ("x0_out", x0_out)):
        if t is not None and not (t.is_cuda and t.dtype == torch.float32 and t.is_contiguous() and t.numel() == x.numel()):
            raise ValueError(f"dpmpp_step: {name} must be a contiguous fp32 GPU tensor of x's size")
    if x_next is None:
        x_next = torch.empty_like(x)
    if x0_out is None and want_x0:
        x0_out = torch.empty_like(x)
    check(lib.af_dpmpp_step(ptr(x), ptr(e_cond), ptr(eu), ptr(xp), x.numel(), float(guidance), float(alpha_t), float(sigma_t),
                            float(c_x), float(c_d), float(w_cur), float(w_prev), ptr(x_next), ptr(x0_out), stream_ptr()),
          "af_dpmpp_step")
    return x_next, x0_out


def philox4x32_10(ctr, key):
    import ctypes
    c = (ctypes.c_uint32 * 4)(*[int(v) & 0xFFFFFFFF for v in ctr])
    k = (ctypes.c_uint32 * 2)(*[int(v) & 0xFFFFFFFF for v in key])
    out = (ctypes.c_uint32 * 4)()
    check(_lib.load().af_philox4x32_10(c, k, out), "af_philox4x32_10")
    return tuple(int(v) for v in out)


def philox_randn(n_samples, per_sample, seed, stream, step, sample_ids=None, first_id=0, device=None, out=None):
    n_samples, per_sample = int(n_samples), int(per_sample)
    if out is None:
        out = torch.empty(n_samples, per_sample, device=device, dtype=torch.float32)
    if not (out.is_cuda and out.dtype == torch.float32 and out.is_contiguous() and out.numel() == n_samples * per_sample):
        raise ValueError("philox_randn: out must be a contiguous fp32 GPU tensor of n_samples * per_sample elements")
    if sample_ids is not None and not (sample_ids.is_cuda and sample_ids.dtype == torch.int64 and sample_ids.is_contiguous()
                                       and sample_ids.numel() >= n_samples):
        raise ValueError("philox_randn: sample_ids must be a contiguous int64 GPU tensor of at least n_samples elements")
    check(_lib.load().af_philox_randn(ptr(out), n_samples, per_sample, ptr(sample_ids), int(first_id),
                                      int(seed) & 0xFFFFFFFFFFFFFFFF, int(stream), int(step), stream_ptr()), "af_philox_randn")
    return out


def dpmpp_sde_coeffs(acp_t, acp_prev, h_last=0.0):
    import ctypes
    out = (ctypes.c_double * 9)()
    check(_lib.load().af_dpmpp_sde_coeffs(float(acp_t), float(acp_prev), float(h_last), out), "af_dpmpp_sde_coeffs")
    return tuple(float(v) for v in out)


def dpmpp_sde_step(x, e_cond, e_uncond, x0_prev, guidance, alpha_t, sigma_t, c_x, c_d, c_n, w_cur=1.0, w_prev=0.0, noise=None,
                   seed=0, step=0, sample_ids=None, first_id=0, x_next=None, x0_out=None, want_x0=True):
    lib = _lib.load()
    x, e_cond = _dev_f32(x), _dev_f32(e_cond)
    eu = None if e_uncond is None else _dev_f32(e_uncond)
    xp = None if x0_prev is None else _dev_f32(x0_prev)
    nz = None if noise is None else _dev_f32(noise)
    for name, t in (("e_cond", e_cond), ("e_uncond", eu), ("x0_prev", xp), ("noise", nz)):
        if t is not None and t.numel() != x.numel():
            raise ValueError(f"dpmpp_sde_step: {name} has {t.numel()} elements, x has {x.numel()}")
    for name, t in (("x_next", x_next), ("x0_out", x0_out)):
        if t is not None and not (t.is_cuda and t.dtype == torch.float32 and t.is_contiguous() and t.numel() == x.numel()):
            raise ValueError(f"dpmpp_sde_step: {name} must be a contiguous fp32 GPU tensor of x's size")
    n_samples = x.shape[0] if x.dim() > 0 else 1
    if sample_ids is not None and not (sample_ids.is_cuda and sample_ids.dtype == torch.int64 and sample_ids.is_contiguous()
                                       and sample_ids.numel() >= n_samples):
        raise ValueError("dpmpp_sde_step: sample_ids must be a contiguous int64 GPU tensor of at least x.shape[0] elements")
    if x_next is None:
        x_next = torch.empty_like(x)
    if x0_out is None and want_x0:
        x0_out = torch.empty_like(x)
    check(lib.af_dpmpp_sde_step(ptr(x), ptr(e_cond), ptr(eu), ptr(xp), x.numel(), float(guidance), float(alpha_t), float(sigma_t),
                                float(c_x), float(c_d), float(w_cur), float(w_prev), ptr(x_next), ptr(x0_out), float(c_n), ptr(nz),
                                x.numel() // n_samples, ptr(sample_ids), int(first_id), int(seed) & 0xFFFFFFFFFFFFFFFF, int(step),
                                stream_ptr()), "af_dpmpp_sde_step")
    return x_next, x0_out


def lincomb(terms, cfg=False):
    lib = _lib.load()
    xs = [_dev_f32(t) for t, _ in terms]
    ws = [float(w) for _, w in terms]
    while len(xs) < 4:
        xs.append(None)
        ws.append(0.0)
# ... 16 lines not shown
```

include/adaface_hip.h:

```cpp
#ifndef ADAFACE_HIP_H
#define ADAFACE_HIP_H
#include <stdint.h>
#ifdef __cplusplus
extern "C" {
#endif

typedef struct af_handle af_handle;

enum { AF_DTYPE_BF16 = 0, AF_DTYPE_F32 = 1, AF_DTYPE_F16 = 2 };
enum {
  AF_OK = 0,
  AF_ERR_INVALID = -1,
  AF_ERR_HIP = -2,
  AF_ERR_NAME = -3,
  AF_ERR_STATE = -4
};

typedef struct af_config {
  int dtype;
  int build_unet;
  int in_channels, model_channels, out_channels, num_res_blocks;
  int n_attention_resolutions, attention_resolutions[8];
  int n_channel_mult, channel_mult[8];
  int num_heads, context_dim, transformer_depth;
  int n_context_layers;
  int build_vae;
  int vae_ch, vae_out_ch, vae_num_res_blocks, vae_z_channels, vae_embed_dim;
  int n_vae_ch_mult, vae_ch_mult[8];
  int build_vae_encoder;
  int vae_in_channels;
  int build_clip;
  int clip_vocab, clip_hidden, clip_layers, clip_heads, clip_intermediate, clip_max_pos;
} af_config;

const char* af_last_error(void);
int af_version(void);

int af_create(int device_id, const af_config* cfg, af_handle** out);
void af_destroy(af_handle* h);

int af_load_tensor(af_handle* h, const char* name, const float* host_data, int ndim, const int64_t* shape);
int af_load_tensor_device(af_handle* h, const char* name, const float* dev_data, int ndim, const int64_t* shape);
int af_num_tensors(af_handle* h);
const char* af_tensor_name(af_handle* h, int i);
int af_tensor_loaded(af_handle* h, int i);
int af_tensor_shape(af_handle* h, int i, int64_t* shape4 );

int af_set_conv_attn(af_handle* h, int ks, int n_subj, const int* batch_idx, const int* token_idx);
int af_set_context(af_handle* h, const float* ctx_dev, int Bf, int n_tokens, int layerwise, void* stream);

int af_unet_forward(af_handle* h, const float* x_dev, const int64_t* t_dev, float* eps_dev, int Bf, int H, int W,
                    void* stream);
int af_unet_forward_twin(af_handle* h, const float* x_dev, const int64_t* t_dev, float* eps_dev, int Bf, int H, int W,
                         void* stream);

enum { AF_DEEPCACHE_REFRESH = 1, AF_DEEPCACHE_REUSE = 2 };
int af_unet_forward_cached(af_handle* h, const float* x_dev, const int64_t* t_dev, float* eps_dev, int Bf, int H, int W,
                           int twin, int depth, int mode, void* stream);
int af_unet_cache_invalidate(af_handle* h);

int af_set_tome(af_handle* h, double ratio, int max_downsample);
int af_tome_plan_query(int H, int W, double ratio, int64_t out[4]);
int af_tome_num_sites(af_handle* h);
int af_tome_set_tap(af_handle* h, int site, int32_t* map_dev);
int af_op_tome_match(int dtype, const float* x_dev, int B, int H, int W, int C, double ratio, int normalize, int32_t* node_idx_dev,
                     float* node_max_dev, int32_t* map_dev, void* stream);
int af_op_tome_merge(int dtype, const float* x_dev, const float* gamma_dev, const float* beta_dev, float eps,
                     const int32_t* map_dev, int B, int N, int Nprime, int C, float* y_dev, void* stream);
int af_op_tome_unmerge_add(int dtype, const float* o_dev, const float* res_dev, const int32_t* map_dev, int B, int N, int Nprime,
                           int C, float* y_dev, void* stream);

int af_set_freeu(af_handle* h, int version, double b1, double b2, double s1, double s2);
int af_freeu_num_sites(af_handle* h);
int af_freeu_site(af_handle* h, int site, int out[4]);
int af_freeu_plan_query(int dtype, int H, int W, int Ch, int Cs, int version, int64_t out[4]);
int af_op_freeu(int dtype, const float* h_dev, const float* skip_dev, int B, int Ch, int Cs, int H, int W, int version, double b,
                double s, float* h_out_dev, float* skip_out_dev, void* stream);

int af_clip_embed_tokens(af_handle* h, const int64_t* ids_dev, int64_t n, float* emb_dev, void* stream);
int af_clip_text_forward(af_handle* h, const float* inputs_embeds_dev, int Bn, int T, float w_prev, float w_last,
                         float* out_dev, void* stream);
int af_clip_text_forward3(af_handle* h, const float* inputs_embeds_dev, int Bn, int T, float w_prev2, float w_prev, float w_last,
                          float* out_dev, void* stream);

int af_unet_num_blocks(af_handle* h);
int af_unet_block_shape(af_handle* h, int block, int H, int W, int* C_out, int* H_out, int* W_out);
int af_unet_set_tap(af_handle* h, int block, float* out_dev);

int af_ddim_step(const float* x_dev, const float* eps_cond_dev, const float* eps_uncond_dev, const float* noise_dev,
                 int64_t n, float guidance, float a_t, float a_prev, float sqrt_one_minus_at, float sigma_t,
                 float temperature, float* x_prev_dev, float* pred_x0_dev, void* stream);

int af_dpmpp_coeffs(double acp_t, double acp_prev, double h_last, double out[8]);
int af_dpmpp_step(const float* x_dev, const float* eps_cond_dev, const float* eps_uncond_dev, const float* x0_prev_dev, int64_t n,
                  float guidance, float alpha_t, float sigma_t, float c_x, float c_d, float w_cur, float w_prev,
                  float* x_next_dev, float* x0_out_dev, void* stream);

int af_philox4x32_10(const uint32_t ctr[4], const uint32_t key[2], uint32_t out[4]);
int af_philox_randn(float* out_dev, int64_t n_samples, int64_t per_sample, const int64_t* sample_ids_dev, int64_t first_id,
                    uint64_t seed, uint32_t stream_id, uint32_t step, void* stream);
int af_dpmpp_sde_coeffs(double acp_t, double acp_prev, double h_last, double out[9]);
int af_dpmpp_sde_step(const float* x_dev, const float* eps_cond_dev, const float* eps_uncond_dev, const float* x0_prev_dev, int64_t n,
                      float guidance, float alpha_t, float sigma_t, float c_x, float c_d, float w_cur, float w_prev,
                      float* x_next_dev, float* x0_out_dev, float c_n, const float* noise_dev, int64_t per_sample,
                      const int64_t* sample_ids_dev, int64_t first_id, uint64_t seed, uint32_t step, void* stream);

int af_lincomb(float* out_dev, int64_t n, const float* x0_dev, float w0, const float* x1_dev, float w1,
               const float* x2_dev, float w2, const float* x3_dev, float w3, int mode, void* stream);

int af_vae_decode(af_handle* h, const float* z_dev, float scale_factor, float* img_dev, uint8_t* u8_dev, int B, int H,
                  int W, void* stream);

int af_vae_encode(af_handle* h, const float* x_dev, float* moments_dev, int B, int H, int W, void* stream);
int af_posterior_sample(const float* moments_dev, const float* noise_dev, float scale, float* z_dev, int B, int C,
                        int HW, void* stream);
int af_to_uint8(const float* img_dev, uint8_t* u8_dev, int B, int H, int W, void* stream);

int64_t af_arena_bytes(af_handle* h);

int af_prof_enable(int class_mask);
int af_prof_reset(void);
int af_prof_set_stride(int every);
double af_flops_issued(int reset);
int af_clock_probe(void* stream, int iters, double* mfma_mhz, double* mfma_tflops);
int af_prof_collect(int n_classes, double* ms, int64_t* launches, double* flops, double* bytes);
double af_prof_event_overhead_us(void* stream, int n);
int af_last_gemm_plan(int* tile, int* splitk, int* halo_tw);
int af_gemm_plan_counts(int64_t* counts10);
int af_gemm_plan_counts_reset(void);
enum {
  AF_PQ_GEGLU = 1, AF_PQ_RESIDUAL = 2, AF_PQ_ROWBIAS = 4, AF_PQ_LN_CONSUMER = 8, AF_PQ_LN_PRODUCER = 16, AF_PQ_GN_AB = 32,
  AF_PQ_GN_STATS_OUT = 64, AF_PQ_FP8 = 128, AF_PQ_PHASE_WEIGHTS = 256, AF_PQ_WORKSPACE = 512
};
int af_gemm_plan_query(int dtype, int64_t M, int N, int K, int cin_pad, int ks, int stride, int pad, int up, int Hs, int Ws, int Ho,
                       int Wo, int ldc, int ldo, int gn_hw, int gn_cpg, int flags, int64_t* out7);
int af_norm_plan_query(int kind, int dtype, int B, int64_t n, int C, int pre_npart, int64_t* out5);

int af_knob_set(const char* name, int value);
int af_knob_get(const char* name, int* value);
int af_knob_reset(void);

int af_op_conv2d(int dtype, const float* x_dev, const float* w_dev, const float* bias_dev, const float* residual_dev,
                 float* y_dev, int B, int Cin, int H, int W, int Cout, int ks, int stride, int pad, int upsample,
                 void* stream);
int af_op_conv2d_ex(int dtype, const float* x_dev, const float* w_dev, const float* bias_dev, const float* residual_dev,
                    const float* rowbias_dev, float alpha, float* y_dev, int B, int Cin, int H, int W, int Cout, int ks, int stride,
                    int pad, int upsample, int ld_slack, void* stream);
int af_op_linear(int dtype, const float* x_dev, const float* w_dev, const float* bias_dev, const float* residual_dev,
                 float* y_dev, int64_t M, int K, int N, int geglu, void* stream);
int af_op_linear_ex(int dtype, const float* x_dev, const float* w_dev, const float* bias_dev, const float* residual_dev, float alpha,
                    float* y_dev, int64_t M, int K, int N, int geglu, int ld_slack, void* stream);
int af_op_conv_gn(const float* x_dev, const float* w_dev, const float* bias_dev, const float* residual_dev,
                  const float* gamma_dev, const float* beta_dev, float eps, int silu, float* h_dev, float* y_dev, int B,
                  int Cin, int H, int W, int Cout, void* stream);
int af_op_groupnorm(int dtype, const float* x_dev, const float* gamma_dev, const float* beta_dev, float eps, int silu,
                    float* y_dev, int B, int C, int H, int W, void* stream);
int af_set_fp8(af_handle* h, int on);
#define AF_FP8_SHIFT_MIN (-16)
#define AF_FP8_SHIFT_MAX 8
#define AF_FP8_SHIFT_DEFAULT 3
int af_fp8_num_sites(af_handle* h);
const char* af_fp8_site_name(af_handle* h, int i);
int af_fp8_record(af_handle* h, int on, void* stream);
int af_fp8_read_record(af_handle* h, int n, float* amax, int64_t* nsat, void* stream);
int af_fp8_get_shifts(af_handle* h, int n, int* shifts);
int af_fp8_set_shifts(af_handle* h, int n, const int* shifts);
int af_fp8_shift_for_amax(float amax, int headroom);
#define AF_FP8_SCOPE_BASE 1
#define AF_FP8_SCOPE_FF 2
int af_set_fp8_scope(af_handle* h, int mask);
int af_get_fp8_scope(af_handle* h);
int64_t af_ff8_launches(void);
int af_op_ff_fp8(const float* x_dev, const unsigned char* x8_dev, const float* gamma_dev, const float* beta_dev, float eps,
                 const float* w1_dev, const float* b1_dev, const float* w2_dev, const float* b2_dev, const float* residual_dev,
                 int64_t M, int C, int F, int Cout, int shift1, int shift2, void* rec_out_dev, float* y_dev,
                 unsigned char* mid8_dev, int* plan_out, void* stream);
int64_t af_fp8_gemm_launches(void);
int64_t af_halo8_launches(void);
int64_t af_gn_producer_launches(void);
int64_t af_attn_short_launches(void);
int64_t af_xattn_fused_launches(void);
int64_t af_conv_attn_short_launches(void);
int af_op_conv_attention(int dtype, const float* q_dev, const float* k_dev, const float* v_dev, float* o_dev, int B, int Hh,
                         int Ww, int Nk, int heads, int dh, float scale, int ks, int n_groups, int path, void* stream);
int af_op_vae_attention(int dtype, const float* q_dev, const float* k_dev, const float* v_dev, float* o_dev, int B, int N, int C,
                        float* scores_dev, float* probs_dev, int* plans6, void* stream);
int af_op_xattn_fused(const float* x_dev, const float* ln_stats_dev, const float* gamma_dev, const float* beta_dev,
                      const float* wq_dev, const float* kv_dev, const float* wo_dev, const float* bo_dev, float* y_dev,
                      float* ln_parts_out_dev, int B, int N, int S, void* stream);
int64_t af_gn_consumer_launches(void);
int64_t af_up_phase4_launches(void);
int64_t af_rowpanel_launches(void);
int af_op_conv2d_fp8(const float* x_dev, const float* w_dev, const float* bias_dev, const float* residual_dev, float* y_dev,
                     int B, int Cin, int H, int W, int Cout, int ks, int stride, int pad, int upsample, int act_shift,
                     void* stream);
int af_op_groupnorm_fp8(const float* x_dev, const float* gamma_dev, const float* beta_dev, float eps, int silu,
                        unsigned char* y8_dev, int B, int C, int H, int W, int act_shift, void* stream);
int af_op_layernorm_fp8(const float* x_dev, const float* gamma_dev, const float* beta_dev, float eps, unsigned char* y8_dev,
                        int64_t rows, int C, int act_shift, void* stream);
int af_op_groupnorm_fp8_rec(const float* x_dev, const float* gamma_dev, const float* beta_dev, float eps, int silu,
                            unsigned char* y8_dev, int B, int C, int H, int W, int act_shift, void* rec_out_dev, void* stream);
int af_op_layernorm_fp8_rec(const float* x_dev, const float* gamma_dev, const float* beta_dev, float eps, unsigned char* y8_dev,
                            int64_t rows, int C, int act_shift, void* rec_out_dev, void* stream);
int af_op_gn_conv1x1(const float* x_dev, const float* gamma_dev, const float* beta_dev, float eps, const float* w_dev,
                     const float* bias_dev, float* y_plain_dev, float* y_fused_dev, int B, int C, int H, int W, int N,
                     void* stream);
int af_op_layernorm(int dtype, const float* x_dev, const float* gamma_dev, const float* beta_dev, float eps,
                    float* y_dev, int64_t rows, int C, void* stream);
int af_op_attention(int dtype, const float* q_dev, const float* k_dev, const float* v_dev, float* o_dev, int B, int Nq,
                    int Nk, int heads, int dh, float scale, int causal, void* stream);
int af_op_timestep_embedding(int dtype, const int64_t* t_dev, float* y_dev, int B, int dim, void* stream);

#ifdef __cplusplus
}
#endif
#endif
```

Measured before the change: 10.83.

## Add strip-halo 3x3 conv kernel for tile-4 bf16 convs and enable by default

Adds a new 8-wave 3x3 convolution kernel that stages an input halo strip (up to 64-wide rows) in LDS, double-buffered per Cin chunk. All nine taps are read from that strip instead of re-gathering the input per tap, and weights are staged through a 3-slot LDS ring. The planner routes eligible stride-1, pad-1, power-of-two-sized tile-4 convs to this kernel, and the default conv_halo8 knob changes from 3 to 11 so the path is on by default. The kernel uses the direct epilogue and can feed group-norm statistics. It adds a large LDS footprint, which may reduce occupancy. The change also exposes a conv_gn variant that copies out partial GN statistics, plus a launch counter.

Result: no change. 10.86, median of 6 (+0.3%).

```diff
diff --git a/adaface_amd/_lib.py b/adaface_amd/_lib.py
--- a/adaface_amd/_lib.py
+++ b/adaface_amd/_lib.py
@@ -96,6 +96,7 @@
     ("af_op_linear_ex", C.c_int, [C.c_int, _P, _P, _P, _P, C.c_float, _P, C.c_int64, C.c_int, C.c_int, C.c_int, C.c_int, _P]),
     ("af_op_groupnorm", C.c_int, [C.c_int, _P, _P, _P, C.c_float, C.c_int, _P, C.c_int, C.c_int, C.c_int, C.c_int, _P]),
     ("af_op_conv_gn", C.c_int, [_P, _P, _P, _P, _P, _P, C.c_float, C.c_int, _P, _P] + [C.c_int] * 5 + [_P]),
+    ("af_op_conv_gn_parts", C.c_int, [_P, _P, _P, _P, _P, _P, C.c_float, C.c_int, _P, _P, _P] + [C.c_int] * 5 + [_P]),
     ("af_set_fp8", C.c_int, [_P, C.c_int]),
     ("af_fp8_gemm_launches", C.c_int64, []),
     ("af_set_fp8_scope", C.c_int, [_P, C.c_int]),
@@ -110,6 +111,7 @@
     ("af_fp8_set_shifts", C.c_int, [_P, C.c_int, C.POINTER(C.c_int)]),
     ("af_fp8_shift_for_amax", C.c_int, [C.c_float, C.c_int]),
     ("af_halo8_launches", C.c_int64, []),
+    ("af_halo8v_launches", C.c_int64, []),
     ("af_rowpanel_launches", C.c_int64, []),
     ("af_up_phase4_launches", C.c_int64, []),
     ("af_gn_producer_launches", C.c_int64, []),
@@ -190,6 +192,7 @@
     out["fp8"] = int(lib.af_fp8_gemm_launches())
     out["ff8"] = int(lib.af_ff8_launches())
     out["halo8"] = int(lib.af_halo8_launches())
+    out["halo8v"] = int(lib.af_halo8v_launches())
     out["rowpanel"] = int(lib.af_rowpanel_launches())
     out["up_phase4"] = int(lib.af_up_phase4_launches())
     out["gn_producer"] = int(lib.af_gn_producer_launches())
diff --git a/adaface_amd/csrc/af_common.h b/adaface_amd/csrc/af_common.h
--- a/adaface_amd/csrc/af_common.h
+++ b/adaface_amd/csrc/af_common.h
@@ -311,7 +311,8 @@
   AF_GK_S8 = 6,
   AF_GK_UP_PHASE4 = 7,
   AF_GK_ROWPANEL = 8,
-  AF_GK_M128 = 9
+  AF_GK_M128 = 9,
+  AF_GK_HALO8V = 10
 };
 
 struct AfGemmPlan {
diff --git a/adaface_amd/csrc/af_conv_gemm.hip b/adaface_amd/csrc/af_conv_gemm.hip
--- a/adaface_amd/csrc/af_conv_gemm.hip
+++ b/adaface_amd/csrc/af_conv_gemm.hip
@@ -1002,6 +1002,219 @@
 #endif
 }
 
+struct Halo8vCfg {
+  static constexpr int BN = 128;
+  static constexpr int HPIX = 400, HBUF = HPIX * 128, WBYTES = BN * 128;
+  static constexpr int W_BASE = 2 * HBUF, LDS_BYTES = 2 * HBUF + 3 * WBYTES;
+  static constexpr int NHQ = 7;
+  static constexpr int NWQ = 2;
+  static_assert(LDS_BYTES <= 160 * 1024, "LDS budget");
+};
+__global__ __launch_bounds__(512) void conv3x3_halo8v_kernel(const ConvGemmParams p) {
+  using C = PpCfg<128>;
+  using H = Halo8vCfg;
+  typedef bf16 T;
+  constexpr int BN = 128, NI = C::NI, MI = C::MI, NHQ = H::NHQ, NWQ = H::NWQ;
+  extern __shared__ __attribute__((aligned(1024))) char smem[];
+  const int tid = threadIdx.x, lane = tid & 63, wid = __builtin_amdgcn_readfirstlane(tid >> 6);
+  const int g = wid >> 2, wq = wid & 3;
+  const int ntm = p.M / 256, ntn = p.N / BN;
+  int tm, tn;
+  tile_coords(blockIdx.x, gridDim.x, ntm, ntn, p.group_m, tm, tn);
+  const int n0 = tn * BN;
+  const int zk = blockIdx.z;
+  const __amdgpu_buffer_rsrc_t rs_x = buffer_rsrc(p.src);
+  const __amdgpu_buffer_rsrc_t rs_w = buffer_rsrc(p.W);
+
+  const int KT_all = p.K / 64;
+  const int kt_per = (KT_all + p.splitk - 1) / p.splitk;
+  const int kt_begin = zk * kt_per;
+  const int KT = min(KT_all, kt_begin + kt_per) - kt_begin;
+  const int chunk0 = kt_begin / 9;
+  const int nch = KT / 9;
+
+  const int Wo = p.Wo, wsh = p.wo_shift;
+  const int tsh = wsh < 6 ? wsh : 6, TW = 1 << tsh, HW = TW + 2;
+  const int R = 256 >> tsh;
+  const int HP = (R + 2) * HW;
+  const int ish = p.howo_shift - 8;
+  const int img = tm >> ish, ti = tm & ((1 << ish) - 1);
+  const int y0 = (ti >> (wsh - tsh)) * R, x0 = (ti & ((1 << (wsh - tsh)) - 1)) << tsh;
+  const int m0w = (img << p.howo_shift) + (y0 + ((wq * 64) >> tsh)) * Wo + x0 + ((wq * 64) & (TW - 1)) - wq * 64;
+  const int srow = lane >> 3;
+  const unsigned dchunk = (unsigned)((lane & 7) ^ srow);
+  const unsigned ldcb = (unsigned)p.ldc * 2u;
+
+  unsigned h_off[NHQ];
+  const int nhq = (H::HPIX / 8 - 1 - wid) / 8 + 1;
+#pragma unroll
+  for (int q = 0; q < NHQ; ++q) {
+    const int hp = (wid + 8 * q) * 8 + srow;
+    const int hy = hp / HW, hx = hp - hy * HW;
+    const int iy = y0 - 1 + hy, ix = x0 - 1 + hx;
+    const bool ok = hp < HP && (unsigned)iy < (unsigned)p.Hi && (unsigned)ix < (unsigned)p.Wi;
+    h_off[q] = ok ? (unsigned)((long)img * p.src_batch_stride * 2) + (unsigned)(iy * p.Ws + ix) * ldcb + dchunk * 16u : 0xFFFFFFFFu;
+  }
+  const unsigned hl6 = (unsigned)(wid < 2 ? 8 * (NHQ - 1) * 1024 : 0);
+  if (wid >= 2) h_off[NHQ - 1] = h_off[0];
+  unsigned w_off[NWQ];
+#pragma unroll
+  for (int q = 0; q < NWQ; ++q) {
+    const int n = n0 + (wid + 8 * q) * 8 + srow;
+    w_off[q] = n < p.Wrows ? (unsigned)((long)n * p.ldw * 2) + dchunk * 16u : 0xFFFFFFFFu;
+  }
+  const unsigned cin2 = (unsigned)p.Cin * 2u;
+
+  const unsigned lds0 = (unsigned)(__UINTPTR_TYPE__)((__attribute__((address_space(3))) char*)smem);
+  const unsigned fch0 = (unsigned)((lane >> 4) ^ (lane & 7)) * 16u;
+  const unsigned fch1 = (unsigned)(((lane >> 4) + 4) ^ (lane & 7)) * 16u;
+  const unsigned w_base = (unsigned)((g * C::HN + (lane & 15)) * 128);
+  const unsigned wrd0 = lds0 + (unsigned)H::W_BASE + w_base + fch0, wrd1 = lds0 + (unsigned)H::W_BASE + w_base + fch1;
+  unsigned xh16[MI];
+#pragma unroll
+  for (int j = 0; j < MI; ++j) {
+    const int t = wq * 64 + j * 16 + (lane & 15);
+    xh16[j] = (unsigned)((t >> tsh) * HW + (t & (TW - 1))) << 4;
+  }
+  const unsigned qsel16 = (unsigned)(lane >> 4) << 4;
+  const unsigned hw16 = (unsigned)HW * 16u;
+
+  f32x4 acc[NI][MI];
+#pragma unroll
+  for (int i = 0; i < NI; ++i)
+#pragma unroll
+    for (int j = 0; j < MI; ++j) acc[i][j] = f32x4{0.f, 0.f, 0.f, 0.f};
+  u32x4 w8[NI][2], xp[MI][2];
+#pragma unroll
+  for (int i = 0; i < NI; ++i) w8[i][0] = w8[i][1] = u32x4{0u, 0u, 0u, 0u};
+#pragma unroll
+  for (int j = 0; j < MI; ++j) xp[j][0] = xp[j][1] = u32x4{0u, 0u, 0u, 0u};
+  auto mfma2 = [&](f32x4& c, const u32x4 (&wv)[2], const u32x4 (&xv)[2]) {
+    c = __builtin_amdgcn_mfma_f32_16x16x32_bf16(__builtin_bit_cast(bf16x8, wv[0]), __builtin_bit_cast(bf16x8, xv[0]), c, 0, 0, 0);
+    c = __builtin_amdgcn_mfma_f32_16x16x32_bf16(__builtin_bit_cast(bf16x8, wv[1]), __builtin_bit_cast(bf16x8, xv[1]), c, 0, 0, 0);
+    asm volatile("" : "+v"(c));
+  };
+  auto wait_block = [&](auto nc, u32x4 (&blk)[2]) {
+    constexpr int n = decltype(nc)::value;
+    wait_lgkm<n>(blk[0], blk[1]);
+  };
+  auto wait_block2 = [&](auto nc, u32x4 (&b0)[2], u32x4 (&b1)[2]) {
+    constexpr int n = decltype(nc)::value;
+    wait_lgkm<n>(b0[0], b0[1], b1[0], b1[1]);
+  };
+
+  {
+    const unsigned kc = (unsigned)chunk0 * 128u;
+#pragma unroll
+    for (int q = 0; q < NHQ; ++q)
+      if (q < nhq) lds_dma16(rs_x, smem + (wid + 8 * q) * 1024, h_off[q], kc);
+#pragma unroll
+    for (int s = 0; s < 2; ++s) {
+      char* const dst = smem + H::W_BASE + s * H::WBYTES + wid * 1024;
+#pragma unroll
+      for (int q = 0; q < NWQ; ++q) lds_dma16(rs_w, dst + 8 * q * 1024, w_off[q], s * cin2 + kc);
+    }
+  }
+
+  auto chunk_loop = [&](auto gc) {
+    constexpr int G = decltype(gc)::value;
+    constexpr int NHT = G == 0 ? 7 : 6;
+    char* const wdst = smem + H::W_BASE + wid * 1024;
+    for (int c = 0; c < nch; ++c) {
+      const unsigned kc = (unsigned)(chunk0 + c) * 128u;
+      const int nrec = c + 1 < nch ? (int)0xFFFFFFF0u : 0;
+      const __amdgpu_buffer_rsrc_t rs_xn = buffer_rsrc(p.src, nrec);
+      const __amdgpu_buffer_rsrc_t rs_wn = buffer_rsrc(p.W, nrec);
+      const unsigned hrd8 = (lds0 + (unsigned)((c & 1) * H::HBUF)) >> 3;
+      char* const hdst = smem + ((c & 1) ^ 1) * H::HBUF + wid * 1024;
+      static_for<0, 9>([&](auto tc) {
+        constexpr int TAP = decltype(tc)::value;
+        constexpr int KY = TAP / 3, KX = TAP % 3, WS = TAP % 3, WS2 = (TAP + 2) % 3, T2 = TAP + 2;
+        constexpr int NB = NI + MI;
+        wait_vm<NWQ + (TAP >= 1 && TAP <= NHT ? 1 : 0)>();
+        __builtin_amdgcn_s_barrier();
+        const unsigned ut = hrd8 + KY * hw16 + KX * 16u;
+        unsigned xa0[MI];
+#pragma unroll
+        for (int j = 0; j < MI; ++j) {
+          const unsigned u = xh16[j] + ut;
+          xa0[j] = (u << 3) | ((u ^ qsel16) & 0x70u);
+        }
+        u32x4 xc[MI][2];
+        auto rd_block = [&](auto bc) {
+          constexpr int bi = decltype(bc)::value;
+          if constexpr (bi == 0) {
+            w8[0][0] = lds_read128<WS * H::WBYTES>(wrd0);
+            w8[0][1] = lds_read128<WS * H::WBYTES>(wrd1);
+          } else if constexpr (bi <= MI) {
+            xc[bi - 1][0] = lds_read128<0>(xa0[bi - 1]);
+            xc[bi - 1][1] = lds_read128<0>(xa0[bi - 1] ^ 64u);
+          } else {
+            w8[bi - MI][0] = lds_read128<WS * H::WBYTES + (bi - MI) * 2048>(wrd0);
+            w8[bi - MI][1] = lds_read128<WS * H::WBYTES + (bi - MI) * 2048>(wrd1);
+          }
+        };
+        auto stage_w = [&](auto qc) {
+          constexpr int q = decltype(qc)::value;
+          char* const dst = wdst + WS2 * H::WBYTES + 8 * q * 1024;
+          if constexpr (T2 < 9) lds_dma16(rs_w, dst, w_off[q], T2 * cin2 + kc);
+          else lds_dma16(rs_wn, dst, w_off[q], (T2 - 9) * cin2 + kc + 128u);
+        };
+        auto stage_h = [&]() {
+          if constexpr (TAP < NHT) {
+            if constexpr (TAP < NHQ - 1) lds_dma16(rs_xn, hdst + 8 * TAP * 1024, h_off[TAP], kc + 128u);
+            else lds_dma16(rs_xn, hdst + hl6, h_off[NHQ - 1], kc + 128u);
+          }
+        };
+        rd_block(std::integral_constant<int, 0>{});
+        rd_block(std::integral_constant<int, 1>{});
+        __builtin_amdgcn_sched_barrier(0);
+        static_for<0, MI * NI>([&](auto mc) {
+          constexpr int m = decltype(mc)::value;
+          if constexpr (m < MI) {
+            mfma2(acc[NI - 1][m], w8[NI - 1], xp[m]);
+          } else {
+            constexpr int i = (m - MI) / MI, j = (m - MI) % MI;
+            constexpr int issued = (2 + m) < NB ? (2 + m) : NB;
+            constexpr int need = i == 0 ? 1 + j : (j == 0 ? MI + i : -1);
+            if constexpr (need >= 0) {
+              std::integral_constant<int, 2 * (issued - need - 1)> cnt;
+              if constexpr (i == 0 && j == 0) wait_block2(cnt, xc[0], w8[0]);
+              else if constexpr (i == 0) wait_block(cnt, xc[j]);
+              else wait_block(cnt, w8[i]);
+            }
+            mfma2(acc[i][j], w8[i], xc[j]);
+          }
+          if constexpr (2 + m < NB) rd_block(std::integral_constant<int, 2 + m>{});
+          if constexpr (m == MI + G) stage_w(std::integral_constant<int, 0>{});
+          if constexpr (m == MI + 2 + G) stage_w(std::integral_constant<int, 1>{});
+          if constexpr (m == MI + 6 + G) stage_h();
+          __builtin_amdgcn_sched_barrier(0);
+        });
+        wait_lgkm_fenced<0>();
+#pragma unroll
+        for (int j = 0; j < MI; ++j) xp[j][0] = xc[j][0], xp[j][1] = xc[j][1];
+      });
+    }
+  };
+  if (g == 0) chunk_loop(std::integral_constant<int, 0>{});
+  else chunk_loop(std::integral_constant<int, 1>{});
+  wait_vm<0>();
+#pragma unroll
+  for (int j = 0; j < MI; ++j) mfma2(acc[NI - 1][j], w8[NI - 1], xp[j]);
+  __builtin_amdgcn_s_barrier();
+  const int cl = 4 * (lane >> 4);
+  float4 bias_r[NI];
+#pragma unroll
+  for (int i = 0; i < NI; ++i) {
+    bias_r[i] = float4{0.f, 0.f, 0.f, 0.f};
+    if (p.bias && p.splitk <= 1) bias_r[i] = *reinterpret_cast<const float4*>(p.bias + n0 + g * C::HN + i * 16 + cl);
+  }
+  float4 ln_cs[1];
+  float ln_mu[1], ln_rs[1];
+  pp_epilogue<128, 0>(p, acc, bias_r, ln_cs, ln_mu, ln_rs, smem, tid, lane, g, wq, m0w, n0, tn, zk);
+}
+
 template <bool GEGLU, int KC_ = 5, int MJ_ = 2, int D_ = 2> struct RowPanelCfgT {
   static constexpr int KC = KC_, MJ = MJ_, K = KC * 64, D = D_, NS = D_ + 1;
   static constexpr int WROWS = 16 * MJ, BM = 8 * WROWS;
@@ -2050,6 +2263,13 @@
     pl.halo_tw = 256;
     while (pl.splitk > 1 && (p.Cin / 64) % pl.splitk != 0) --pl.splitk;
   }
+  if (pl.tile == 4 && pl.halo_tw == 0 && p.ks == 3 && p.stride == 1 && p.pad == 1 && p.up == 0 && p.Ho == p.Hi && p.Wo == p.Wi &&
+      p.Wo >= 64 && (p.Wo & (p.Wo - 1)) == 0 && (p.Ho & (p.Ho - 1)) == 0 && p.Ho >= 4 && p.M % (p.Ho * p.Wo) == 0 &&
+      (p.Wo > 64 || p.N > 128 || (g_af_knobs.conv_halo8 & 16)) && p.K == 9 * p.Cin && p.Cin % 64 == 0 && p.ldc >= p.Cin && p.Ws == p.Wi && !geglu &&
+      (g_af_knobs.conv_halo8 & 8) && !p.ln_stats && !p.ln_stats_out) {
+    pl.halo_tw = 64;
+    while (pl.splitk > 1 && (p.Cin / 64) % pl.splitk != 0) --pl.splitk;
+  }
   if (is_bf16 && (g_af_knobs.conv_halo8 & 2) && g_af_knobs.gemm_pp && af_conv_s8_slices(p, batch) && !p.gn_stats_out &&
       (p.Wo <= 16 || (g_af_knobs.conv_halo8 & 4))) {
     pl.tile = 5;
@@ -2061,9 +2281,11 @@
   const int fs = g_af_knobs.gemm_splitk;
   if (fs >= 1 && batch == 1 && !geglu) pl.splitk = fs > KT ? KT : fs;
   if (pl.halo_tw == 8 && (pl.tile != 5 || pl.splitk != af_conv_s8_slices(p, batch))) pl.halo_tw = 0;
-  if (pl.splitk > 1 && pl.halo_tw != 256 && pl.halo_tw != 8) pl.halo_tw = 0;
+  if (pl.splitk > 1 && pl.halo_tw != 256 && pl.halo_tw != 8 && pl.halo_tw != 64) pl.halo_tw = 0;
   if (pl.halo_tw == 256 && (pl.tile != 5 || (p.Cin / 64) % pl.splitk != 0)) pl.halo_tw = 0;
-  pl.kernel = pl.halo_tw == 8 ? AF_GK_S8 : pl.halo_tw == 256 ? AF_GK_HALO8 : pl.halo_tw ? AF_GK_HALO4 : pl.tile >= 4 ? AF_GK_PP : AF_GK_WAVE4;
+  if (pl.halo_tw == 64 && (pl.tile != 4 || (p.Cin / 64) % pl.splitk != 0)) pl.halo_tw = 0;
+  pl.kernel = pl.halo_tw == 8 ? AF_GK_S8 : pl.halo_tw == 256 ? AF_GK_HALO8 : pl.halo_tw == 64 ? AF_GK_HALO8V : pl.halo_tw ? AF_GK_HALO4 :
+              pl.tile >= 4 ? AF_GK_PP : AF_GK_WAVE4;
   plan_group_m(pl, p);
   return pl;
 }
@@ -2113,7 +2335,7 @@
   p.howo_shift = lg2(p.Ho * p.Wo);
   p.wo_shift = lg2(p.Wo);
   p.group_m = pl.group_m > 0 ? pl.group_m : 1;
-  p.epi_direct = (p.gn_stats_out || p.phase4) ? 1 : 0;
+  p.epi_direct = (p.gn_stats_out || p.phase4 || pl.kernel == AF_GK_HALO8V) ? 1 : 0;
   p.ablate = p.phase4 ? 0 : g_af_knobs.ablate;
 }
 
@@ -2219,6 +2441,19 @@
   return launch_halo8_lab<0>(p, stream);
 }
 
+static int launch_halo8v(const ConvGemmParams& p, hipStream_t stream) {
+  auto pow2 = [](int v) { return v > 0 && (v & (v - 1)) == 0; };
+  if (p.Cin % 64 != 0 || (p.Cin / 64) % (p.splitk > 1 ? p.splitk : 1) != 0 || p.K != 9 * p.Cin || p.N % 128 != 0 || !pow2(p.Wo) || p.Wo < 64 ||
+      !pow2(p.Ho) || p.Ho < 4 || p.M % (p.Ho * p.Wo) != 0 || p.Ho != p.Hi || p.Wo != p.Wi || p.Ws != p.Wi || p.up != 0 || p.stride != 1 ||
+      p.pad != 1 || p.ks != 3 || p.ldc < p.Cin || !p.epi_direct || p.phase4 || p.epilogue == AF_EPI_GEGLU || p.ln_stats || p.ln_stats_out) {
+    af_set_error_msg("conv_gemm: strip halo kernel cannot take M=%d N=%d Cin=%d %dx%d ks=%d stride=%d up=%d splitk=%d", p.M, p.N, p.Cin, p.Ho,
+                     p.Wo, p.ks, p.stride, p.up, p.splitk);
+    return -1;
+  }
+  dim3 grid((p.M / 256) * (p.N / 128), 1, p.splitk > 1 ? p.splitk : 1);
+  return af_launch_lds<conv3x3_halo8v_kernel>(grid, dim3(512), Halo8vCfg::LDS_BYTES, Halo8vCfg::LDS_BYTES, stream, p);
+}
+
 template <typename T, int TW, int BN> static int launch_halo(const ConvGemmParams& p, hipStream_t stream) {
   using C = HaloCfg<TW, BN>;
   dim3 grid((p.M / 128) * ((p.N + BN - 1) / BN), 1, 1);
@@ -2290,7 +2525,7 @@
 bool af_conv_gn_stats_ok(const ConvGemmParams& p, const AfGemmPlan& pl, int cpg) {
   auto pow2 = [](int v) { return v > 0 && (v & (v - 1)) == 0; };
   const int hn = pl.tile == 5 ? 80 : 64;
-  const bool eight_wave = pl.kernel == AF_GK_PP || pl.kernel == AF_GK_PP_FP8 || pl.kernel == AF_GK_HALO8;
+  const bool eight_wave = pl.kernel == AF_GK_PP || pl.kernel == AF_GK_PP_FP8 || pl.kernel == AF_GK_HALO8 || pl.kernel == AF_GK_HALO8V;
   return g_af_knobs.gn_producer && eight_wave && pl.splitk <= 1 && p.ks == 3 && p.stride == 1 && p.up == 0 &&
          p.epilogue != AF_EPI_GEGLU && !p.ln_stats && !p.ln_stats_out && cpg >= 2 && cpg % 2 == 0 && hn % cpg == 0 &&
          p.N == 32 * cpg && pow2(p.Ho * p.Wo) && p.Ho * p.Wo >= 64 && p.M % 64 == 0;
@@ -2360,6 +2595,7 @@
     case AF_GK_PP: return pl.tile == 4 ? launch_pp<128>(p, stream) : launch_pp<160>(p, stream);
     case AF_GK_PP_FP8: return pl.tile == 4 ? launch_pp8<128>(p, stream) : launch_pp8<160>(p, stream);
     case AF_GK_HALO8: return launch_halo8(p, stream);
+    case AF_GK_HALO8V: return launch_halo8v(p, stream);
     case AF_GK_S8: return af_launch_conv_s8(p, stream);
     case AF_GK_UP_PHASE4: return launch_up_phase4(p, pl.tile, stream);
     case AF_GK_M128: return launch_gemm_m128(p, stream);
@@ -2435,6 +2671,7 @@
   } else {
     g_af_plan_counts[k == AF_GK_HALO4 ? AF_PC_HALO4 : AF_PC_TILE0 + (pl.tile >= 0 && pl.tile < 6 ? pl.tile : 0)] += 1;
     if (k == AF_GK_HALO8) g_af_plan_counts[AF_PC_HALO8] += 1;
+    if (k == AF_GK_HALO8V) g_af_plan_counts[AF_PC_HALO8V] += 1;
     if (p.ln_stats) g_af_plan_counts[AF_PC_LN_CONSUMER] += 1;
     if (p.ln_stats_out) g_af_plan_counts[AF_PC_LN_PRODUCER] += 1;
   }
diff --git a/adaface_amd/csrc/af_kernels.h b/adaface_amd/csrc/af_kernels.h
--- a/adaface_amd/csrc/af_kernels.h
+++ b/adaface_amd/csrc/af_kernels.h
@@ -181,7 +181,8 @@
   AF_PC_ROWPANEL = 12,
   AF_PC_UP_PHASE4 = 13,
   AF_PC_GN_PRODUCER = 14,
-  AF_PC_COUNT = 15
+  AF_PC_HALO8V = 15,
+  AF_PC_COUNT = 16
 };
 extern std::atomic<long> g_af_plan_counts[AF_PC_COUNT];
 extern std::atomic<long> g_af_gn_consumer_launches;
diff --git a/adaface_amd/csrc/af_model.hip b/adaface_amd/csrc/af_model.hip
--- a/adaface_amd/csrc/af_model.hip
+++ b/adaface_amd/csrc/af_model.hip
@@ -28,7 +28,7 @@
     knob_env("AF_GEMM_PP_MINFILL", 50), knob_env("AF_GEMM_TILE", -1),
     knob_env("AF_GEMM_SPLITK", -1),    knob_env("AF_GEMM_GROUPM", -1),    knob_env("AF_GEMM_DMA", -1),
     knob_env("AF_ATTN_RING", 3),       knob_env("AF_GN_SMALL", 1),
-    knob_env("AF_LN_FUSE", 1),         knob_env("AF_GEGLU_ROWPANEL", 4), knob_env("AF_CONV_HALO8", 3), knob_env("AF_ABLATE", 0),
+    knob_env("AF_LN_FUSE", 1),         knob_env("AF_GEGLU_ROWPANEL", 4), knob_env("AF_CONV_HALO8", 11), knob_env("AF_ABLATE", 0),
     knob_env("AF_GN_PRODUCER", 1),     knob_env("AF_CONV_UP_PHASE4", 1), knob_env("AF_ATTN_SHORT", 1),
     knob_env("AF_GEMM_M128", 1),       knob_env("AF_SMALL_M_TILE64", 1),  knob_env("AF_GN_CONSUMER", 1),
     knob_env("AF_XATTN_FUSED", 1),     knob_env("AF_PLAN_LOG", 0),      knob_env("AF_FF8_MIN_K", 512),   knob_env("AF_FF8_MIN_ROWS", 0),
@@ -2578,6 +2578,7 @@
 int64_t af_fp8_gemm_launches(void) { return g_af_plan_counts[AF_PC_FP8]; }
 int64_t af_ff8_launches(void) { return g_af_ff8_launches; }
 int64_t af_halo8_launches(void) { return g_af_plan_counts[AF_PC_HALO8]; }
+int64_t af_halo8v_launches(void) { return g_af_plan_counts[AF_PC_HALO8V]; }
 int64_t af_rowpanel_launches(void) { return g_af_plan_counts[AF_PC_ROWPANEL]; }
 int64_t af_up_phase4_launches(void) { return g_af_plan_counts[AF_PC_UP_PHASE4]; }
 int64_t af_gn_producer_launches(void) { return g_af_plan_counts[AF_PC_GN_PRODUCER]; }
diff --git a/adaface_amd/csrc/af_ops.hip b/adaface_amd/csrc/af_ops.hip
--- a/adaface_amd/csrc/af_ops.hip
+++ b/adaface_amd/csrc/af_ops.hip
@@ -563,6 +563,12 @@
 int af_op_conv_gn(const float* x_dev, const float* w_dev, const float* bias_dev, const float* residual_dev,
                   const float* gamma_dev, const float* beta_dev, float eps, int silu, float* h_dev, float* y_dev, int B,
                   int Cin, int H, int W, int Cout, void* stream) {
+  return af_op_conv_gn_parts(x_dev, w_dev, bias_dev, residual_dev, gamma_dev, beta_dev, eps, silu, h_dev, y_dev, nullptr, B, Cin, H, W,
+                             Cout, stream);
+}
+int af_op_conv_gn_parts(const float* x_dev, const float* w_dev, const float* bias_dev, const float* residual_dev,
+                        const float* gamma_dev, const float* beta_dev, float eps, int silu, float* h_dev, float* y_dev,
+                        float* parts_dev, int B, int Cin, int H, int W, int Cout, void* stream) {
   hipStream_t s = reinterpret_cast<hipStream_t>(stream);
   Tmp tmp;
   if (Cin % 64 != 0 || Cout % 32 != 0) { af_set_error_msg("af_op_conv_gn: Cin%%64==0 and Cout%%32==0"); return AF_ERR_INVALID; }
@@ -604,6 +610,8 @@
   p.gn_stats_out = reinterpret_cast<float*>(st);
   p.gn_cpg = Cout / 32;
   AF_TRY(af_launch_conv_gemm<bf16>(p, 1, s, &pl, nullptr));
+  if (parts_dev && hipMemcpyAsync(parts_dev, st, (size_t)B * (HW / 64) * 32 * 2 * sizeof(float), hipMemcpyDeviceToDevice, s) != hipSuccess)
+    return AF_ERR_HIP;
   AF_TRY(af_launch_groupnorm<bf16>(hn, (long)HW * Cout, Cout, B, HW, Cout, gamma_dev, beta_dev, eps, silu, yn, (long)HW * Cout,
                                    Cout, ws, s, 0.f, reinterpret_cast<const float*>(st), HW / 64));
   AF_TRY(af_launch_nhwc_to_nchw<bf16>(hn, h_dev, B, Cout, HW, Cout, s));
diff --git a/adaface_amd/ops.py b/adaface_amd/ops.py
--- a/adaface_amd/ops.py
+++ b/adaface_amd/ops.py
@@ -173,17 +173,18 @@
     return y
 
 
-def conv_gn(x, w, b, gamma, beta, eps=1e-5, silu=True, residual=None):
+def conv_gn(x, w, b, gamma, beta, eps=1e-5, silu=True, residual=None, parts=False):
     lib = _lib.load()
     x = _dev_f32(x)
     B, Cin, H, W = x.shape
     Cout = w.shape[0]
     h = torch.empty(B, Cout, H, W, device=x.device, dtype=torch.float32)
     y = torch.empty_like(h)
-    check(lib.af_op_conv_gn(ptr(x), ptr(_dev_f32(w)), ptr(_dev_f32(b)) if b is not None else None,
-                            ptr(_dev_f32(residual)) if residual is not None else None, ptr(_dev_f32(gamma)), ptr(_dev_f32(beta)),
-                            eps, 1 if silu else 0, ptr(h), ptr(y), B, Cin, H, W, Cout, stream_ptr()), "af_op_conv_gn")
-    return h, y
+    ps = torch.empty(B, H * W // 64, 32, 2, device=x.device, dtype=torch.float32) if parts else None
+    check(lib.af_op_conv_gn_parts(ptr(x), ptr(_dev_f32(w)), ptr(_dev_f32(b)) if b is not None else None,
+                                  ptr(_dev_f32(residual)) if residual is not None else None, ptr(_dev_f32(gamma)), ptr(_dev_f32(beta)),
+                                  eps, 1 if silu else 0, ptr(h), ptr(y), ptr(ps), B, Cin, H, W, Cout, stream_ptr()), "af_op_conv_gn_parts")
+    return (h, y, ps) if parts else (h, y)
 
 
 def gn_conv1x1(x, gamma, beta, w, bias=None, eps=1e-6):
@@ -313,7 +314,7 @@
     return o
 
 
-GEMM_KERNELS = {1: "wave4", 2: "halo4", 3: "pp", 4: "pp_fp8", 5: "halo8", 6: "s8", 7: "up_phase4", 8: "rowpanel", 9: "m128"}
+GEMM_KERNELS = {1: "wave4", 2: "halo4", 3: "pp", 4: "pp_fp8", 5: "halo8", 6: "s8", 7: "up_phase4", 8: "rowpanel", 9: "m128", 10: "halo8v"}
 
 
 def vae_attention(q, k, v, dtype="bf16", taps=False):
diff --git a/include/adaface_hip.h b/include/adaface_hip.h
--- a/include/adaface_hip.h
+++ b/include/adaface_hip.h
@@ -153,6 +153,9 @@
 int af_op_conv_gn(const float* x_dev, const float* w_dev, const float* bias_dev, const float* residual_dev,
                   const float* gamma_dev, const float* beta_dev, float eps, int silu, float* h_dev, float* y_dev, int B,
                   int Cin, int H, int W, int Cout, void* stream);
+int af_op_conv_gn_parts(const float* x_dev, const float* w_dev, const float* bias_dev, const float* residual_dev,
+                        const float* gamma_dev, const float* beta_dev, float eps, int silu, float* h_dev, float* y_dev,
+                        float* parts_dev, int B, int Cin, int H, int W, int Cout, void* stream);
 int af_op_groupnorm(int dtype, const float* x_dev, const float* gamma_dev, const float* beta_dev, float eps, int silu,
                     float* y_dev, int B, int C, int H, int W, void* stream);
 int af_set_fp8(af_handle* h, int on);
@@ -177,6 +180,7 @@
                  unsigned char* mid8_dev, int* plan_out, void* stream);
 int64_t af_fp8_gemm_launches(void);
 int64_t af_halo8_launches(void);
+int64_t af_halo8v_launches(void);
 int64_t af_gn_producer_launches(void);
 int64_t af_attn_short_launches(void);
 int64_t af_xattn_fused_launches(void);
```
